# leosampaio/sketchformer

Hardware: AMD Instinct MI355X
Metric: stroke-tokens/sec training step, d_model=128 L=200 B=128, 1/2/4/8 GPU (higher is better)
Workload: dtype f32; 1 GPU; cfg2: sketch-transformer-tf2 4L/8H/d128/dff512 L=200 V=1004 C=345 dropout=0.1, fwd+bwd+Adam(WarmupDecay); global_batch=128, per_gpu_batch=128, seq_len=200, parallelism=dp1, hip_graph=0, dense_gemm_arithmetic=fp32 operands split exactly into 3 bf16 pieces, 6 product...

## Files before the change

include/skf.h:

```cpp
#ifndef SKF_H_
#define SKF_H_
#include <stddef.h>
#include <stdint.h>
#ifdef __cplusplus
extern "C" {
#endif

typedef void* skf_stream_t;

#define SKF_OK 0
#define SKF_EINVAL (-1)
#define SKF_EUNSUPPORTED (-2)
#define SKF_EHIP (-3)

const char* skf_last_error(void);
int skf_version(void);
int skf_device_info(char* name_host, size_t name_len, int* n_devices_host);

int skf_profiler_enable(int on);
int skf_profiler_report(char* buf_host, size_t len);

#define SKF_PREC_F32 0
#define SKF_PREC_BF16X3 3
#define SKF_PREC_BF16X6 6
#define SKF_ATTN_TWO_PASS 0x100
size_t skf_gemm_workspace_bytes(int M, int N, int K, int splits, int with_bias_grad);
int skf_gemm_default_splits(int M, int N, int K);
int skf_gemm_f32(int a_kcontig, int b_kcontig, int M, int N, int K, const float* A, int lda, const float* B, int ldb,
                 float* C, int ldc, const float* bias, int act, const float* relu_src, int ld_relu, int accumulate,
                 int splits, float* bias_grad, int bias_grad_accumulate, void* workspace, size_t workspace_bytes,
                 int precision, skf_stream_t stream);

typedef struct SkfReduceDesc {
  const float* slab; float* C; float* bias_grad;
  int32_t splits, M, N, ldc, block_begin, pad;
} SkfReduceDesc;
int skf_gemm_wgrad_partial(int M, int N, int K, const float* A, int lda, const float* B, int ldb, int splits,
                           int with_bias_grad, float* slab, size_t slab_bytes, int* splits_used_host, int precision,
                           skf_stream_t stream);
int skf_target_live_len(const long long* tar, int tar_ld, int B, int Ld, int* live_len, skf_stream_t stream);
size_t skf_row_blocks_bytes(int rows, int granule);
int skf_row_blocks_build(const int* live_len, int B, int rows_per_sample, int granule, int* blocks, skf_stream_t stream);
int skf_gemm_f32_rows(int a_kcontig, int b_kcontig, int M, int N, int K, const float* A, int lda, const float* B, int ldb,
                      float* C, int ldc, const float* bias, int act, const float* relu_src, int ld_relu, int accumulate,
                      int splits, float* bias_grad, int bias_grad_accumulate, void* workspace, size_t workspace_bytes,
                      int precision, const int* row_blocks, int row_block_rows, skf_stream_t stream);
size_t skf_gemm_relu_bits_bytes(int M, int N, int K, int precision);
int skf_gemm_f32_bits(int a_kcontig, int b_kcontig, int M, int N, int K, const float* A, int lda, const float* B, int ldb,
                      float* C, int ldc, const float* bias, int act, const float* relu_src, int ld_relu, int accumulate,
                      int splits, float* bias_grad, int bias_grad_accumulate, void* workspace, size_t workspace_bytes,
                      int precision, const int* row_blocks, int row_block_rows, void* relu_bits_out, const void* relu_bits_in,
                      skf_stream_t stream);
int skf_gemm_ln_residual_supported(int M, int N, int K, int precision);
int skf_gemm_ln_residual_f32(int M, int N, int K, const float* A, int lda, const float* W, int ldw, const float* bias,
                             const float* x, const float* gamma, const float* beta, float* z, float* out, float* stats,
                             float rate, unsigned site, const void* step_state, int precision, skf_stream_t stream);
int skf_ffn_fused_supported(int M, int d, int dff, int precision);
size_t skf_ffn_image_bytes(int d, int dff, int precision);
size_t skf_ffn_relu_bits_bytes(int M, int d, int dff, int precision);
int skf_ffn_weight_images(int n, const float* const* W1, const int* ld1, const float* const* W2, const int* ld2,
                          const int* transpose, void* const* images, int d, int dff, int precision, skf_stream_t stream);
int skf_ffn_fused_fwd_f32(int M, int d, int dff, const float* x, const void* image, const float* b1, const float* b2,
                          float* h, void* relu_bits_out, const float* gamma, const float* beta, float* z, float* out,
                          float* stats, float rate, unsigned site, const void* step_state, int precision, skf_stream_t stream);
int skf_ffn_fused_bwd_f32(int M, int d, int dff, const float* dy, const void* image_t, const void* relu_bits_in,
                          float* dh, float* dx, int accumulate, const int* row_blocks, int row_block_rows,
                          int precision, skf_stream_t stream);
int skf_ffn_fused_fwd_proj_f32(int M, int d, int dff, const float* x, const void* image, const float* b1, const float* b2,
                               float* h, void* relu_bits_out, const float* gamma, const float* beta, float* z, float* out,
                               float* stats, float rate, unsigned site, const void* step_state, const void* proj_image,
                               const float* proj_bias, int proj_n, float* proj_out, int precision, skf_stream_t stream);
typedef struct SkfFfnBlockFwd {
  uint32_t struct_size; int32_t M, d, dff, precision;
  const float* x; const void* image; const float* b1; const float* b2; float* h; void* relu_bits_out;
  const float* gamma; const float* beta; float* z; float* out; float* stats;
  float rate; uint32_t site; const void* step_state;
  const void* pre_image; const float* pre_bias; const float* pre_residual; const float* pre_gamma; const float* pre_beta;
  float* pre_z; float* pre_out; float* pre_stats; uint32_t pre_site; int32_t proj_n;
  const void* proj_image; const float* proj_bias; float* proj_out;
} SkfFfnBlockFwd;
int skf_ffn_block_fwd_f32(const SkfFfnBlockFwd* block, skf_stream_t stream);
int skf_ffn_fused_ln_partials(int M);
int skf_ffn_fused_bwd_ln_f32(int M, int d, int dff, const float* dout, const float* z, const float* stats, const float* gamma,
                             float rate, unsigned site, const void* step_state, const void* image_t, const void* relu_bits_in,
                             float* dy, float* dh, float* dx, float* ln_partials, size_t ln_partials_bytes,
                             const int* row_blocks, int row_block_rows, int precision, skf_stream_t stream);
size_t skf_dense_image_bytes(int K, int N, int precision);
int skf_dense_weight_images(int n, const float* const* src, const int* ld, const int* transpose, const int* K, const int* N,
                            void* const* images, int precision, skf_stream_t stream);
int skf_layernorm_bwd_dgrad_supported(int M, int d, int precision);
int skf_layernorm_bwd_dgrad_partials(int M);
int skf_layernorm_bwd_dgrad_f32(int M, int d, const float* dout, const float* z, const float* stats, const float* gamma,
                                float rate, unsigned site, const void* step_state, const void* image_t, float* dz, float* dy,
                                float* da, float* ln_partials, size_t ln_partials_bytes, const int* row_blocks,
                                int row_block_rows, int precision, skf_stream_t stream);
int skf_layernorm_bwd_dgrad_lead_f32(int M, int d, const float* dout, const float* lead_a, const void* lead_image_t, const float* z,
                                     const float* stats, const float* gamma, float rate, unsigned site, const void* step_state,
                                     const void* image_t, float* dz, float* dy, float* da, float* ln_partials, size_t ln_partials_bytes,
                                     const int* row_blocks, int row_block_rows, int precision, skf_stream_t stream);
int skf_gemm_wgrad_partial_rows(int M, int N, int K, const float* A, int lda, const float* B, int ldb, int splits,
                                int with_bias_grad, float* slab, size_t slab_bytes, int* splits_used_host, int precision,
                                const int* row_blocks, int row_block_rows, skf_stream_t stream);
typedef struct SkfWgradProblem {
  const float* A; const float* B; float* slab; size_t slab_bytes; const int* row_blocks;
  int32_t M, N, K, lda, ldb, splits, with_bias_grad, row_block_rows, splits_used, pad;
} SkfWgradProblem;
int skf_gemm_wgrad_partial_group(SkfWgradProblem* probs, int n, int precision, skf_stream_t stream);
int skf_splitk_reduce(const float* slab, int splits, int M, int N, float* C, int ldc, int accumulate, float* bias_grad,
                      int bias_grad_accumulate, skf_stream_t stream);
int skf_splitk_reduce_blocks(int M, int N);
int skf_splitk_reduce_batch(const SkfReduceDesc* descs_dev, int ndesc, int total_blocks, skf_stream_t stream);

int skf_attention_fwd(const float* Q, int ldq, const float* K, int ldk, const float* V, int ldv,
                      const unsigned char* key_mask, int key_mask_ld, int causal, int B, int H, int Lq, int Lk, int dh,
                      float* O, int ldo, float* stats, int precision, skf_stream_t stream);
int skf_attention_bwd(const float* Q, int ldq, const float* K, int ldk, const float* V, int ldv, const float* O, int ldo,
                      const float* dO, int lddo, const float* stats, const unsigned char* key_mask, int key_mask_ld,
                      int causal, int B, int H, int Lq, int Lk, int dh, float* dQ, int lddq, float* dK, int lddk,
                      float* dV, int lddv, int precision, skf_stream_t stream);
int skf_attention_bwd_rows(const float* Q, int ldq, const float* K, int ldk, const float* V, int ldv, const float* O, int ldo,
                           const float* dO, int lddo, const float* stats, const unsigned char* key_mask, int key_mask_ld,
                           int causal, int B, int H, int Lq, int Lk, int dh, float* dQ, int lddq, float* dK, int lddk,
                           float* dV, int lddv, int precision, const int* q_live_len, skf_stream_t stream);
int skf_sample_order(const unsigned char* mask_a, int lda, int La, const unsigned char* mask_b, int ldb, int Lb, int B, int* order,
                     skf_stream_t stream);
int skf_attention_fwd_ordered(const float* Q, int ldq, const float* K, int ldk, const float* V, int ldv,
                              const unsigned char* key_mask, int key_mask_ld, int causal, int B, int H, int Lq, int Lk, int dh,
                              float* O, int ldo, float* stats, int precision, const int* sample_order, skf_stream_t stream);
int skf_attention_bwd_ordered(const float* Q, int ldq, const float* K, int ldk, const float* V, int ldv, const float* O, int ldo,
                              const float* dO, int lddo, const float* stats, const unsigned char* key_mask, int key_mask_ld,
                              int causal, int B, int H, int Lq, int Lk, int dh, float* dQ, int lddq, float* dK, int lddk,
                              float* dV, int lddv, int precision, const int* q_live_len, const int* sample_order, skf_stream_t stream);
int skf_attention_weights(const float* Q, int ldq, const float* K, int ldk, const unsigned char* key_mask, int key_mask_ld,
                          int causal, int B, int H, int Lq, int Lk, int dh, float* W, skf_stream_t stream);
int skf_attention_fwd_float_mask(const float* Q, int ldq, const float* K, int ldk, const float* V, int ldv, const float* mask,
                                 long mask_stride_b, long mask_stride_h, long mask_stride_q, int B, int H, int Lq, int Lk, int dh,
                                 float* O, int ldo, float* W, skf_stream_t stream);
int skf_row_mean(const float* a, const float* b, long rows, int cols, int mode, float* out, skf_stream_t stream);

int skf_embed_fwd(const long long* tokens, int tok_ld, int B, int L, const float* table, int vocab, int d,
                  const float* pos, float* out, float rate, unsigned site, const void* step_state, skf_stream_t stream);
int skf_embed_bwd(const long long* tokens, int tok_ld, int B, int L, const float* dx, int vocab, int d, float* dtable,
                  float rate, unsigned site, const void* step_state, skf_stream_t stream);
size_t skf_embed_sort_workspace_bytes(int B, int L, int vocab);
int skf_embed_sort(const long long* tokens, int tok_ld, int B, int L, int vocab, float* zero_table, int d, void* ws,
                   size_t ws_bytes, skf_stream_t stream);
int skf_embed_bwd_sorted(const void* ws, int B, int L, const float* dx, int vocab, int d, float* dtable, float rate,
                         unsigned site, const void* step_state, skf_stream_t stream);
int skf_padding_mask(const long long* tokens, int tok_ld, int B, int L, unsigned char* out, skf_stream_t stream);

int skf_layernorm_residual_fwd(const float* x, float* y_inout_z, const float* gamma, const float* beta, float* out,
                               float* stats, int rows, int d, float rate, unsigned site, const void* step_state,
                               skf_stream_t stream);
size_t skf_layernorm_bwd_workspace_bytes(int rows, int d);
int skf_layernorm_residual_bwd(const float* dout, const float* z, const float* stats, const float* gamma, float* dz,
                               float* dy, float* dgamma, float* dbeta, int rows, int d, float rate, unsigned site,
                               const void* step_state, void* workspace, size_t workspace_bytes, skf_stream_t stream);
int skf_layernorm_residual_bwd_rows(const float* dout, const float* z, const float* stats, const float* gamma, float* dz,
                                    float* dy, float* dgamma, float* dbeta, int rows, int d, float rate, unsigned site,
                                    const void* step_state, void* workspace, size_t workspace_bytes, const int* live_len,
                                    int rows_per_sample, skf_stream_t stream);
int skf_colsum(const float* in, int nrows, int ld, int ncols, float* out, int accumulate, skf_stream_t stream);

int skf_softmax_ce(float* logits, int ld, int rows, int ncls, const long long* target, int tgt_ld, int tgt_cols,
                   int tgt_off, int mask_pad, float scale, float* row_loss, float* row_hit, float* probs_out,
                   int write_grad, skf_stream_t stream);
int skf_metrics_update(const float* recon_loss, const float* recon_hit, int recon_rows, float recon_weight,
                       const float* class_loss, const float* class_hit, int class_rows, float class_weight,
                       const float* recon_scalar ,
                       float* metrics, skf_stream_t stream);

int skf_padding_mask_continuous(const float* x, int x_ld_rows, int B, int L, unsigned char* out, skf_stream_t stream);
int skf_embed_continuous_fwd(const float* x, int x_ld_rows, int B, int L, const float* W, const float* bias, int d,
                             const float* pos, float* out, float rate, unsigned site, const void* step_state,
                             skf_stream_t stream);
size_t skf_embed_continuous_bwd_workspace_bytes(int rows, int d);
int skf_embed_continuous_bwd(const float* x, int x_ld_rows, int B, int L, const float* dx, int d, float* dW, float* dbias,
                             float rate, unsigned site, const void* step_state, void* workspace, size_t workspace_bytes,
                             skf_stream_t stream);
int skf_continuous_loss(float* pred_inout_grad, const float* target, int tgt_ld_rows, int tgt_cols, int tgt_off, int rows,
                        float weight, float* row_loc, float* row_ce, float* row_mask, float* scalars, int write_grad,
                        skf_stream_t stream);

int skf_pool_fwd(const float* u, const float* Vw, const float* x, int B, int L, int U, int d, float* a_out, float* emb,
                 skf_stream_t stream);
int skf_pool_bwd(float* u_inout_dpre, const float* Vw, const float* x, const float* a, const float* demb, int B, int L,
                 int U, int d, float* dx, float* dV, void* workspace, size_t workspace_bytes, skf_stream_t stream);
int skf_expander_fwd(const float* emb, const float* w, const float* bias, int B, int L, int d, float* pre,
                     skf_stream_t stream);
int skf_expander_bwd(const float* dpre, const float* emb, const float* w, int B, int L, int d, float* demb,
                     int demb_accumulate, float* dw, float* dbias, void* workspace, size_t workspace_bytes,
                     skf_stream_t stream);

size_t skf_step_state_bytes(void);
int skf_step_prologue(void* step_state, int schedule, float p0, float p1, float p2, float p3, float beta1, float beta2,
                      unsigned seed, skf_stream_t stream);
int skf_step_epilogue(void* step_state, skf_stream_t stream);
int skf_adam_step(float* w, const float* g, float* m, float* v, size_t n, const void* step_state, float grad_scale,
                  float beta1, float beta2, float eps, skf_stream_t stream);
int skf_sgd_momentum_step(float* w, const float* g, float* velocity, size_t n, const void* step_state, float grad_scale,
                          float momentum, skf_stream_t stream);
int skf_dropout(const float* x, float* y, size_t n, float rate, unsigned site, const void* step_state, skf_stream_t stream);
int skf_dropout_keep_mask(unsigned drop_key, unsigned site, float rate, size_t n, unsigned char* out_host);

int skf_attention_decode(const float* Q, int ldq, const float* K, const float* V, int ld_kv, long long kv_batch_stride,
                         const unsigned char* key_mask, int key_mask_ld, const int* key_limit, int key_limit_all, int B,
                         int H, int Lk, int dh, float* O, int ldo, const int* step_dev, const float* K_new,
                         const float* V_new, int ld_new, int limit_from_step, skf_stream_t stream);
int skf_decode_init(long long* tokens, int tok_ld, float* cont, int cont_ld_rows, unsigned char* selfmask, int mask_ld,
                    int* eos_seen, int* done_step, int B, long long sos, int* step_dev, skf_stream_t stream);
int skf_decode_embed(const long long* tokens, const float* cont, int ld, int B, const float* table, int vocab,
                     const float* W, const float* bias, int d, const float* pos, const int* step_dev, float* out,
                     skf_stream_t stream);
int skf_decode_select_tokens(const float* logits, int ld, int B, int V, int n_valid, int step, long long eos,
                             long long* tokens, int tok_ld, unsigned char* selfmask, int mask_ld, int* eos_seen,
                             int* done_step, int* step_dev, const long long* dyn, skf_stream_t stream);
int skf_decode_select_continuous(const float* pred, int ld, int B, int n_valid, int step, float* out, int out_ld_rows,
                                 unsigned char* selfmask, int mask_ld, int* done_step, int* step_dev,
                                 const long long* dyn, skf_stream_t stream);

typedef struct SkfSampling {
  uint32_t struct_size;
  float temperature;
  int32_t top_k;
  float top_p;
  uint32_t seed;
} SkfSampling;
float skf_sample_uniform(unsigned seed, unsigned stream_id, unsigned step);
int skf_decode_sample_tokens(const float* logits, int ld, int B, int V, int n_valid, int step, long long eos,
                             long long* tokens, int tok_ld, unsigned char* selfmask, int mask_ld, int* eos_seen,
                             int* done_step, int* step_dev, const long long* dyn, const SkfSampling* sampling,
                             const int* stream_ids, skf_stream_t stream);

#define SKF_BEAM_MAX 8
typedef struct SkfBeam {
  uint32_t struct_size;
  int32_t beam_width;
  float length_alpha;
} SkfBeam;
// ... 229 lines not shown
```

sketchformer_amd/_lib.py:

```python
import ctypes as C
import os

HERE = os.path.dirname(os.path.abspath(__file__))
LIB_PATH = os.path.join(HERE, "libskf.so")

SKF_OK = 0
PREC_F32, PREC_BF16X3, PREC_BF16X6 = 0, 3, 6


def default_precision():
    e = os.environ.get("SKF_GEMM_PRECISION", "bf16x6").lower()
    try:
        return {"f32": PREC_F32, "bf16x6": PREC_BF16X6, "bf16x3": PREC_BF16X3, "0": 0, "3": 3, "6": 6}[e]
    except KeyError:
        raise ValueError("SKF_GEMM_PRECISION must be f32, bf16x6 or bf16x3 (got %r)" % e)


class SkfError(RuntimeError):
    pass


ATTN_TWO_PASS = 0x100
MODEL_DECODE_LAYERWISE = 1
MODEL_FFN_LAUNCHES = 2
MODEL_TWO_STREAM_GRAPH = 4


class SkfConfig(C.Structure):
    _fields_ = [
        ("struct_size", C.c_uint32),
        ("batch", C.c_int32), ("seq_len", C.c_int32), ("d_model", C.c_int32), ("num_heads", C.c_int32),
        ("dff", C.c_int32), ("num_layers", C.c_int32),
        ("vocab_size", C.c_int32), ("n_classes", C.c_int32), ("lowerdim", C.c_int32), ("attn_version", C.c_int32),
        ("continuous", C.c_int32), ("blind_decoder_mask", C.c_int32), ("max_pos", C.c_int32),
        ("dropout_rate", C.c_float), ("recon_weight", C.c_float), ("class_weight", C.c_float),
        ("schedule", C.c_int32),
        ("sched_p0", C.c_float), ("sched_p1", C.c_float), ("sched_p2", C.c_float), ("sched_p3", C.c_float),
        ("beta1", C.c_float), ("beta2", C.c_float), ("eps", C.c_float),
        ("seed", C.c_uint32),
        ("use_graph", C.c_int32),
        ("optimizer", C.c_int32), ("momentum", C.c_float),
        ("class_buffer_layers", C.c_int32), ("class_dropout", C.c_float),
        ("do_classification", C.c_int32), ("do_reconstruction", C.c_int32),
        ("gemm_precision", C.c_int32), ("act_dtype", C.c_int32),
    ]

    def __init__(self, *args, **kw):
        super().__init__(*args, **kw)
        if not self.struct_size:
            self.struct_size = C.sizeof(SkfConfig)


class SkfFfnBlockFwd(C.Structure):
    _fields_ = [("struct_size", C.c_uint32), ("M", C.c_int32), ("d", C.c_int32), ("dff", C.c_int32), ("precision", C.c_int32),
                ("x", C.c_void_p), ("image", C.c_void_p), ("b1", C.c_void_p), ("b2", C.c_void_p), ("h", C.c_void_p), ("relu_bits_out", C.c_void_p),
                ("gamma", C.c_void_p), ("beta", C.c_void_p), ("z", C.c_void_p), ("out", C.c_void_p), ("stats", C.c_void_p),
                ("rate", C.c_float), ("site", C.c_uint32), ("step_state", C.c_void_p),
                ("pre_image", C.c_void_p), ("pre_bias", C.c_void_p), ("pre_residual", C.c_void_p), ("pre_gamma", C.c_void_p), ("pre_beta", C.c_void_p),
                ("pre_z", C.c_void_p), ("pre_out", C.c_void_p), ("pre_stats", C.c_void_p), ("pre_site", C.c_uint32), ("proj_n", C.c_int32),
                ("proj_image", C.c_void_p), ("proj_bias", C.c_void_p), ("proj_out", C.c_void_p)]


class SkfKmeansState(C.Structure):
    _fields_ = [("iterations", C.c_int32), ("converged", C.c_int32), ("n_empty", C.c_int32), ("pad", C.c_int32),
                ("inertia", C.c_double), ("shift", C.c_double)]


class SkfSampling(C.Structure):
    _fields_ = [("struct_size", C.c_uint32), ("temperature", C.c_float), ("top_k", C.c_int32), ("top_p", C.c_float),
                ("seed", C.c_uint32)]

    def __init__(self, *args, **kw):
        super().__init__(*args, **kw)
        if not self.struct_size:
            self.struct_size = C.sizeof(SkfSampling)


class SkfBeam(C.Structure):
    _fields_ = [("struct_size", C.c_uint32), ("beam_width", C.c_int32), ("length_alpha", C.c_float)]

    def __init__(self, *args, **kw):
        super().__init__(*args, **kw)
        if not self.struct_size:
            self.struct_size = C.sizeof(SkfBeam)


BEAM_MAX = 8


class SkfParamEntry(C.Structure):
    _fields_ = [("name", C.c_char * 96), ("offset", C.c_int64), ("rows", C.c_int32), ("cols", C.c_int32),
                ("row_stride", C.c_int32)]


_P = C.c_void_p
_I = C.c_int
_F = C.c_float
_Z = C.c_size_t
_U = C.c_uint
_L = C.c_longlong
_D = C.c_double

SIGNATURES = {
    "skf_last_error": (C.c_char_p, []),
    "skf_version": (_I, []),
    "skf_device_info": (_I, [C.c_char_p, _Z, C.POINTER(_I)]),
    "skf_profiler_enable": (_I, [_I]),
    "skf_profiler_report": (_I, [C.c_char_p, _Z]),
    "skf_gemm_workspace_bytes": (_Z, [_I, _I, _I, _I, _I]),
    "skf_gemm_default_splits": (_I, [_I, _I, _I]),
    "skf_gemm_wgrad_partial": (_I, [_I, _I, _I, _P, _I, _P, _I, _I, _I, _P, _Z, _P, _I, _P]),
    "skf_gemm_wgrad_partial_group": (_I, [_P, _I, _I, _P]),
    "skf_gemm_wgrad_partial_rows": (_I, [_I, _I, _I, _P, _I, _P, _I, _I, _I, _P, _Z, _P, _I, _P, _I, _P]),
    "skf_gemm_f32_rows": (_I, [_I, _I, _I, _I, _I, _P, _I, _P, _I, _P, _I, _P, _I, _P, _I, _I, _I, _P, _I, _P, _Z, _I, _P, _I, _P]),
    "skf_gemm_relu_bits_bytes": (_Z, [_I, _I, _I, _I]),
    "skf_gemm_f32_bits": (_I, [_I, _I, _I, _I, _I, _P, _I, _P, _I, _P, _I, _P, _I, _P, _I, _I, _I, _P, _I, _P, _Z, _I, _P, _I, _P, _P, _P]),
    "skf_gemm_ln_residual_supported": (_I, [_I, _I, _I, _I]),
    "skf_gemm_ln_residual_f32": (_I, [_I, _I, _I, _P, _I, _P, _I, _P, _P, _P, _P, _P, _P, _P, _F, _U, _P, _I, _P]),
    "skf_ffn_fused_supported": (_I, [_I, _I, _I, _I]),
    "skf_ffn_image_bytes": (_Z, [_I, _I, _I]),
    "skf_ffn_relu_bits_bytes": (_Z, [_I, _I, _I, _I]),
    "skf_ffn_weight_images": (_I, [_I, _P, _P, _P, _P, _P, _P, _I, _I, _I, _P]),
    "skf_ffn_fused_fwd_f32": (_I, [_I, _I, _I, _P, _P, _P, _P, _P, _P, _P, _P, _P, _P, _P, _F, _U, _P, _I, _P]),
    "skf_ffn_fused_bwd_f32": (_I, [_I, _I, _I, _P, _P, _P, _P, _P, _I, _P, _I, _I, _P]),
    "skf_ffn_fused_ln_partials": (_I, [_I]),
    "skf_ffn_fused_bwd_ln_f32": (_I, [_I, _I, _I, _P, _P, _P, _P, _F, _U, _P, _P, _P, _P, _P, _P, _P, _Z, _P, _I, _I, _P]),
    "skf_dense_image_bytes": (_Z, [_I, _I, _I]),
    "skf_dense_weight_images": (_I, [_I, _P, _P, _P, _P, _P, _P, _I, _P]),
    "skf_layernorm_bwd_dgrad_supported": (_I, [_I, _I, _I]),
    "skf_layernorm_bwd_dgrad_partials": (_I, [_I]),
    "skf_layernorm_bwd_dgrad_f32": (_I, [_I, _I, _P, _P, _P, _P, _F, _U, _P, _P, _P, _P, _P, _P, _Z, _P, _I, _I, _P]),
    "skf_layernorm_bwd_dgrad_lead_f32": (_I, [_I, _I, _P, _P, _P, _P, _P, _P, _F, _U, _P, _P, _P, _P, _P, _P, _Z, _P, _I, _I, _P]),
    "skf_ffn_fused_fwd_proj_f32": (_I, [_I, _I, _I, _P, _P, _P, _P, _P, _P, _P, _P, _P, _P, _P, _F, _U, _P, _P, _P, _I, _P, _I, _P]),
    "skf_ffn_block_fwd_f32": (_I, [C.POINTER(SkfFfnBlockFwd), _P]),
    "skf_target_live_len": (_I, [_P, _I, _I, _I, _P, _P]),
    "skf_row_blocks_bytes": (_Z, [_I, _I]),
    "skf_row_blocks_build": (_I, [_P, _I, _I, _I, _P, _P]),
    "skf_splitk_reduce": (_I, [_P, _I, _I, _I, _P, _I, _I, _P, _I, _P]),
    "skf_splitk_reduce_blocks": (_I, [_I, _I]),
    "skf_splitk_reduce_batch": (_I, [_P, _I, _I, _P]),
    "skf_gemm_f32": (_I, [_I, _I, _I, _I, _I, _P, _I, _P, _I, _P, _I, _P, _I, _P, _I, _I, _I, _P, _I, _P, _Z, _I, _P]),
    "skf_attention_fwd": (_I, [_P, _I, _P, _I, _P, _I, _P, _I, _I, _I, _I, _I, _I, _I, _P, _I, _P, _I, _P]),
    "skf_attention_bwd": (_I, [_P, _I, _P, _I, _P, _I, _P, _I, _P, _I, _P, _P, _I, _I, _I, _I, _I, _I, _I,
                               _P, _I, _P, _I, _P, _I, _I, _P]),
    "skf_attention_bwd_rows": (_I, [_P, _I, _P, _I, _P, _I, _P, _I, _P, _I, _P, _P, _I, _I, _I, _I, _I, _I, _I, _P, _I, _P, _I, _P, _I, _I, _P, _P]),
    "skf_attention_fwd_ordered": (_I, [_P, _I, _P, _I, _P, _I, _P, _I, _I, _I, _I, _I, _I, _I, _P, _I, _P, _I, _P, _P]),
    "skf_attention_bwd_ordered": (_I, [_P, _I, _P, _I, _P, _I, _P, _I, _P, _I, _P, _P, _I, _I, _I, _I, _I, _I, _I, _P, _I, _P, _I, _P, _I, _I, _P, _P, _P]),
    "skf_sample_order": (_I, [_P, _I, _I, _P, _I, _I, _I, _P, _P]),
    "skf_attention_weights": (_I, [_P, _I, _P, _I, _P, _I, _I, _I, _I, _I, _I, _I, _P, _P]),
    "skf_attention_fwd_float_mask": (_I, [_P, _I, _P, _I, _P, _I, _P, C.c_long, C.c_long, C.c_long, _I, _I, _I, _I, _I, _P, _I, _P, _P]),
    "skf_row_mean": (_I, [_P, _P, C.c_long, _I, _I, _P, _P]),
    "skf_embed_fwd": (_I, [_P, _I, _I, _I, _P, _I, _I, _P, _P, _F, _U, _P, _P]),
    "skf_embed_bwd": (_I, [_P, _I, _I, _I, _P, _I, _I, _P, _F, _U, _P, _P]),
    "skf_embed_sort_workspace_bytes": (_Z, [_I, _I, _I]),
    "skf_embed_sort": (_I, [_P, _I, _I, _I, _I, _P, _I, _P, _Z, _P]),
    "skf_embed_bwd_sorted": (_I, [_P, _I, _I, _P, _I, _I, _P, _F, _U, _P, _P]),
    "skf_padding_mask": (_I, [_P, _I, _I, _I, _P, _P]),
    "skf_layernorm_residual_fwd": (_I, [_P, _P, _P, _P, _P, _P, _I, _I, _F, _U, _P, _P]),
    "skf_layernorm_bwd_workspace_bytes": (_Z, [_I, _I]),
    "skf_layernorm_residual_bwd": (_I, [_P, _P, _P, _P, _P, _P, _P, _P, _I, _I, _F, _U, _P, _P, _Z, _P]),
    "skf_layernorm_residual_bwd_rows": (_I, [_P, _P, _P, _P, _P, _P, _P, _P, _I, _I, _F, _U, _P, _P, _Z, _P, _I, _P]),
    "skf_colsum": (_I, [_P, _I, _I, _I, _P, _I, _P]),
    "skf_softmax_ce": (_I, [_P, _I, _I, _I, _P, _I, _I, _I, _I, _F, _P, _P, _P, _I, _P]),
    "skf_metrics_update": (_I, [_P, _P, _I, _F, _P, _P, _I, _F, _P, _P, _P]),
    "skf_padding_mask_continuous": (_I, [_P, _I, _I, _I, _P, _P]),
    "skf_embed_continuous_fwd": (_I, [_P, _I, _I, _I, _P, _P, _I, _P, _P, _F, _U, _P, _P]),
    "skf_embed_continuous_bwd_workspace_bytes": (_Z, [_I, _I]),
    "skf_embed_continuous_bwd": (_I, [_P, _I, _I, _I, _P, _I, _P, _P, _F, _U, _P, _P, _Z, _P]),
    "skf_continuous_loss": (_I, [_P, _P, _I, _I, _I, _I, _F, _P, _P, _P, _P, _I, _P]),
    "skf_pool_fwd": (_I, [_P, _P, _P, _I, _I, _I, _I, _P, _P, _P]),
    "skf_pool_bwd": (_I, [_P, _P, _P, _P, _P, _I, _I, _I, _I, _P, _P, _P, _Z, _P]),
    "skf_expander_fwd": (_I, [_P, _P, _P, _I, _I, _I, _P, _P]),
    "skf_expander_bwd": (_I, [_P, _P, _P, _I, _I, _I, _P, _I, _P, _P, _P, _Z, _P]),
    "skf_config_size": (_Z, []),
    "skf_model_set_flags": (_I, [_P, C.c_uint32]),
    "skf_step_state_bytes": (_Z, []),
    "skf_step_prologue": (_I, [_P, _I, _F, _F, _F, _F, _F, _F, _U, _P]),
    "skf_step_epilogue": (_I, [_P, _P]),
    "skf_adam_step": (_I, [_P, _P, _P, _P, _Z, _P, _F, _F, _F, _F, _P]),
    "skf_sgd_momentum_step": (_I, [_P, _P, _P, _Z, _P, _F, _F, _P]),
    "skf_dropout": (_I, [_P, _P, _Z, _F, _U, _P, _P]),
    "skf_dropout_keep_mask": (_I, [_U, _U, _F, _Z, _P]),
    "skf_attention_decode": (_I, [_P, _I, _P, _P, _I, C.c_longlong, _P, _I, _P, _I, _I, _I, _I, _I, _P, _I, _P, _P, _P, _I,
                                  _I, _P]),
    "skf_decode_init": (_I, [_P, _I, _P, _I, _P, _I, _P, _P, _I, C.c_longlong, _P, _P]),
    "skf_decode_embed": (_I, [_P, _P, _I, _I, _P, _I, _P, _P, _I, _P, _P, _P, _P]),
    "skf_decode_select_tokens": (_I, [_P, _I, _I, _I, _I, _I, C.c_longlong, _P, _I, _P, _I, _P, _P, _P, _P, _P]),
    "skf_sample_uniform": (_F, [_U, _U, _U]),
    "skf_decode_sample_tokens": (_I, [_P, _I, _I, _I, _I, _I, C.c_longlong, _P, _I, _P, _I, _P, _P, _P, _P, C.POINTER(SkfSampling), _P, _P]),
    "skf_decode_select_continuous": (_I, [_P, _I, _I, _I, _I, _P, _I, _P, _I, _P, _P, _P, _P]),
    "skf_gemm_bf16": (_I, [_I, _I, _I, _P, _I, _P, _I, _P, _I, _P, _I, _P, _I, _I, _P, _I, _P]),
    "skf_gemm_bf16_tile_rows": (_I, [_I, _I, _I, _I]),
    "skf_gemm_bf16_rows": (_I, [_I, _I, _I, _P, _I, _P, _I, _P, _I, _P, _I, _P, _I, _I, _P, _I, _P, _I, _P]),
    "skf_gemm_bf16_relu_bits_bytes": (_Z, [_I, _I]),
    "skf_gemm_bf16_bits": (_I, [_I, _I, _I, _P, _I, _P, _I, _P, _I, _P, _I, _P, _I, _I, _P, _I, _P, _I, _P, _P, _I, _P]),
    "skf_gemm_bf16_wgrad_rows": (_I, [_I, _I, _I, _P, _I, _P, _I, _P, _I, _P, _P, _Z, _P, _P]),
    "skf_gemm_bf16_wgrad_partial_rows": (_I, [_I, _I, _I, _P, _I, _P, _I, _I, _I, _P, _Z, _P, _P, _P]),
    "skf_gemm_bf16_wgrad_splits": (_I, [_I, _I, _I]),
    "skf_gemm_bf16_wgrad_workspace_bytes": (_Z, [_I, _I, _I, _I]),
    "skf_gemm_bf16_wgrad_partial": (_I, [_I, _I, _I, _P, _I, _P, _I, _I, _I, _P, _Z, _P, _P]),
    "skf_gemm_bf16_wgrad": (_I, [_I, _I, _I, _P, _I, _P, _I, _P, _I, _P, _P, _Z, _P]),
    "skf_attention_bf16_fwd": (_I, [_P, _I, _P, _I, _P, _I, _P, _I, _I, _I, _I, _I, _I, _I, _P, _I, _P, _P, _P]),
    "skf_attention_bf16_bwd_workspace_bytes": (_Z, [_I, _I, _I]),
    "skf_attention_bf16_bwd": (_I, [_P, _I, _P, _I, _P, _I, _P, _I, _P, _P, _I, _P, _P, _I, _I, _I, _I, _I, _I, _I,
                                    _P, _I, _P, _I, _P, _I, _P, _Z, _P]),
    "skf_attention_bf16_bwd_rows": (_I, [_P, _I, _P, _I, _P, _I, _P, _I, _P, _P, _I, _P, _P, _I, _I, _I, _I, _I, _I, _I, _P, _I, _P, _I, _P, _I, _P, _Z, _P, _P]),
    "skf_attention_bf16_fwd_ordered": (_I, [_P, _I, _P, _I, _P, _I, _P, _I, _I, _I, _I, _I, _I, _I, _P, _I, _P, _P, _P, _P]),
    "skf_attention_bf16_bwd_ordered": (_I, [_P, _I, _P, _I, _P, _I, _P, _I, _P, _P, _I, _P, _P, _I, _I, _I, _I, _I, _I, _I, _P, _I, _P, _I, _P, _I, _P, _Z, _P, _P, _P]),
    "skf_embed_fwd_bf16": (_I, [_P, _I, _I, _I, _P, _I, _I, _P, _P, _F, _U, _P, _P]),
    "skf_embed_bwd_sorted_bf16": (_I, [_P, _I, _I, _P, _I, _I, _P, _F, _U, _P, _P]),
    "skf_layernorm_residual_fwd_bf16": (_I, [_P, _P, _P, _P, _P, _P, _I, _I, _F, _U, _P, _P]),
    "skf_layernorm_bwd_bf16_workspace_bytes": (_Z, [_I, _I]),
    "skf_layernorm_residual_bwd_bf16": (_I, [_P, _P, _P, _P, _P, _P, _P, _P, _I, _I, _F, _U, _P, _P, _Z, _P]),
    "skf_layernorm_residual_bwd_bf16_rows": (_I, [_P, _P, _P, _P, _P, _P, _P, _P, _I, _I, _F, _U, _P, _P, _Z, _P, _I, _P]),
    "skf_softmax_ce_bf16": (_I, [_P, _I, _I, _I, _P, _I, _I, _I, _I, _F, _P, _P, _I, _P]),
    "skf_pool_fwd_bf16": (_I, [_P, _P, _P, _I, _I, _I, _I, _P, _P, _P]),
    "skf_pool_bwd_bf16": (_I, [_P, _P, _P, _P, _P, _I, _I, _I, _I, _P, _P, _P, _Z, _P]),
    "skf_expander_fwd_bf16": (_I, [_P, _P, _P, _I, _I, _I, _P, _P]),
    "skf_expander_bwd_bf16": (_I, [_P, _P, _P, _I, _I, _I, _P, _I, _P, _P, _P, _Z, _P]),
    "skf_cast_weight_bf16": (_I, [_P, _I, _I, _I, _P, _I, _P, _I, _P]),
    "skf_cast_weight_bf16_blocks": (_I, [_I, _I, _I, _I, _P]),
    "skf_cast_weight_bf16_batch": (_I, [_P, _I, _I, _P]),
    "skf_cast_f32_to_bf16": (_I, [_P, _P, _Z, _P]),
    "skf_cast_bf16_to_f32": (_I, [_P, _P, _Z, _P]),
    "skf_config_validate": (_I, [C.POINTER(SkfConfig)]),
    "skf_model_param_floats": (_Z, [C.POINTER(SkfConfig)]),
    "skf_model_param_entries": (_I, [C.POINTER(SkfConfig), C.POINTER(SkfParamEntry), _I]),
    "skf_model_workspace_bytes": (_Z, [C.POINTER(SkfConfig)]),
    "skf_model_create": (_I, [C.POINTER(SkfConfig), C.POINTER(_P)]),
    "skf_model_destroy": (None, [_P]),
    "skf_model_bind": (_I, [_P, _P, _P, _P, _P, _P, _P, _Z, _P, _P]),
    "skf_model_forward": (_I, [_P, _P, _P, _I, _I, _P]),
    "skf_model_wait_inputs_staged": (_I, [_P, _P]),
    "skf_model_forward_backward": (_I, [_P, _P, _P, _I, _P, _P]),
    "skf_model_grad_buckets": (_I, [_P, _I, C.POINTER(_Z), C.POINTER(_Z)]),
    "skf_model_wait_grad_bucket": (_I, [_P, _I, _P]),
    "skf_model_apply_gradients_range": (_I, [_P, _Z, _Z, _F, _I, _P]),
    "skf_model_encode": (_I, [_P, _P, _P]),
    "skf_model_greedy_decode": (_I, [_P, _P, C.POINTER(_I), _I, C.c_longlong, C.c_longlong, _I, _P, C.POINTER(_I), _P]),
    "skf_model_greedy_decode_attn": (_I, [_P, _P, C.POINTER(_I), _I, C.c_longlong, C.c_longlong, _I, _P, C.POINTER(_I), _P, _P]),
    "skf_model_sample_decode": (_I, [_P, _P, C.POINTER(_I), _I, C.c_longlong, C.c_longlong, _I, _P, C.POINTER(_I), C.POINTER(SkfSampling),
                                     C.POINTER(_I), _P]),
    "skf_beam_finish": (_I, [_P, _P, _P, _I, _P, _I, _I, _I, _I, _I, _F, _P, _P, _P, _P]),
    "skf_beam_advance": (_I, [_P, _P, _I, _I, _I, C.c_longlong, _P, _P, _P, _P, _I, _P, _I, _P, _I, _P, _P]),
    "skf_model_beam_decode": (_I, [_P, _P, C.POINTER(_I), _I, C.c_longlong, C.c_longlong, _I, _P, _P, _P, C.POINTER(_I), C.POINTER(SkfBeam), _P]),
    "skf_model_apply_gradients": (_I, [_P, _F, _P]),
    "skf_model_buffer": (_I, [_P, C.c_char_p, C.POINTER(_P), C.POINTER(_I), C.POINTER(_I)]),
    "skf_model_buffer_info": (_I, [_P, C.c_char_p, C.POINTER(_P), C.POINTER(_I), C.POINTER(_I), C.POINTER(_I), C.POINTER(_I)]),
    "skf_knn_workspace_bytes": (_Z, [_I, _I, _I]),
    "skf_knn_topk_f32": (_I, [_P, _I, _I, _P, _I, _I, _I, _I, _P, _P, _P, _P, _Z, _P]),
    "skf_row_normalize_f32": (_I, [_P, _I, _I, _I, _P, _I, _P]),
    "skf_kmeans_workspace_bytes": (_Z, [_L, _I]),
    "skf_kmeans_assign_f32": (_I, [_P, _I, _L, _I, _P, _I, _I, _P, _P, _P]),
    "skf_kmeans_step_f32": (_I, [_P, _I, _L, _I, _P, _I, _I, _I, _D, _P, _P, _P, _P, _Z, _P]),
    "skf_interpolate_f32": (_I, [_P, _I, _P, _I, _I, _I, _P, _I, _I, _P, _I, _P]),
    "skf_tsne_workspace_bytes": (_Z, [_I]),
    "skf_tsne_affinities_f32": (_I, [_P, _I, _I, _I, _D, _P, _I, _P, _P, _Z, _P]),
    "skf_tsne_step_f32": (_I, [_P, _I, _I, _P, _P, _P, _P, _F, _F, _F, _P, _Z, _P]),
    "skf_tsne_kl_f32": (_I, [_P, _I, _I, _P, _P, _P, _Z, _P]),
    "skf_sketch_points": (_I, [_I, _P, _L, _P, _P, _I, _I, _I, _P, _P, _P, _P, _P]),
    "skf_rasterize_f32": (_I, [_P, _P, _P, _P, _I, _I, _I, _I, _F, _F, _P, _P]),
    "skf_raster_overlap_f32": (_I, [_P, _L, _P, _L, _I, _L, _P, _P]),
    "skf_nearest_center_f64": (_I, [_P, _I, _L, _P, _I, _P, _P]),
    "skf_sketch_encode_workspace_bytes": (_Z, [_L, _I]),
    "skf_sketch_encode": (_I, [_P, _L, _P, _I, _I, _P, _I, _I, _U, _P, _P, _P, _Z, _P]),
    "skf_sketch_augment_workspace_bytes": (_Z, [_L, _I]),
    "skf_sketch_augment": (_I, [_P, _L, _P, _I, _P, _D, _D, _U, _P, _P, _P, _Z, _P]),
    "skf_edit_distance_i64": (_I, [_P, _L, _P, _I, _I, _P, _L, _P, _I, _I, _I, _P, _P]),
    "skf_dtw_f32": (_I, [_P, _L, _P, _I, _I, _P, _L, _P, _I, _I, _I, _P, _P]),
}

_lib = None


def load():
    global _lib
    if _lib is not None:
        return _lib
    if not os.path.exists(LIB_PATH):
# ... 24 lines not shown
```

sketchformer_amd/csrc/skf_ffn_fused.h:

```cpp
#pragma once
#include <hip/hip_runtime.h>
#include <stddef.h>

struct FfnFusedParams {
  const float* A; int lda; int M;
  const char* img1; const char* img2;
  const float* bias1; const float* bias2;
  float* H;
  unsigned long long* bits_out;
  const unsigned long long* bits_in;
  float* C;
  int accumulate;
  const float* res;
  const float* gamma; const float* beta; float* out; float* stats;
  float rate; unsigned site; const void* state;
  const int* row_blocks;
  const char* pre_img; const float* pre_bias; const float* pre_res; const float* pre_gamma; const float* pre_beta; unsigned pre_site;
  float* pre_z; float* pre_out; float* pre_stats;
  const char* img3; const float* bias3; float* out2; int n2;
  const float* ln_dout; const float* ln_z; const float* ln_stats;
  float* ln_dy;
  float* ln_part;
};

int skf_ffn_fused_launch(const FfnFusedParams& p, int pieces, int direction, hipStream_t st);
```

sketchformer_amd/csrc/skf_ffn_fused.hip:

```cpp
#include "skf_common.h"
#include "skf_ffn_fused.h"
#include <string>
#include <vector>

namespace {

typedef __bf16 bf16x8 __attribute__((ext_vector_type(8)));
typedef unsigned u32x4 __attribute__((ext_vector_type(4)));
typedef unsigned u32x2 __attribute__((ext_vector_type(2)));

constexpr int FD = 128;
constexpr int FF = 512;
constexpr int HB = 128;
constexpr int NBLK = FF / HB;
constexpr int TR = 16;
constexpr int MAXRT = 4;
constexpr int ROWS = TR * MAXRT;
constexpr int RPITCH = 256;
constexpr int PLANE = ROWS * RPITCH;
constexpr int NKS = 4;
constexpr int YPITCH = FD + 4;
constexpr unsigned OOB = 0x7ffffff0u;

__device__ __forceinline__ f32x4 mfma_bf16(u32x4 a, u32x4 b, f32x4 c) {
  return __builtin_amdgcn_mfma_f32_16x16x32_bf16(__builtin_bit_cast(bf16x8, a), __builtin_bit_cast(bf16x8, b), c, 0, 0, 0);
}

__device__ __forceinline__ __amdgpu_buffer_rsrc_t ffn_rows_rsrc(const float* base, int ld, int M, int row0) {
  const int rows_left = M - row0 > 0 ? M - row0 : 0;
  const unsigned rem = rows_left > 0 ? (unsigned)rows_left * (unsigned)ld * 4u : 0u;
  const unsigned off = rows_left > 0 ? (unsigned)row0 * (unsigned)ld * 4u : 0u;
  return __builtin_amdgcn_make_buffer_rsrc(const_cast<char*>(reinterpret_cast<const char*>(base) + off), 0, rem, 0x00020000);
}

size_t image_bytes(int pieces) { return (size_t)2 * pieces * (FD * FF * 2); }

struct DenseImageDesc { const float* src; char* img; int ld, transpose, K, N, block_begin, pad; };
constexpr int kImageBatch = 80;
struct DenseImageBatch { DenseImageDesc d[kImageBatch]; int n; };

template <int P>
__global__ __launch_bounds__(256) void dense_image_kernel(DenseImageBatch batch) {
  int j = 0;
  while (j + 1 < batch.n && (int)blockIdx.x >= batch.d[j + 1].block_begin) ++j;
  const DenseImageDesc d = batch.d[j];
  const SkfSplitSel sel = skf_split_sel();
  const int t = ((int)blockIdx.x - d.block_begin) * 256 + threadIdx.x;
  const int nks = d.K / 32, f = t >> 6, lane = t & 63, i = lane & 15, g = lane >> 4;
  if (f >= (d.N / 16) * nks) return;
  const int cb = f / nks, s = f % nks;
  float v[8];
#pragma unroll
  for (int e = 0; e < 8; ++e) {
    const int k = 32 * s + 8 * g + e, n = 16 * cb + i;
    v[e] = d.transpose ? d.src[(size_t)n * d.ld + k] : d.src[(size_t)k * d.ld + n];
  }
  u32x4 pc[P];
#pragma unroll
  for (int dd = 0; dd < 4; ++dd) {
    unsigned o[P];
    skf_split2<P>(v[2 * dd], v[2 * dd + 1], o, sel);
#pragma unroll
    for (int q = 0; q < P; ++q) pc[q][dd] = o[q];
  }
  char* base = d.img + (size_t)f * P * 1024 + lane * 16;
#pragma unroll
  for (int q = 0; q < P; ++q) *reinterpret_cast<u32x4*>(base + q * 1024) = pc[q];
}

int launch_images(const DenseImageDesc* descs, int n, int P, hipStream_t st) {
  for (int b0 = 0; b0 < n; b0 += kImageBatch) {
    DenseImageBatch batch{};
    batch.n = n - b0 < kImageBatch ? n - b0 : kImageBatch;
    int blocks = 0;
    for (int j = 0; j < batch.n; ++j) {
      batch.d[j] = descs[b0 + j];
      batch.d[j].block_begin = blocks;
      blocks += skf_cdiv((batch.d[j].N / 16) * (batch.d[j].K / 32) * 64, 256);
    }
    if (P == 2) hipLaunchKernelGGL(dense_image_kernel<2>, dim3(blocks), dim3(256), 0, st, batch);
    else hipLaunchKernelGGL(dense_image_kernel<3>, dim3(blocks), dim3(256), 0, st, batch);
    SKF_LAUNCH_CHECK();
  }
  return SKF_OK;
}

template <int P>
__device__ __forceinline__ void load_frags(u32x4 (&w)[NKS][P], __amdgpu_buffer_rsrc_t img, unsigned lane16, int soff) {
#pragma unroll
  for (int s = 0; s < NKS; ++s)
#pragma unroll
    for (int q = 0; q < P; ++q) w[s][q] = __builtin_amdgcn_raw_buffer_load_b128(img, lane16, soff + (s * P + q) * 1024, 0);
}

template <int P> struct FfnFrags { u32x4 f[2][2][P]; };
template <int P>
__device__ __forceinline__ void load_half(const char* rows, const unsigned (&a_off)[NKS], u32x4 (&f)[2][P], int half) {
#pragma unroll
  for (int sl = 0; sl < 2; ++sl)
#pragma unroll
    for (int q = 0; q < P; ++q) f[sl][q] = *reinterpret_cast<const u32x4*>(rows + q * PLANE + a_off[2 * half + sl]);
}
template <int P>
__device__ __forceinline__ void half_products(const u32x4 (&w)[NKS][P], const u32x4 (&f)[2][P], int half, f32x4& acc0, f32x4& acc1, int& c) {
#pragma unroll
  for (int sl = 0; sl < 2; ++sl) {
    const int s = 2 * half + sl;
#pragma unroll
    for (int d = 1; d < P; ++d)
#pragma unroll
      for (int qa = 0; qa <= d; ++qa) {
        if (c & 1) acc1 = mfma_bf16(w[s][d - qa], f[sl][qa], acc1);
        else acc0 = mfma_bf16(w[s][d - qa], f[sl][qa], acc0);
        ++c;
      }
  }
#pragma unroll
  for (int sl = 0; sl < 2; ++sl) {
    if (c & 1) acc1 = mfma_bf16(w[2 * half + sl][0], f[sl][0], acc1);
    else acc0 = mfma_bf16(w[2 * half + sl][0], f[sl][0], acc0);
    ++c;
  }
}

__device__ __forceinline__ float ffn_half_wave_sum(float v) {
  v += __builtin_bit_cast(float, __builtin_amdgcn_update_dpp(0, __builtin_bit_cast(int, v), 0xB1, 0xf, 0xf, true));
  v += __builtin_bit_cast(float, __builtin_amdgcn_update_dpp(0, __builtin_bit_cast(int, v), 0x4E, 0xf, 0xf, true));
  v += __builtin_bit_cast(float, __builtin_amdgcn_update_dpp(0, __builtin_bit_cast(int, v), 0x141, 0xf, 0xf, true));
  v += __builtin_bit_cast(float, __builtin_amdgcn_update_dpp(0, __builtin_bit_cast(int, v), 0x140, 0xf, 0xf, true));
  return v + __shfl_xor(v, 16, 64);
}

template <int P, int MODE, bool LNB, bool POST, bool PRE, bool NOFFN>
__device__ __forceinline__ void ffn_fused_body(const FfnFusedParams& p) {
  static_assert(!LNB || MODE == 1, "LayerNorm-backward prologue: backward only");
  static_assert(!POST || MODE == 0, "chained projection: forward only");
  static_assert(!PRE || MODE == 0, "leading projection + LayerNorm: forward only");
  static_assert(!NOFFN || (PRE && POST), "tail + projection: needs both stages");
  extern __shared__ __attribute__((aligned(16))) char smem_f[];
  char* Xp = smem_f;
  char* Hp = smem_f + P * PLANE;
  float* Yt = reinterpret_cast<float*>(P * PLANE >= ROWS * YPITCH * 4 ? Hp : Hp + 2 * P * PLANE);
  float* B1s = reinterpret_cast<float*>(Hp + 2 * P * PLANE + (P * PLANE >= ROWS * YPITCH * 4 ? 0 : ROWS * YPITCH * 4));

  const SkfSplitSel sel = skf_split_sel();
  const int tid = threadIdx.x, lane = tid & 63;
  const int wave = __builtin_amdgcn_readfirstlane(tid >> 6);
  const int i = lane & 15, g = lane >> 4;
  const int ntiles = (p.M + TR - 1) / TR;
  typedef const __attribute__((address_space(4))) int* const_i32p;
  const const_i32p blk = (const_i32p)p.row_blocks;
  const int nlive = blk ? blk[0] : ntiles;
  auto phys = [&](int pos) -> int { return pos < nlive ? (blk ? blk[2 + pos] : pos) : ntiles; };

  const int G = gridDim.x, wg = blockIdx.x;
  const int base = nlive / G, rem = nlive % G;
  const int pos_begin = wg * base + (wg < rem ? wg : rem), count = base + (wg < rem ? 1 : 0);
  const int nsub = (count + MAXRT - 1) / MAXRT;

  unsigned a_off[NKS];
#pragma unroll
  for (int s = 0; s < NKS; ++s) a_off[s] = (unsigned)(i * RPITCH + (((4 * s + g) ^ i) << 4));
  const unsigned hw_off = (unsigned)(i * RPITCH + (((2 * wave + (g >> 1)) ^ i) << 4) + 8 * (g & 1));
  const unsigned hc_voff = (unsigned)(i * FF + 16 * wave + 4 * g) * 4u;
  const int st_row = tid >> 5, st_c = tid & 31;
  const unsigned st_off = (unsigned)(st_row * RPITCH + (((st_c >> 1) ^ st_row) << 4) + (st_c & 1) * 8);
  const unsigned st_voff = (unsigned)(st_row * p.lda + 4 * st_c) * 4u;
  if (MODE == 0 && !NOFFN && tid < FF / 4) *reinterpret_cast<f32x4*>(B1s + 4 * tid) = *reinterpret_cast<const f32x4*>(p.bias1 + 4 * tid);
  float* B3s = B1s + FF;
  if (POST && tid >= 128 && tid - 128 < p.n2 / 4) *reinterpret_cast<f32x4*>(B3s + 4 * (tid - 128)) = *reinterpret_cast<const f32x4*>(p.bias3 + 4 * (tid - 128));
  float* PREs = B3s + 384;
  if (PRE && tid >= 256 && tid < 256 + 96) {
    const int j = tid - 256, which = j >> 5, c4 = (j & 31) * 4;
    const float* src = which == 0 ? p.pre_bias : which == 1 ? p.pre_gamma : p.pre_beta;
    *reinterpret_cast<f32x4*>(PREs + which * FD + c4) = *reinterpret_cast<const f32x4*>(src + c4);
  }
  const float* bias1_p = B1s + 16 * wave + 4 * g;
  const f32x4 bias2_r = MODE == 0 && !NOFFN ? *reinterpret_cast<const f32x4*>(p.bias2 + 16 * wave + 4 * g) : (f32x4){0.f, 0.f, 0.f, 0.f};

  const int e_half = lane >> 5, e_sub = lane & 31;
  float inv_keep = 1.f;
  uint32_t thresh = 0u, sk = 0u;
  f32x4 gm = (f32x4){0.f, 0.f, 0.f, 0.f}, bt = gm;
  if constexpr (MODE == 0 || LNB) {
    if (p.rate > 0.f) {
      typedef const __attribute__((address_space(4))) uint32_t* const_u32p;
      const uint32_t key = *(const_u32p)&reinterpret_cast<const SkfStepState*>(p.state)->drop_key;
      sk = skf_site_key(key, p.site);
      thresh = skf_drop_thresh(p.rate);
      inv_keep = 1.0f / (1.0f - p.rate);
    }
    if constexpr (!NOFFN) {
      gm = *reinterpret_cast<const f32x4*>(p.gamma + 4 * e_sub);
      if constexpr (MODE == 0) bt = *reinterpret_cast<const f32x4*>(p.beta + 4 * e_sub);
    }
  }
  f32x4 ln_dg = (f32x4){0.f, 0.f, 0.f, 0.f}, ln_db = ln_dg;

  const __amdgpu_buffer_rsrc_t r_H = __builtin_amdgcn_make_buffer_rsrc(p.H, 0, p.M * (FF * 4), 0x00020000);
  const __amdgpu_buffer_rsrc_t r_A = __builtin_amdgcn_make_buffer_rsrc(const_cast<float*>(LNB ? p.ln_dout : p.A), 0, p.M * p.lda * 4, 0x00020000);
  const __amdgpu_buffer_rsrc_t r_Z = __builtin_amdgcn_make_buffer_rsrc(const_cast<float*>(LNB ? p.ln_z : p.A), 0, LNB ? p.M * (FD * 4) : 0, 0x00020000);
  const __amdgpu_buffer_rsrc_t r_S = __builtin_amdgcn_make_buffer_rsrc(const_cast<float*>(LNB ? p.ln_stats : p.A), 0, LNB ? p.M * 8 : 0, 0x00020000);
  const __amdgpu_buffer_rsrc_t r_DY = __builtin_amdgcn_make_buffer_rsrc(LNB ? p.ln_dy : p.H, 0, LNB ? p.M * (FD * 4) : 0, 0x00020000);
  const __amdgpu_buffer_rsrc_t r_bits = __builtin_amdgcn_make_buffer_rsrc(MODE == 0 && p.bits_out ? (void*)p.bits_out : (void*)p.H, 0,
                                                                          MODE == 0 && p.bits_out ? ntiles * (NBLK * 8 * 32) : 0, 0x00020000);
  const unsigned bits_voff = lane < 4 ? (unsigned)lane * 8u : OOB;
  const __amdgpu_buffer_rsrc_t r_O2 = __builtin_amdgcn_make_buffer_rsrc(POST ? (void*)p.out2 : (void*)p.H, 0, POST ? p.M * p.n2 * 4 : 0, 0x00020000);
  const __amdgpu_buffer_rsrc_t r_R = __builtin_amdgcn_make_buffer_rsrc(const_cast<float*>(PRE ? p.pre_out : p.A), 0, p.M * (PRE ? FD : p.lda) * 4, 0x00020000);
  const __amdgpu_buffer_rsrc_t r_PR = __builtin_amdgcn_make_buffer_rsrc(const_cast<float*>(PRE ? p.pre_res : p.A), 0, PRE ? p.M * (FD * 4) : 0, 0x00020000);
  const __amdgpu_buffer_rsrc_t r_imgp = __builtin_amdgcn_make_buffer_rsrc(const_cast<char*>(PRE ? p.pre_img : p.img1), 0, PRE ? P * FD * FD * 2 : 0, 0x00020000);
  uint32_t sk_pre = 0u;
  if constexpr (PRE) {
    if (p.rate > 0.f) {
      typedef const __attribute__((address_space(4))) uint32_t* const_u32p;
      sk_pre = skf_site_key(*(const_u32p)&reinterpret_cast<const SkfStepState*>(p.state)->drop_key, p.pre_site);
    }
  }
  const unsigned lane16 = (unsigned)lane * 16u;
  const __amdgpu_buffer_rsrc_t r_img1 = __builtin_amdgcn_make_buffer_rsrc(const_cast<char*>(p.img1), 0, P * (FD * FF * 2), 0x00020000);
  const __amdgpu_buffer_rsrc_t r_img2 = __builtin_amdgcn_make_buffer_rsrc(const_cast<char*>(p.img2), 0, P * (FD * FF * 2), 0x00020000);
  const __amdgpu_buffer_rsrc_t r_img3 = __builtin_amdgcn_make_buffer_rsrc(const_cast<char*>(POST ? p.img3 : p.img1), 0, POST ? P * FD * 2 * p.n2 : 0, 0x00020000);
  const int img1_w = wave * (NKS * P * 1024);
  const int img2_w = wave * (16 * P * 1024);
  u32x4 w1[NKS][P], w2[NKS][P];
  if (!NOFFN && nsub > 0) load_frags<P>(w1, r_img1, lane16, img1_w);

  f32x4 xn[MAXRT];
  f32x4 zn[LNB ? MAXRT : 1];
  u32x2 sn[LNB ? MAXRT : 1];
  int tn[MAXRT];
  auto sub_tiles = [&](int pos0, int sub_i, int (&t)[MAXRT]) -> int {
    const int left = count - (pos0 - pos_begin);
    const int n = sub_i < nsub ? (left + (nsub - sub_i) - 1) / (nsub - sub_i) : 0;
#pragma unroll
    for (int rt = 0; rt < MAXRT; ++rt) t[rt] = rt < n ? phys(pos0 + rt) : ntiles;
    return n;
  };
  auto request_rows = [&](const int (&t)[MAXRT], f32x4 (&x)[MAXRT]) {
#pragma unroll
    for (int rt = 0; rt < MAXRT; ++rt) {
      const unsigned voff = t[rt] < ntiles ? st_voff + (unsigned)t[rt] * (unsigned)(TR * p.lda * 4) : OOB;
      x[rt] = __builtin_bit_cast(f32x4, __builtin_amdgcn_raw_buffer_load_b128(r_A, voff, 0, 0));
      if constexpr (LNB) {
        zn[rt] = __builtin_bit_cast(f32x4, __builtin_amdgcn_raw_buffer_load_b128(r_Z, voff, 0, 0));
        sn[rt] = __builtin_amdgcn_raw_buffer_load_b64(r_S, t[rt] < ntiles ? (unsigned)(t[rt] * TR + st_row) * 8u : OOB, 0, 0);
      }
    }
  };
  int pos = pos_begin;
  int nrt_next = sub_tiles(pos, 0, tn);
  request_rows(tn, xn);
  for (int sub = 0; sub < nsub; ++sub) {
    const int nrt = nrt_next;
    int tl[MAXRT];
#pragma unroll
    for (int rt = 0; rt < MAXRT; ++rt) tl[rt] = tn[rt];
    pos += nrt;

    {
    constexpr int NRT = MAXRT;
    constexpr int TILE = TR * RPITCH;
    f32x4 dzr[LNB ? NRT : 1];
#pragma unroll
    for (int rt = 0; rt < NRT; ++rt) {
      if constexpr (LNB) {
        const f32x4 dv = xn[rt], zv = zn[rt];
        typedef float f32x2_t __attribute__((ext_vector_type(2)));
        const f32x2_t ms = __builtin_bit_cast(f32x2_t, sn[rt]);
        const float mean = ms[0], rstd = ms[1];
        const f32x4 xh = (zv - mean) * rstd, gg = dv * gm;
        ln_dg += dv * xh; ln_db += dv;
        const float s1 = ffn_half_wave_sum((gg[0] + gg[1]) + (gg[2] + gg[3])) * (1.0f / FD);
        const float s2 = ffn_half_wave_sum((gg[0] * xh[0] + gg[1] * xh[1]) + (gg[2] * xh[2] + gg[3] * xh[3])) * (1.0f / FD);
        const f32x4 gz = rstd * (gg - s1 - xh * s2);
        dzr[rt] = gz;
        f32x4 gy = gz;
        const unsigned voff = tl[rt] < ntiles ? st_voff + (unsigned)tl[rt] * (unsigned)(TR * FD * 4) : OOB;
        if (p.rate > 0.f) {
#pragma unroll
          for (int e = 0; e < 4; ++e) gy[e] = gz[e] * (skf_keep(sk, (voff >> 2) + e, thresh) ? inv_keep : 0.f);
        }
        __builtin_amdgcn_raw_buffer_store_b128(__builtin_bit_cast(u32x4, gy), r_DY, voff, 0, 0);
        xn[rt] = gy;
      }
      unsigned lo[P], hi[P];
      skf_split2<P>(xn[rt][0], xn[rt][1], lo, sel);
      skf_split2<P>(xn[rt][2], xn[rt][3], hi, sel);
#pragma unroll
      for (int q = 0; q < P; ++q) *reinterpret_cast<u32x2*>(Xp + q * PLANE + rt * TILE + st_off) = (u32x2){lo[q], hi[q]};
    }
    __syncthreads();
    FfnFrags<P> fr;
    auto ln_row = [&](int rt, const f32x4& yv, const f32x4& xv, uint32_t skey, const f32x4& gmv, const f32x4& btv, float* zp, float* op,
                      float* sp, bool planes) {
      const int grow = tl[rt] * TR + 2 * wave + e_half;
      const bool ok = grow < p.M;
      const size_t off = (size_t)(ok ? grow : 0) * FD + 4 * e_sub;
      f32x4 z;
      float sum = 0.f;
#pragma unroll
      for (int e = 0; e < 4; ++e) {
        float yy = yv[e];
        if (p.rate > 0.f) yy *= skf_keep(skey, (uint32_t)off + e, thresh) ? inv_keep : 0.f;
        z[e] = xv[e] + yy;
        sum += z[e];
      }
      const float mean = ffn_half_wave_sum(sum) * (1.0f / FD);
      float sq = 0.f;
#pragma unroll
      for (int e = 0; e < 4; ++e) { const float c = z[e] - mean; sq += c * c; }
      const float rstd = rsqrtf(ffn_half_wave_sum(sq) * (1.0f / FD) + 1e-6f);
      const f32x4 o = (z - mean) * rstd * gmv + btv;
      if (ok) {
        *reinterpret_cast<f32x4*>(zp + off) = z;
        *reinterpret_cast<f32x4*>(op + off) = o;
        if (e_sub == 0) { sp[2 * (size_t)grow] = mean; sp[2 * (size_t)grow + 1] = rstd; }
      }
      if (planes) {
        unsigned lo[P], hi[P];
        skf_split2<P>(o[0], o[1], lo, sel);
        skf_split2<P>(o[2], o[3], hi, sel);
#pragma unroll
        for (int q = 0; q < P; ++q) *reinterpret_cast<u32x2*>(Xp + q * PLANE + rt * TILE + st_off) = (u32x2){lo[q], hi[q]};
      }
    };
    if constexpr (PRE) {
      load_frags<P>(w2, r_imgp, lane16, wave * (NKS * P * 1024));
      f32x4 xres[NRT];
#pragma unroll
      for (int rt = 0; rt < NRT; ++rt)
        xres[rt] = __builtin_bit_cast(f32x4, __builtin_amdgcn_raw_buffer_load_b128(r_PR, tl[rt] < ntiles ? st_voff + (unsigned)tl[rt] * (unsigned)(TR * FD * 4) : OOB, 0, 0));
      const f32x4 bp = *reinterpret_cast<const f32x4*>(PREs + 16 * wave + 4 * g);
      load_half<P>(Xp, a_off, fr.f[0], 0);
#pragma unroll
      for (int t = 0; t < NRT; ++t) {
        if (t < nrt) {
          load_half<P>(Xp + t * TILE, a_off, fr.f[1], 1);
          f32x4 acc0 = bp, acc1 = (f32x4){0.f, 0.f, 0.f, 0.f};
          int c = 0;
          half_products<P>(w2, fr.f[0], 0, acc0, acc1, c);
          if (t + 1 < NRT) load_half<P>(Xp + (t + 1) * TILE, a_off, fr.f[0], 0);
          half_products<P>(w2, fr.f[1], 1, acc0, acc1, c);
          *reinterpret_cast<f32x4*>(Yt + (t * TR + i) * YPITCH + 16 * wave + 4 * g) = acc0 + acc1;
          __builtin_amdgcn_sched_barrier(0);
        }
      }
      __syncthreads();
      const f32x4 gmp = *reinterpret_cast<const f32x4*>(PREs + FD + 4 * e_sub), btp = *reinterpret_cast<const f32x4*>(PREs + 2 * FD + 4 * e_sub);
#pragma unroll
      for (int rt = 0; rt < NRT; ++rt) {
        const f32x4 yv = *reinterpret_cast<const f32x4*>(Yt + (rt * TR + 2 * wave + e_half) * YPITCH + 4 * e_sub);
        ln_row(rt, yv, xres[rt], sk_pre, gmp, btp, p.pre_z, p.pre_out, p.pre_stats, true);
      }
      __syncthreads();
    }

    f32x4 y[NRT];
#pragma unroll
    for (int rt = 0; rt < NRT; ++rt) y[rt] = bias2_r;

#pragma unroll 1
    for (int b = 0; b < (NOFFN ? 0 : NBLK); ++b) {
      char* Hb = Hp + (b & 1) * (P * PLANE);
      const f32x4 b1 = MODE == 0 ? *reinterpret_cast<const f32x4*>(bias1_p + HB * b) : (f32x4){0.f, 0.f, 0.f, 0.f};
      if (b == NBLK - 1) {
        nrt_next = sub_tiles(pos, sub + 1, tn);
        request_rows(tn, xn);
      }
      auto hidden_out = [&](int rt, const f32x4& acc0, const f32x4& acc1) {
        f32x4 h = acc0 + acc1;
        const int tile = tl[rt];
        if constexpr (MODE == 0) {
          unsigned wlo = 0u, whi = 0u;
#pragma unroll
          for (int r = 0; r < 4; ++r) h[r] = __builtin_amdgcn_fmed3f(h[r], 0.f, __builtin_inff());
          const unsigned long long m0 = __ballot(h[0] > 0.f), m1 = __ballot(h[1] > 0.f), m2 = __ballot(h[2] > 0.f), m3 = __ballot(h[3] > 0.f);
#define FFN_WRITELANE(M, L) asm("s_nop 1\n\tv_writelane_b32 %0, %2, " #L "\n\tv_writelane_b32 %1, %3, " #L : "+v"(wlo), "+v"(whi) : "s"((unsigned)(M)), "s"((unsigned)((M) >> 32)))
          FFN_WRITELANE(m0, 0); FFN_WRITELANE(m1, 1); FFN_WRITELANE(m2, 2); FFN_WRITELANE(m3, 3);
#undef FFN_WRITELANE
          __builtin_amdgcn_raw_buffer_store_b64((u32x2){wlo, whi}, r_bits, bits_voff, ((tile * NBLK + b) * 8 + wave) * 32, 0);
        } else {
          typedef const __attribute__((address_space(4))) unsigned long long* const_u64p;
          const const_u64p wp = (const_u64p)(p.bits_in + (((size_t)tile * NBLK + b) * 8 + wave) * 4);
          f32x4 hm;
#pragma unroll
          for (int r = 0; r < 4; ++r) {
            const unsigned long long m = wp[r];
            float v;
            asm("v_cndmask_b32 %0, 0, %1, %2" : "=v"(v) : "v"(h[r]), "s"(m));
            hm[r] = v;
          }
          h = hm;
        }
        __builtin_amdgcn_raw_buffer_store_b128(__builtin_bit_cast(u32x4, h), r_H, hc_voff + (unsigned)tile * (TR * FF * 4), b * (HB * 4), 0);
        unsigned p01[P], p23[P];
        skf_split2<P>(h[0], h[1], p01, sel);
        skf_split2<P>(h[2], h[3], p23, sel);
        char* hrow = Hb + rt * TILE;
#pragma unroll
        for (int q = 0; q < P; ++q) *reinterpret_cast<u32x2*>(hrow + q * PLANE + hw_off) = (u32x2){p01[q], p23[q]};
      };
      load_half<P>(Xp, a_off, fr.f[0], 0);
      f32x4 pacc0 = b1, pacc1 = b1;
#pragma unroll
      for (int t = 0; t < NRT; ++t) {
        if (t < nrt) {
          load_half<P>(Xp + t * TILE, a_off, fr.f[1], 1);
          f32x4 acc0 = b1, acc1 = (f32x4){0.f, 0.f, 0.f, 0.f};
          int c = 0;
          half_products<P>(w1, fr.f[0], 0, acc0, acc1, c);
          if (t == 0) {
            __builtin_amdgcn_sched_barrier(0);
            load_frags<P>(w2, r_img2, lane16, img2_w + b * (NKS * P * 1024));
            __builtin_amdgcn_sched_barrier(0);
          }
          if (t > 0) hidden_out(t - 1, pacc0, pacc1);
          if (t + 1 < NRT) load_half<P>(Xp + (t + 1) * TILE, a_off, fr.f[0], 0);
          half_products<P>(w1, fr.f[1], 1, acc0, acc1, c);
          pacc0 = acc0; pacc1 = acc1;
          __builtin_amdgcn_sched_barrier(0);
        }
      }
#pragma unroll
      for (int t = 0; t < NRT; ++t)
        if (t == nrt - 1) hidden_out(t, pacc0, pacc1);
      load_frags<P>(w1, r_img1, lane16, img1_w + ((b + 1) & (NBLK - 1)) * (8 * NKS * P * 1024));
      __syncthreads();
      load_half<P>(Hb, a_off, fr.f[0], 0);
#pragma unroll
      for (int t = 0; t < NRT; ++t) {
        if (t < nrt) {
          load_half<P>(Hb + t * TILE, a_off, fr.f[1], 1);
          int c = 0;
          f32x4 ya = (f32x4){0.f, 0.f, 0.f, 0.f}, yb = ya;
          half_products<P>(w2, fr.f[0], 0, ya, yb, c);
          if (t + 1 < NRT) load_half<P>(Hb + (t + 1) * TILE, a_off, fr.f[0], 0);
          half_products<P>(w2, fr.f[1], 1, ya, yb, c);
          y[t] += ya + yb;
          __builtin_amdgcn_sched_barrier(0);
        }
      }
    }

    if constexpr (NOFFN) {
      nrt_next = sub_tiles(pos, sub + 1, tn);
      request_rows(tn, xn);
    }
    if constexpr (POST) load_frags<P>(w2, r_img3, lane16, wave * (NKS * P * 1024));
    if constexpr (!NOFFN) {
#pragma unroll
    for (int rt = 0; rt < NRT; ++rt) *reinterpret_cast<f32x4*>(Yt + (rt * TR + i) * YPITCH + 16 * wave + 4 * g) = y[rt];
    f32x4 xres[NRT];
    if constexpr (MODE == 0) {
#pragma unroll
      for (int rt = 0; rt < NRT; ++rt)
        xres[rt] = __builtin_bit_cast(f32x4, __builtin_amdgcn_raw_buffer_load_b128(r_R, tl[rt] < ntiles ? st_voff + (unsigned)tl[rt] * (unsigned)(TR * (PRE ? FD : p.lda) * 4) : OOB, 0, 0));
    }
    __syncthreads();
#pragma unroll
    for (int rt = 0; rt < NRT; ++rt) {
      const int rloc = rt * TR + 2 * wave + e_half;
      const int grow = tl[rt] * TR + 2 * wave + e_half;
      const bool ok = grow < p.M;
      const size_t off = (size_t)(ok ? grow : 0) * FD + 4 * e_sub;
      const f32x4 yv = *reinterpret_cast<const f32x4*>(Yt + rloc * YPITCH + 4 * e_sub);
      if constexpr (MODE == 0) {
        ln_row(rt, yv, xres[rt], sk, gm, bt, p.C, p.out, p.stats, POST);
      } else {
        if (ok) {
          f32x4 v = yv;
          if constexpr (LNB) v += dzr[rt];
          else if (p.accumulate) v += *reinterpret_cast<const f32x4*>(p.C + off);
          *reinterpret_cast<f32x4*>(p.C + off) = v;
        }
      }
    }
    }
    if constexpr (POST) {
      const int nb2 = p.n2 >> 7;
      const int img3_w = wave * (NKS * P * 1024);
      const unsigned o_voff = (unsigned)(i * p.n2 + 16 * wave + 4 * g) * 4u;
      auto post_block = [&](const u32x4 (&w)[NKS][P], int nb) {
        const f32x4 b3 = *reinterpret_cast<const f32x4*>(B3s + nb * 128 + 16 * wave + 4 * g);
        load_half<P>(Xp, a_off, fr.f[0], 0);
#pragma unroll
        for (int t = 0; t < NRT; ++t) {
          if (t < nrt) {
            load_half<P>(Xp + t * TILE, a_off, fr.f[1], 1);
            f32x4 acc0 = b3, acc1 = (f32x4){0.f, 0.f, 0.f, 0.f};
            int c = 0;
            half_products<P>(w, fr.f[0], 0, acc0, acc1, c);
            if (t + 1 < NRT) load_half<P>(Xp + (t + 1) * TILE, a_off, fr.f[0], 0);
            half_products<P>(w, fr.f[1], 1, acc0, acc1, c);
            const f32x4 r = acc0 + acc1;
            __builtin_amdgcn_raw_buffer_store_b128(__builtin_bit_cast(u32x4, r), r_O2, o_voff + (unsigned)tl[t] * (unsigned)(TR * 4) * (unsigned)p.n2, nb * 512, 0);
            __builtin_amdgcn_sched_barrier(0);
          }
        }
      };
      __syncthreads();
      if (nb2 > 1) load_frags<P>(w1, r_img3, lane16, img3_w + 1 * (8 * NKS * P * 1024));
      post_block(w2, 0);
      if (nb2 > 1) {
        if (nb2 > 2) load_frags<P>(w2, r_img3, lane16, img3_w + 2 * (8 * NKS * P * 1024));
        post_block(w1, 1);
        if (nb2 > 2) post_block(w2, 2);
        if constexpr (!NOFFN) load_frags<P>(w1, r_img1, lane16, img1_w);
      }
      __syncthreads();
    }
    }
  }

  if (MODE == 1 && blk) {
    const f32x4 zero = (f32x4){0.f, 0.f, 0.f, 0.f};
    for (int dpos = nlive + wg; dpos < ntiles; dpos += G) {
      const int tile = blk[2 + dpos];
#pragma unroll
      for (int v = 0; v < 4; ++v) {
        const int e = tid + v * 512, row = tile * TR + e / (FF / 4), c4 = (e % (FF / 4)) * 4;
        if (row < p.M) *reinterpret_cast<f32x4*>(p.H + (size_t)row * FF + c4) = zero;
      }
      if (LNB || !p.accumulate) {
        const int row = tile * TR + (tid >> 5);
        if (row < p.M) {
          *reinterpret_cast<f32x4*>(p.C + (size_t)row * FD + 4 * (tid & 31)) = zero;
          if constexpr (LNB) *reinterpret_cast<f32x4*>(p.ln_dy + (size_t)row * FD + 4 * (tid & 31)) = zero;
        }
      }
    }
  }
  if constexpr (LNB) {
#pragma unroll
    for (int e = 0; e < 4; ++e) { ln_dg[e] += __shfl_xor(ln_dg[e], 32, 64); ln_db[e] += __shfl_xor(ln_db[e], 32, 64); }
    float* red = reinterpret_cast<float*>(smem_f);
    __syncthreads();
    if (lane < 32) {
      *reinterpret_cast<f32x4*>(red + (wave * 2 + 0) * FD + 4 * lane) = ln_dg;
      *reinterpret_cast<f32x4*>(red + (wave * 2 + 1) * FD + 4 * lane) = ln_db;
    }
    __syncthreads();
    if (tid < 2 * FD) {
      float t = red[tid];
#pragma unroll
      for (int k = 1; k < 8; ++k) t += red[k * 2 * FD + tid];
      p.ln_part[(size_t)wg * 2 * FD + tid] = t;
    }
  }
}

template <int P, int MODE, bool LNB = false, bool POST = false, bool PRE = false>
__global__ __launch_bounds__(512, 2) void ffn_fused_kernel(FfnFusedParams p) { ffn_fused_body<P, MODE, LNB, POST, PRE, false>(p); }
template <int P>
__global__ __launch_bounds__(512, 2) void attn_tail_proj_kernel(FfnFusedParams p) { ffn_fused_body<P, 0, false, true, true, true>(p); }

struct LnDgradParams {
  const float* dout; const float* z; const float* stats; const float* gamma;
  float* dz; float* dy; float* C;
  const char* img;
  float* part;
  int M; float rate; unsigned site; const void* state;
  const int* row_blocks;
  const float* lead_a; const char* lead_img;
};

template <int P, bool LEAD>
__global__ __launch_bounds__(512, 2) void ln_bwd_dgrad_kernel(LnDgradParams p) {
  extern __shared__ __attribute__((aligned(16))) char smem_f[];
  char* Xp = smem_f;
  float* Yt = reinterpret_cast<float*>(smem_f + P * PLANE);
  constexpr int TILE = TR * RPITCH;
  const SkfSplitSel sel = skf_split_sel();
  const int tid = threadIdx.x, lane = tid & 63;
  const int wave = __builtin_amdgcn_readfirstlane(tid >> 6);
  const int i = lane & 15, g = lane >> 4;
  const int ntiles = (p.M + TR - 1) / TR;
  typedef const __attribute__((address_space(4))) int* const_i32p;
  const const_i32p blk = (const_i32p)p.row_blocks;
  const int nlive = blk ? blk[0] : ntiles;
  auto phys = [&](int pos) -> int { return pos < nlive ? (blk ? blk[2 + pos] : pos) : ntiles; };
  const int G = gridDim.x, wg = blockIdx.x;
  const int base = nlive / G, rem = nlive % G;
  const int pos_begin = wg * base + (wg < rem ? wg : rem), count = base + (wg < rem ? 1 : 0);
  const int nsub = (count + MAXRT - 1) / MAXRT;

  unsigned a_off[NKS];
#pragma unroll
  for (int s = 0; s < NKS; ++s) a_off[s] = (unsigned)(i * RPITCH + (((4 * s + g) ^ i) << 4));
  const unsigned c_voff = (unsigned)(i * FD + 16 * wave + 4 * g) * 4u;
  const int st_row = tid >> 5, st_c = tid & 31;
  const unsigned st_off = (unsigned)(st_row * RPITCH + (((st_c >> 1) ^ st_row) << 4) + (st_c & 1) * 8);
  const unsigned st_voff = (unsigned)(st_row * FD + 4 * st_c) * 4u;
  float inv_keep = 1.f;
  uint32_t thresh = 0u, sk = 0u;
  if (p.rate > 0.f) {
    typedef const __attribute__((address_space(4))) uint32_t* const_u32p;
    const uint32_t key = *(const_u32p)&reinterpret_cast<const SkfStepState*>(p.state)->drop_key;
    sk = skf_site_key(key, p.site);
    thresh = skf_drop_thresh(p.rate);
    inv_keep = 1.0f / (1.0f - p.rate);
  }
  const f32x4 gm = *reinterpret_cast<const f32x4*>(p.gamma + 4 * st_c);
  f32x4 ln_dg = (f32x4){0.f, 0.f, 0.f, 0.f}, ln_db = ln_dg;
  const unsigned row_bytes = (unsigned)p.M * (FD * 4);
  const __amdgpu_buffer_rsrc_t r_D = __builtin_amdgcn_make_buffer_rsrc(const_cast<float*>(p.dout), 0, row_bytes, 0x00020000);
  const __amdgpu_buffer_rsrc_t r_Z = __builtin_amdgcn_make_buffer_rsrc(const_cast<float*>(p.z), 0, row_bytes, 0x00020000);
  const __amdgpu_buffer_rsrc_t r_S = __builtin_amdgcn_make_buffer_rsrc(const_cast<float*>(p.stats), 0, (unsigned)p.M * 8u, 0x00020000);
  const __amdgpu_buffer_rsrc_t r_DZ = __builtin_amdgcn_make_buffer_rsrc(p.dz, 0, row_bytes, 0x00020000);
  const __amdgpu_buffer_rsrc_t r_DY = __builtin_amdgcn_make_buffer_rsrc(p.dy, 0, row_bytes, 0x00020000);
  const __amdgpu_buffer_rsrc_t r_C = __builtin_amdgcn_make_buffer_rsrc(p.C, 0, row_bytes, 0x00020000);
  const __amdgpu_buffer_rsrc_t r_L = __builtin_amdgcn_make_buffer_rsrc(const_cast<float*>(LEAD ? p.lead_a : p.dout), 0, LEAD ? row_bytes : 0, 0x00020000);

  u32x4 w[NKS][P];
  if (nsub > 0) load_frags<P>(w, __builtin_amdgcn_make_buffer_rsrc(const_cast<char*>(p.img), 0, P * FD * FD * 2, 0x00020000), (unsigned)lane * 16u, wave * (NKS * P * 1024));
  u32x4 wl[LEAD ? NKS : 1][P];
  if constexpr (LEAD) {
    if (nsub > 0) load_frags<P>(wl, __builtin_amdgcn_make_buffer_rsrc(const_cast<char*>(p.lead_img), 0, P * FD * FD * 2, 0x00020000), (unsigned)lane * 16u, wave * (NKS * P * 1024));
  }

  f32x4 xn[MAXRT], zn[MAXRT];
  f32x4 an[LEAD ? MAXRT : 1];
  u32x2 sn[MAXRT];
  int tn[MAXRT];
  auto sub_tiles = [&](int pos0, int sub_i, int (&t)[MAXRT]) -> int {
    const int left = count - (pos0 - pos_begin);
    const int n = sub_i < nsub ? (left + (nsub - sub_i) - 1) / (nsub - sub_i) : 0;
#pragma unroll
    for (int rt = 0; rt < MAXRT; ++rt) t[rt] = rt < n ? phys(pos0 + rt) : ntiles;
    return n;
  };
  auto request_rows = [&]() {
#pragma unroll
    for (int rt = 0; rt < MAXRT; ++rt) {
      const unsigned voff = tn[rt] < ntiles ? st_voff + (unsigned)tn[rt] * (unsigned)(TR * FD * 4) : OOB;
      if constexpr (LEAD) an[rt] = __builtin_bit_cast(f32x4, __builtin_amdgcn_raw_buffer_load_b128(r_L, voff, 0, 0));
      xn[rt] = __builtin_bit_cast(f32x4, __builtin_amdgcn_raw_buffer_load_b128(r_D, voff, 0, 0));
      zn[rt] = __builtin_bit_cast(f32x4, __builtin_amdgcn_raw_buffer_load_b128(r_Z, voff, 0, 0));
      sn[rt] = __builtin_amdgcn_raw_buffer_load_b64(r_S, tn[rt] < ntiles ? (unsigned)(tn[rt] * TR + st_row) * 8u : OOB, 0, 0);
    }
  };
  int pos = pos_begin;
  int nrt_next = sub_tiles(pos, 0, tn);
  request_rows();
  for (int sub = 0; sub < nsub; ++sub) {
    const int nrt = nrt_next;
    int tl[MAXRT];
#pragma unroll
    for (int rt = 0; rt < MAXRT; ++rt) tl[rt] = tn[rt];
    pos += nrt;
    if constexpr (LEAD) {
#pragma unroll
      for (int rt = 0; rt < MAXRT; ++rt) {
        unsigned lo[P], hi[P];
        skf_split2<P>(an[rt][0], an[rt][1], lo, sel);
        skf_split2<P>(an[rt][2], an[rt][3], hi, sel);
#pragma unroll
        for (int q = 0; q < P; ++q) *reinterpret_cast<u32x2*>(Xp + q * PLANE + rt * TILE + st_off) = (u32x2){lo[q], hi[q]};
      }
      __syncthreads();
#pragma unroll
      for (int t = 0; t < MAXRT; ++t) {
        if (t < nrt) {
          FfnFrags<P> fr;
          load_half<P>(Xp + t * TILE, a_off, fr.f[0], 0);
          load_half<P>(Xp + t * TILE, a_off, fr.f[1], 1);
          f32x4 acc0 = (f32x4){0.f, 0.f, 0.f, 0.f}, acc1 = acc0;
          int c = 0;
          half_products<P>(wl, fr.f[0], 0, acc0, acc1, c);
          half_products<P>(wl, fr.f[1], 1, acc0, acc1, c);
          *reinterpret_cast<f32x4*>(Yt + (t * TR + i) * YPITCH + 16 * wave + 4 * g) = acc0 + acc1;
        }
      }
      __syncthreads();
    }
#pragma unroll
    for (int rt = 0; rt < MAXRT; ++rt) {
      typedef float f32x2_t __attribute__((ext_vector_type(2)));
      const f32x2_t ms = __builtin_bit_cast(f32x2_t, sn[rt]);
      f32x4 dv = xn[rt];
      if constexpr (LEAD) { if (rt < nrt) dv += *reinterpret_cast<const f32x4*>(Yt + (rt * TR + st_row) * YPITCH + 4 * st_c); }
      const f32x4 zv = zn[rt];
      const f32x4 xh = (zv - ms[0]) * ms[1], gg = dv * gm;
      ln_dg += dv * xh; ln_db += dv;
      const float s1 = ffn_half_wave_sum((gg[0] + gg[1]) + (gg[2] + gg[3])) * (1.0f / FD);
      const float s2 = ffn_half_wave_sum((gg[0] * xh[0] + gg[1] * xh[1]) + (gg[2] * xh[2] + gg[3] * xh[3])) * (1.0f / FD);
      const f32x4 gz = ms[1] * (gg - s1 - xh * s2);
      f32x4 gy = gz;
      const unsigned voff = tl[rt] < ntiles ? st_voff + (unsigned)tl[rt] * (unsigned)(TR * FD * 4) : OOB;
      if (p.rate > 0.f) {
#pragma unroll
        for (int e = 0; e < 4; ++e) gy[e] = gz[e] * (skf_keep(sk, (voff >> 2) + e, thresh) ? inv_keep : 0.f);
      }
      __builtin_amdgcn_raw_buffer_store_b128(__builtin_bit_cast(u32x4, gz), r_DZ, voff, 0, 0);
      __builtin_amdgcn_raw_buffer_store_b128(__builtin_bit_cast(u32x4, gy), r_DY, voff, 0, 0);
      unsigned lo[P], hi[P];
      skf_split2<P>(gy[0], gy[1], lo, sel);
      skf_split2<P>(gy[2], gy[3], hi, sel);
#pragma unroll
      for (int q = 0; q < P; ++q) *reinterpret_cast<u32x2*>(Xp + q * PLANE + rt * TILE + st_off) = (u32x2){lo[q], hi[q]};
    }
    nrt_next = sub_tiles(pos, sub + 1, tn);
    request_rows();
    __syncthreads();
#pragma unroll
    for (int t = 0; t < MAXRT; ++t) {
      if (t < nrt) {
        FfnFrags<P> fr;
        load_half<P>(Xp + t * TILE, a_off, fr.f[0], 0);
        load_half<P>(Xp + t * TILE, a_off, fr.f[1], 1);
        f32x4 acc0 = (f32x4){0.f, 0.f, 0.f, 0.f}, acc1 = acc0;
        int c = 0;
        half_products<P>(w, fr.f[0], 0, acc0, acc1, c);
        half_products<P>(w, fr.f[1], 1, acc0, acc1, c);
        const f32x4 r = acc0 + acc1;
        __builtin_amdgcn_raw_buffer_store_b128(__builtin_bit_cast(u32x4, r), r_C, c_voff + (unsigned)tl[t] * (TR * FD * 4), 0, 0);
      }
    }
    __syncthreads();
  }
  if (blk) {
    const f32x4 zero = (f32x4){0.f, 0.f, 0.f, 0.f};
    for (int dpos = nlive + wg; dpos < ntiles; dpos += G) {
      const int row = blk[2 + dpos] * TR + st_row;
      if (row < p.M) {
        const size_t off = (size_t)row * FD + 4 * st_c;
        *reinterpret_cast<f32x4*>(p.dz + off) = zero;
        *reinterpret_cast<f32x4*>(p.dy + off) = zero;
        *reinterpret_cast<f32x4*>(p.C + off) = zero;
      }
    }
  }
#pragma unroll
  for (int e = 0; e < 4; ++e) { ln_dg[e] += __shfl_xor(ln_dg[e], 32, 64); ln_db[e] += __shfl_xor(ln_db[e], 32, 64); }
  float* red = reinterpret_cast<float*>(smem_f);
  __syncthreads();
  if (lane < 32) {
    *reinterpret_cast<f32x4*>(red + (wave * 2 + 0) * FD + 4 * lane) = ln_dg;
    *reinterpret_cast<f32x4*>(red + (wave * 2 + 1) * FD + 4 * lane) = ln_db;
  }
  __syncthreads();
  if (tid < 2 * FD) {
    float t = red[tid];
#pragma unroll
    for (int k = 1; k < 8; ++k) t += red[k * 2 * FD + tid];
    p.part[(size_t)wg * 2 * FD + tid] = t;
  }
}

int n_cus() {
  static int cache[64] = {0};
  int dev = 0;
  if (hipGetDevice(&dev) != hipSuccess || dev < 0 || dev >= 64) dev = 0;
  if (!cache[dev]) {
    int n = 0;
    if (hipDeviceGetAttribute(&n, hipDeviceAttributeMultiprocessorCount, dev) != hipSuccess || n <= 0) n = 256;
    cache[dev] = n;
  }
  return cache[dev];
}

int ffn_grid(int M) {
  const int ntiles = skf_cdiv(M, TR);
  int g = n_cus();
  if (g > 64) g -= 1;
  return g > ntiles ? ntiles : g;
}

template <int P, int MODE, bool LNB = false, bool POST = false, bool PRE = false>
int launch_ffn(const FfnFusedParams& p, hipStream_t st) {
  const int grid = ffn_grid(p.M);
  const size_t smem = (size_t)3 * P * PLANE + (P * PLANE >= ROWS * YPITCH * 4 ? 0 : ROWS * YPITCH * 4) + (FF + 384 + 3 * FD) * sizeof(float);
  SKF_HIP(hipFuncSetAttribute(reinterpret_cast<const void*>(&ffn_fused_kernel<P, MODE, LNB, POST, PRE>), hipFuncAttributeMaxDynamicSharedMemorySize, (int)smem));
  static const std::string tag = "ffn_fused<d128,dff512,bf16x" + std::to_string(P * (P + 1) / 2) + ">";
  const double live = skf_prof_list_fraction(p.row_blocks);
  const double flops = 2.0 * 2.0 * p.M * FD * FF + (POST ? 2.0 * p.M * FD * p.n2 : 0.0) + (PRE ? 2.0 * p.M * FD * FD : 0.0);
  const double bytes = 4.0 * ((double)p.M * FD * (MODE == 0 ? 4 : 3) + (double)p.M * FF + (POST ? (double)p.M * p.n2 : 0.0) + (PRE ? 4.0 * p.M * FD : 0.0)) + 2.0 * image_bytes(P) / 2;
  SkfProfScope ps(st, tag.c_str(), flops, bytes);
  ps.done(flops * live, bytes * live);
  SKF_LAUNCH_TAIL((ffn_fused_kernel<P, MODE, LNB, POST, PRE>), dim3(grid), dim3(512), smem, st, p);
  SKF_LAUNCH_CHECK();
  return SKF_OK;
}

template <int P>
int launch_tail_proj(const FfnFusedParams& p, hipStream_t st) {
  const int grid = ffn_grid(p.M);
  const size_t smem = (size_t)3 * P * PLANE + (P * PLANE >= ROWS * YPITCH * 4 ? 0 : ROWS * YPITCH * 4) + (FF + 384 + 3 * FD) * sizeof(float);
  SKF_HIP(hipFuncSetAttribute(reinterpret_cast<const void*>(&attn_tail_proj_kernel<P>), hipFuncAttributeMaxDynamicSharedMemorySize, (int)smem));
  static const std::string tag = std::string("attn_tail_proj<d128,bf16x") + std::to_string(P * (P + 1) / 2) + ">";
  const double flops = 2.0 * p.M * FD * FD + 2.0 * p.M * FD * p.n2;
  const double bytes = 4.0 * ((double)p.M * FD * 4 + (double)p.M * p.n2) + 2.0 * P * FD * (FD + p.n2);
  SkfProfScope ps(st, tag.c_str(), flops, bytes);
  ps.done(flops, bytes);
  hipLaunchKernelGGL((attn_tail_proj_kernel<P>), dim3(grid), dim3(512), smem, st, p);
  SKF_LAUNCH_CHECK();
  return SKF_OK;
}

}

int skf_ffn_fused_launch(const FfnFusedParams& p, int pieces, int direction, hipStream_t st) {
  if (direction == 0 && p.pre_img && p.img3 && !p.img1) return pieces == 2 ? launch_tail_proj<2>(p, st) : launch_tail_proj<3>(p, st);
  if (direction == 1 && p.ln_dout) return pieces == 2 ? launch_ffn<2, 1, true>(p, st) : launch_ffn<3, 1, true>(p, st);
  if (direction == 0 && p.pre_img && p.img3) return pieces == 2 ? launch_ffn<2, 0, false, true, true>(p, st) : launch_ffn<3, 0, false, true, true>(p, st);
  if (direction == 0 && p.pre_img) return pieces == 2 ? launch_ffn<2, 0, false, false, true>(p, st) : launch_ffn<3, 0, false, false, true>(p, st);
  if (direction == 0 && p.img3) return pieces == 2 ? launch_ffn<2, 0, false, true>(p, st) : launch_ffn<3, 0, false, true>(p, st);
  if (pieces == 2) return direction == 0 ? launch_ffn<2, 0>(p, st) : launch_ffn<2, 1>(p, st);
  return direction == 0 ? launch_ffn<3, 0>(p, st) : launch_ffn<3, 1>(p, st);
}

extern "C" int skf_ffn_fused_supported(int M, int d, int dff, int precision) {
  return (precision == SKF_PREC_BF16X6 || precision == SKF_PREC_BF16X3) && d == FD && dff == FF && M >= 1 && (double)M * FF * 4 < 2147483648.0;
}
extern "C" size_t skf_ffn_image_bytes(int d, int dff, int precision) {
  if (!skf_ffn_fused_supported(1, d, dff, precision)) return 0;
  return image_bytes(precision == SKF_PREC_BF16X3 ? 2 : 3);
}
extern "C" size_t skf_ffn_relu_bits_bytes(int M, int d, int dff, int precision) {
  if (!skf_ffn_fused_supported(M, d, dff, precision)) return 0;
  return (size_t)skf_cdiv(M, TR) * NBLK * 8 * 4 * sizeof(unsigned long long);
}

extern "C" size_t skf_dense_image_bytes(int K, int N, int precision) {
  if ((precision != SKF_PREC_BF16X6 && precision != SKF_PREC_BF16X3) || K <= 0 || N <= 0 || (K & 31) || (N & 15)) return 0;
  return (size_t)(precision == SKF_PREC_BF16X3 ? 2 : 3) * K * N * 2;
}

extern "C" int skf_dense_weight_images(int n, const float* const* src, const int* ld, const int* transpose, const int* K, const int* N,
                                       void* const* images, int precision, skf_stream_t stream) {
  SKF_CHECK_ARG(precision == SKF_PREC_BF16X6 || precision == SKF_PREC_BF16X3, "pre-split images exist in the split-arithmetic modes only");
  SKF_CHECK_ARG(n >= 0 && (n == 0 || (src && ld && transpose && K && N && images)), "null argument");
  std::vector<DenseImageDesc> descs((size_t)n);
  for (int j = 0; j < n; ++j) {
    SKF_CHECK_ARG(src[j] && images[j] && ((uintptr_t)images[j] & 15) == 0, "null / unaligned operand");
    SKF_CHECK_ARG(K[j] > 0 && N[j] > 0 && (K[j] & 31) == 0 && (N[j] & 15) == 0 && ld[j] >= (transpose[j] ? K[j] : N[j]), "K % 32, N % 16, pitch");
    descs[j] = DenseImageDesc{src[j], (char*)images[j], ld[j], transpose[j] ? 1 : 0, K[j], N[j], 0, 0};
  }
  return launch_images(descs.data(), n, precision == SKF_PREC_BF16X3 ? 2 : 3, (hipStream_t)stream);
}

extern "C" int skf_ffn_weight_images(int n, const float* const* W1, const int* ld1, const float* const* W2, const int* ld2,
                                     const int* transpose, void* const* images, int d, int dff, int precision, skf_stream_t stream) {
  SKF_CHECK_ARG(skf_ffn_fused_supported(1, d, dff, precision), "skf_ffn_weight_images: d = 128, dff = 512 in a split-arithmetic mode only");
  SKF_CHECK_ARG(n >= 0 && (n == 0 || (W1 && ld1 && W2 && ld2 && transpose && images)), "null argument");
  const int P = precision == SKF_PREC_BF16X3 ? 2 : 3;
  std::vector<DenseImageDesc> descs;
  for (int j = 0; j < n; ++j) {
    SKF_CHECK_ARG(W1[j] && W2[j] && images[j] && ld1[j] >= dff && ld2[j] >= d, "bad weight operand");
    SKF_CHECK_ARG(((uintptr_t)images[j] & 15) == 0, "images must be 16-byte aligned");
    char* img = (char*)images[j];
    if (!transpose[j]) {
      descs.push_back(DenseImageDesc{W1[j], img, ld1[j], 0, d, dff, 0, 0});
      descs.push_back(DenseImageDesc{W2[j], img + image_bytes(P) / 2, ld2[j], 0, dff, d, 0, 0});
    } else {
      descs.push_back(DenseImageDesc{W2[j], img, ld2[j], 1, d, dff, 0, 0});
      descs.push_back(DenseImageDesc{W1[j], img + image_bytes(P) / 2, ld1[j], 1, dff, d, 0, 0});
    }
  }
  return launch_images(descs.data(), (int)descs.size(), P, (hipStream_t)stream);
}

static int ffn_common_checks(int M, int d, int dff, int precision, const void* a, const void* img, const void* hid, const void* c) {
  SKF_CHECK_ARG(skf_ffn_fused_supported(M, d, dff, precision), "fused feed-forward block: d = 128, dff = 512 in a split-arithmetic mode only (skf_ffn_fused_supported)");
  SKF_CHECK_ARG(a && img && hid && c, "null operand");
  SKF_CHECK_ARG((((uintptr_t)a | (uintptr_t)img | (uintptr_t)hid | (uintptr_t)c) & 15) == 0, "operands must be 16-byte aligned");
  return SKF_OK;
}

extern "C" int skf_ffn_fused_fwd_f32(int M, int d, int dff, const float* x, const void* image, const float* b1, const float* b2,
                                     float* h, void* relu_bits_out, const float* gamma, const float* beta, float* z, float* out,
                                     float* stats, float rate, unsigned site, const void* step_state, int precision, skf_stream_t stream) {
  const int rc = ffn_common_checks(M, d, dff, precision, x, image, h, z);
  if (rc != SKF_OK) return rc;
  SKF_CHECK_ARG(gamma && beta && out && stats && b1 && b2, "null bias / LayerNorm operand");
  SKF_CHECK_ARG(rate >= 0.f && rate < 1.f && (rate == 0.f || step_state), "dropout needs 0 <= rate < 1 and the step state");
  SKF_CHECK_ARG((((uintptr_t)out | (uintptr_t)gamma | (uintptr_t)beta) & 15) == 0 && (((uintptr_t)stats | (uintptr_t)relu_bits_out) & 7) == 0, "operands must be 16-byte aligned");
  const int P = precision == SKF_PREC_BF16X3 ? 2 : 3;
  FfnFusedParams p{};
  p.A = x; p.lda = d; p.M = M;
  p.img1 = (const char*)image; p.img2 = (const char*)image + image_bytes(P) / 2;
  p.bias1 = b1; p.bias2 = b2; p.H = h; p.bits_out = (unsigned long long*)relu_bits_out;
  p.C = z; p.res = x; p.gamma = gamma; p.beta = beta; p.out = out; p.stats = stats;
  p.rate = rate; p.site = site; p.state = step_state;
  return skf_ffn_fused_launch(p, P, 0, (hipStream_t)stream);
}

extern "C" int skf_ffn_fused_bwd_f32(int M, int d, int dff, const float* dy, const void* image_t, const void* relu_bits_in,
                                     float* dh, float* dx, int accumulate, const int* row_blocks, int row_block_rows,
                                     int precision, skf_stream_t stream) {
  const int rc = ffn_common_checks(M, d, dff, precision, dy, image_t, dh, dx);
  if (rc != SKF_OK) return rc;
  SKF_CHECK_ARG(relu_bits_in && ((uintptr_t)relu_bits_in & 7) == 0, "the backward needs the sign bits the forward wrote");
  SKF_CHECK_ARG(!row_blocks || row_block_rows == TR, "row-block lists of this kernel have 16-row blocks");
  const int P = precision == SKF_PREC_BF16X3 ? 2 : 3;
  FfnFusedParams p{};
  p.A = dy; p.lda = d; p.M = M;
  p.img1 = (const char*)image_t; p.img2 = (const char*)image_t + image_bytes(P) / 2;
  p.H = dh; p.bits_in = (const unsigned long long*)relu_bits_in;
  p.C = dx; p.accumulate = accumulate; p.row_blocks = row_blocks;
  return skf_ffn_fused_launch(p, P, 1, (hipStream_t)stream);
}

extern "C" int skf_ffn_fused_ln_partials(int M) { return ffn_grid(M); }

extern "C" int skf_ffn_fused_bwd_ln_f32(int M, int d, int dff, const float* dout, const float* z, const float* stats, const float* gamma,
                                        float rate, unsigned site, const void* step_state, const void* image_t, const void* relu_bits_in,
                                        float* dy, float* dh, float* dx, float* ln_partials, size_t ln_partials_bytes,
                                        const int* row_blocks, int row_block_rows, int precision, skf_stream_t stream) {
  const int rc = ffn_common_checks(M, d, dff, precision, dout, image_t, dh, dx);
  if (rc != SKF_OK) return rc;
  SKF_CHECK_ARG(z && stats && gamma && dy && ln_partials, "null LayerNorm operand");
  SKF_CHECK_ARG((((uintptr_t)z | (uintptr_t)gamma | (uintptr_t)dy | (uintptr_t)ln_partials) & 15) == 0 && ((uintptr_t)stats & 7) == 0, "operands must be 16-byte aligned");
  SKF_CHECK_ARG(relu_bits_in && ((uintptr_t)relu_bits_in & 7) == 0, "the backward needs the sign bits the forward wrote");
  SKF_CHECK_ARG(rate >= 0.f && rate < 1.f && (rate == 0.f || step_state), "dropout needs 0 <= rate < 1 and the step state");
  SKF_CHECK_ARG(!row_blocks || row_block_rows == TR, "row-block lists of this kernel have 16-row blocks");
  SKF_CHECK_ARG(ln_partials_bytes >= (size_t)ffn_grid(M) * 2 * FD * sizeof(float), "partial buffer too small (skf_ffn_fused_ln_partials(M) x 2 x d floats)");
  const int P = precision == SKF_PREC_BF16X3 ? 2 : 3;
  FfnFusedParams p{};
  p.A = dout; p.lda = d; p.M = M;
  p.img1 = (const char*)image_t; p.img2 = (const char*)image_t + image_bytes(P) / 2;
  p.H = dh; p.bits_in = (const unsigned long long*)relu_bits_in;
  p.C = dx; p.accumulate = 0; p.row_blocks = row_blocks;
  p.gamma = gamma; p.rate = rate; p.site = site; p.state = step_state;
  p.ln_dout = dout; p.ln_z = z; p.ln_stats = stats; p.ln_dy = dy; p.ln_part = ln_partials;
  return skf_ffn_fused_launch(p, P, 1, (hipStream_t)stream);
}

extern "C" int skf_layernorm_bwd_dgrad_supported(int M, int d, int precision) {
  return (precision == SKF_PREC_BF16X6 || precision == SKF_PREC_BF16X3) && d == FD && M >= 1 && (double)M * FD * 4 < 2147483648.0;
}
extern "C" int skf_layernorm_bwd_dgrad_partials(int M) { return ffn_grid(M); }

extern "C" int skf_layernorm_bwd_dgrad_f32(int M, int d, const float* dout, const float* z, const float* stats, const float* gamma,
                                           float rate, unsigned site, const void* step_state, const void* image_t, float* dz, float* dy,
                                           float* da, float* ln_partials, size_t ln_partials_bytes, const int* row_blocks,
                                           int row_block_rows, int precision, skf_stream_t stream) {
  return skf_layernorm_bwd_dgrad_lead_f32(M, d, dout, nullptr, nullptr, z, stats, gamma, rate, site, step_state, image_t, dz, dy, da, ln_partials,
                                          ln_partials_bytes, row_blocks, row_block_rows, precision, stream);
}

extern "C" int skf_layernorm_bwd_dgrad_lead_f32(int M, int d, const float* dout, const float* lead_a, const void* lead_image_t, const float* z,
                                                const float* stats, const float* gamma, float rate, unsigned site, const void* step_state,
                                                const void* image_t, float* dz, float* dy, float* da, float* ln_partials, size_t ln_partials_bytes,
                                                const int* row_blocks, int row_block_rows, int precision, skf_stream_t stream) {
  SKF_CHECK_ARG(skf_layernorm_bwd_dgrad_supported(M, d, precision), "LayerNorm backward + input gradient: d = 128 in a split-arithmetic mode only");
  SKF_CHECK_ARG(!lead_a == !lead_image_t && (((uintptr_t)lead_a | (uintptr_t)lead_image_t) & 15) == 0, "leading product: rows and the transposed image together, 16-byte aligned");
  SKF_CHECK_ARG(dout && z && stats && gamma && image_t && dz && dy && da && ln_partials, "null operand");
  SKF_CHECK_ARG((((uintptr_t)dout | (uintptr_t)z | (uintptr_t)gamma | (uintptr_t)image_t | (uintptr_t)dz | (uintptr_t)dy | (uintptr_t)da |
                  (uintptr_t)ln_partials) & 15) == 0 && ((uintptr_t)stats & 7) == 0, "operands must be 16-byte aligned");
  SKF_CHECK_ARG(rate >= 0.f && rate < 1.f && (rate == 0.f || step_state), "dropout needs 0 <= rate < 1 and the step state");
  SKF_CHECK_ARG(!row_blocks || row_block_rows == TR, "row-block lists of this kernel have 16-row blocks");
  SKF_CHECK_ARG(ln_partials_bytes >= (size_t)ffn_grid(M) * 2 * FD * sizeof(float), "partial buffer too small (skf_layernorm_bwd_dgrad_partials(M) x 2 x d floats)");
  const int P = precision == SKF_PREC_BF16X3 ? 2 : 3;
  LnDgradParams p{};
  p.dout = dout; p.z = z; p.stats = stats; p.gamma = gamma; p.dz = dz; p.dy = dy; p.C = da; p.img = (const char*)image_t;
  p.part = ln_partials; p.M = M; p.rate = rate; p.site = site; p.state = step_state; p.row_blocks = row_blocks;
  p.lead_a = lead_a; p.lead_img = (const char*)lead_image_t;
  const int grid = ffn_grid(M);
  const bool lead = lead_a != nullptr;
  const size_t smem = (size_t)P * PLANE + (lead ? (size_t)ROWS * YPITCH * sizeof(float) : 0);
  hipStream_t st = (hipStream_t)stream;
  static const std::string tag2 = "ln_bwd_dgrad<d128,bf16x3>", tag3 = "ln_bwd_dgrad<d128,bf16x6>";
  const double live = skf_prof_list_fraction(row_blocks);
  const double nprod = lead ? 2.0 : 1.0, nrows = lead ? 6.0 : 5.0;
  SkfProfScope ps(st, (P == 2 ? tag2 : tag3).c_str(), nprod * 2.0 * M * FD * FD, 4.0 * nrows * M * FD);
  ps.done(nprod * 2.0 * M * FD * FD * live, 4.0 * nrows * M * FD * live);
#define SKF_LN_DGRAD_GO(PV, LV)                                                                                                                  \
  {                                                                                                                                              \
    SKF_HIP(hipFuncSetAttribute(reinterpret_cast<const void*>(&ln_bwd_dgrad_kernel<PV, LV>), hipFuncAttributeMaxDynamicSharedMemorySize, (int)smem)); \
    SKF_LAUNCH_TAIL((ln_bwd_dgrad_kernel<PV, LV>), dim3(grid), dim3(512), smem, st, p);                                                          \
  }
  if (P == 2) { if (lead) SKF_LN_DGRAD_GO(2, true) else SKF_LN_DGRAD_GO(2, false) }
  else { if (lead) SKF_LN_DGRAD_GO(3, true) else SKF_LN_DGRAD_GO(3, false) }
#undef SKF_LN_DGRAD_GO
  SKF_LAUNCH_CHECK();
  return SKF_OK;
}

extern "C" int skf_ffn_fused_fwd_proj_f32(int M, int d, int dff, const float* x, const void* image, const float* b1, const float* b2,
                                          float* h, void* relu_bits_out, const float* gamma, const float* beta, float* z, float* out,
                                          float* stats, float rate, unsigned site, const void* step_state, const void* proj_image,
                                          const float* proj_bias, int proj_n, float* proj_out, int precision, skf_stream_t stream) {
  const int rc = ffn_common_checks(M, d, dff, precision, x, image, h, z);
  if (rc != SKF_OK) return rc;
  SKF_CHECK_ARG(gamma && beta && out && stats && b1 && b2, "null bias / LayerNorm operand");
  SKF_CHECK_ARG(rate >= 0.f && rate < 1.f && (rate == 0.f || step_state), "dropout needs 0 <= rate < 1 and the step state");
  SKF_CHECK_ARG((((uintptr_t)out | (uintptr_t)gamma | (uintptr_t)beta) & 15) == 0 && (((uintptr_t)stats | (uintptr_t)relu_bits_out) & 7) == 0, "operands must be 16-byte aligned");
  SKF_CHECK_ARG(proj_image && proj_bias && proj_out && (proj_n == 128 || proj_n == 256 || proj_n == 384), "chained projection: N in {128, 256, 384} with its image, bias and output");
  SKF_CHECK_ARG((((uintptr_t)proj_image | (uintptr_t)proj_bias | (uintptr_t)proj_out) & 15) == 0 && (double)M * proj_n * 4 < 2147483648.0, "chained projection operands");
  const int P = precision == SKF_PREC_BF16X3 ? 2 : 3;
  FfnFusedParams p{};
  p.A = x; p.lda = d; p.M = M;
  p.img1 = (const char*)image; p.img2 = (const char*)image + image_bytes(P) / 2;
  p.bias1 = b1; p.bias2 = b2; p.H = h; p.bits_out = (unsigned long long*)relu_bits_out;
  p.C = z; p.res = x; p.gamma = gamma; p.beta = beta; p.out = out; p.stats = stats;
  p.rate = rate; p.site = site; p.state = step_state;
  p.img3 = (const char*)proj_image; p.bias3 = proj_bias; p.out2 = proj_out; p.n2 = proj_n;
  return skf_ffn_fused_launch(p, P, 0, (hipStream_t)stream);
}

extern "C" int skf_ffn_block_fwd_f32(const SkfFfnBlockFwd* b, skf_stream_t stream) {
  SKF_CHECK_ARG(b && b->struct_size == sizeof(SkfFfnBlockFwd), "SkfFfnBlockFwd.struct_size does not match this library's include/skf.h");
  const bool tail_only = !b->image;
  if (tail_only) {
    SKF_CHECK_ARG(skf_ffn_fused_supported(b->M, b->d, b->dff > 0 ? b->dff : FF, b->precision), "row-owner launches: d = 128 in a split-arithmetic mode only");
    SKF_CHECK_ARG(b->x && b->pre_image && b->proj_image && ((uintptr_t)b->x & 15) == 0, "without a feed-forward image the launch needs the leading stage and the chained projection");
  } else {
    const int rc = ffn_common_checks(b->M, b->d, b->dff, b->precision, b->x, b->image, b->h, b->z);
    if (rc != SKF_OK) return rc;
    SKF_CHECK_ARG(b->gamma && b->beta && b->out && b->stats && b->b1 && b->b2, "null bias / LayerNorm operand");
    SKF_CHECK_ARG((((uintptr_t)b->out | (uintptr_t)b->gamma | (uintptr_t)b->beta | (uintptr_t)b->b1 | (uintptr_t)b->b2) & 15) == 0 &&
                  (((uintptr_t)b->stats | (uintptr_t)b->relu_bits_out) & 7) == 0, "operands must be 16-byte aligned");
  }
  SKF_CHECK_ARG(b->rate >= 0.f && b->rate < 1.f && (b->rate == 0.f || b->step_state), "dropout needs 0 <= rate < 1 and the step state");
  const int P = b->precision == SKF_PREC_BF16X3 ? 2 : 3;
  FfnFusedParams p{};
  p.A = b->x; p.lda = b->d; p.M = b->M;
  p.img1 = (const char*)b->image; p.img2 = tail_only ? nullptr : (const char*)b->image + image_bytes(P) / 2;
  p.bias1 = b->b1; p.bias2 = b->b2; p.H = b->h; p.bits_out = (unsigned long long*)b->relu_bits_out;
  p.C = b->z; p.res = b->x; p.gamma = b->gamma; p.beta = b->beta; p.out = b->out; p.stats = b->stats;
  p.rate = b->rate; p.site = b->site; p.state = b->step_state;
  if (b->pre_image) {
    SKF_CHECK_ARG(b->pre_bias && b->pre_residual && b->pre_gamma && b->pre_beta && b->pre_z && b->pre_out && b->pre_stats, "leading projection: null operand");
    SKF_CHECK_ARG((((uintptr_t)b->pre_image | (uintptr_t)b->pre_bias | (uintptr_t)b->pre_residual | (uintptr_t)b->pre_gamma | (uintptr_t)b->pre_beta |
                    (uintptr_t)b->pre_z | (uintptr_t)b->pre_out) & 15) == 0 && ((uintptr_t)b->pre_stats & 7) == 0, "leading projection: alignment");
    p.pre_img = (const char*)b->pre_image; p.pre_bias = b->pre_bias; p.pre_res = b->pre_residual; p.pre_gamma = b->pre_gamma;
    p.pre_beta = b->pre_beta; p.pre_site = b->pre_site; p.pre_z = b->pre_z; p.pre_out = b->pre_out; p.pre_stats = b->pre_stats;
  }
  if (b->proj_image) {
    SKF_CHECK_ARG(b->proj_bias && b->proj_out && (b->proj_n == 128 || b->proj_n == 256 || b->proj_n == 384), "chained projection: N in {128, 256, 384} with its image, bias and output");
    SKF_CHECK_ARG((((uintptr_t)b->proj_image | (uintptr_t)b->proj_bias | (uintptr_t)b->proj_out) & 15) == 0 && (double)b->M * b->proj_n * 4 < 2147483648.0, "chained projection operands");
    p.img3 = (const char*)b->proj_image; p.bias3 = b->proj_bias; p.out2 = b->proj_out; p.n2 = b->proj_n;
  }
  return skf_ffn_fused_launch(p, P, 0, (hipStream_t)stream);
}
```

sketchformer_amd/csrc/skf_model_bwd.hip:

```cpp
#include "skf_model_internal.h"

namespace skf_model_detail {
namespace {

template <typename F>
int with_ready_event(SkfModel* M, bool want, hipEvent_t* ready, F call) {
  hipEvent_t e = (want && may_park(M)) ? M->sched.take_event() : nullptr;
  bool rode = false;
  const int rc = with_tail_event(M, e, &rode, call);
  *ready = rode ? e : nullptr;
  return rc;
}

int ffn_bwd(SkfModel* M, const DenseP& f1, const DenseP& f2, const float* x_in, const float* h, const float* dy,
            float* dh, float* dx_acc, int rows, hipStream_t s, const void* hbits, const void* image_t) {
  if (M->ctx.ffn_fused) {
    SKF_TRY(dense_wgrad(M, f2, h, f2.in, dy, f2.out, rows, s));
    SKF_TRY(M->sched.before_write(M, dh, s));
    SKF_TRY(M->sched.before_write(M, dx_acc, s));
    const int* blocks = M->ctx.live_blocks(rows, 16);
    hipEvent_t ready = nullptr;
    SKF_TRY(with_ready_event(M, M->sched.holding(), &ready, [&] {
      return skf_ffn_fused_bwd_f32(rows, M->cfg.d_model, M->cfg.dff, dy, image_t, hbits, dh, dx_acc, 1, blocks, blocks ? 16 : 0,
                                   M->cfg.gemm_precision, s);
    }));
    SKF_TRY(M->sched.issue_held(M, s, ready));
    return dense_wgrad(M, f1, x_in, f1.in, dh, f1.out, rows, s);
  }
  SKF_TRY(dense_wgrad(M, f2, h, f2.in, dy, f2.out, rows, s));
  SKF_TRY(dense_dgrad(M, f2, dy, f2.out, rows, dh, f2.in, 0, h, f2.in, s, hbits));
  SKF_TRY(dense_wgrad(M, f1, x_in, f1.in, dh, f1.out, rows, s));
  SKF_TRY(dense_dgrad(M, f1, dh, f1.out, rows, dx_acc, f1.in, 1, nullptr, 0, s));
  return SKF_OK;
}

int ln_partials_desc(SkfModel* M, const LnP& ln, const float* part, int splits) {
  const int d = M->cfg.d_model;
  SkfReduceDesc r;
  r.slab = part; r.C = M->G(ln.g); r.bias_grad = nullptr; r.splits = splits; r.M = 1; r.N = 2 * d;
  r.ldc = 2 * d; r.block_begin = M->red.blocks(); r.pad = 0;
  SKF_TRY(M->red.add(r, skf_splitk_reduce_blocks(1, 2 * d)));
  M->red.ln_cursor += 1;
  return SKF_OK;
}

int colsum_desc(SkfModel* M, const float* part, int splits, int n, float* C) {
  SKF_CHECK_ARG(M->red.end() < M->plan.n_wgrads, "reduction descriptor table exhausted");
  SkfReduceDesc r;
  r.slab = part; r.C = C; r.bias_grad = nullptr; r.splits = splits; r.M = 1; r.N = n;
  r.ldc = n; r.block_begin = M->red.blocks(); r.pad = 0;
  return M->red.add(r, skf_splitk_reduce_blocks(1, n));
}

int ln_bwd(SkfModel* M, const LnP& ln, const float* dout, const float* z, const float* st, float* dz, float* dy,
           int rows, float rate, unsigned site, hipStream_t s) {
  const Plan& P = M->plan;
  const int d = M->cfg.d_model;
  SKF_TRY(M->sched.before_write(M, dz, s));
  if (dy != dz) SKF_TRY(M->sched.before_write(M, dy, s));
  const int* ll = M->ctx.live_lengths(rows);
  const int rps = M->cfg.seq_len - 1;
  if (!M->sched.side || ln.b != ln.g + (size_t)d)
    return skf_layernorm_residual_bwd_rows(dout, z, st, M->P(ln.g), dz, dy, M->G(ln.g), M->G(ln.b), rows, d, rate,
                                           site, M->state, M->at<char>(P.small_ws), P.small_ws_bytes, ll, rps, s);
  float* part = M->red.take_ln_partial(M);
  if (!part) return SKF_EINVAL;
  const size_t bytes = skf_layernorm_bwd_workspace_bytes(rows, d);
  SKF_TRY(skf_layernorm_residual_bwd_rows(dout, z, st, M->P(ln.g), dz, dy, nullptr, nullptr, rows, d, rate, site, M->state, part,
                                          bytes, ll, rps, s));
  return ln_partials_desc(M, ln, part, (int)(bytes / (8 * (size_t)d)));
}

bool row_owner_takes_ln(const SkfModel* M, const LnP& ln, size_t pbytes, int rows = 0, const DenseP* o = nullptr, const DenseP* lead_w = nullptr) {
  const int d = M->cfg.d_model;
  auto square = [d](const DenseP* w) { return !w || (w->in == d && w->out == d); };
  return M->ctx.ffn_fused && M->sched.side && ln.b == ln.g + (size_t)d && pbytes <= M->plan.ln_part_stride && square(o) && square(lead_w) &&
         (!o || skf_layernorm_bwd_dgrad_supported(rows, d, M->cfg.gemm_precision));
}

int ffn_ln_bwd(SkfModel* M, const LnP& ln, const DenseP& f1, const DenseP& f2, const float* dout, const float* z, const float* st,
               const float* x_in, const float* h, float* dy, float* dh, float* dx, int rows, float rate, unsigned site, hipStream_t s,
               const void* hbits, const void* image_t) {
  const int d = M->cfg.d_model;
  M->ctx.last_ready = nullptr;
  const size_t pbytes = (size_t)skf_ffn_fused_ln_partials(rows) * 2 * d * sizeof(float);
  if (!row_owner_takes_ln(M, ln, pbytes)) {
    SKF_TRY(ln_bwd(M, ln, dout, z, st, dx, dy, rows, rate, site, s));
    return ffn_bwd(M, f1, f2, x_in, h, dy, dh, dx, rows, s, hbits, image_t);
  }
  float* part = M->red.take_ln_partial(M);
  if (!part) return SKF_EINVAL;
  SKF_TRY(M->sched.before_write(M, dy, s));
  SKF_TRY(M->sched.before_write(M, dh, s));
  SKF_TRY(M->sched.before_write(M, dx, s));
  const int* blocks = M->ctx.live_blocks(rows, 16);
  hipEvent_t ready = nullptr;
  SKF_TRY(with_ready_event(M, M->sched.holding(), &ready, [&] {
    return skf_ffn_fused_bwd_ln_f32(rows, d, M->cfg.dff, dout, z, st, M->P(ln.g), rate, site, M->state, image_t, hbits, dy, dh, dx, part,
                                    pbytes, blocks, blocks ? 16 : 0, M->cfg.gemm_precision, s);
  }));
  SKF_TRY(ln_partials_desc(M, ln, part, skf_ffn_fused_ln_partials(rows)));
  M->ctx.last_ready = ready;
  SKF_TRY(M->sched.issue_held(M, s, ready));
  SKF_TRY(dense_wgrad(M, f2, h, f2.in, dy, f2.out, rows, s));
  return dense_wgrad(M, f1, x_in, f1.in, dh, f1.out, rows, s);
}

size_t ln_oproj_partial_bytes(const SkfModel* M, int rows) { return (size_t)skf_layernorm_bwd_dgrad_partials(rows) * 2 * M->cfg.d_model * sizeof(float); }
int ln_oproj_bwd(SkfModel* M, const LnP& ln, const DenseP& o, const float* dout, const float* z, const float* st, const float* a_in,
                 float* dz, float* dy, float* da, int rows, float rate, unsigned site, hipStream_t s, const void* image_t,
                 const float* lead_a = nullptr, const void* lead_image_t = nullptr) {
  const int d = M->cfg.d_model;
  const size_t pbytes = ln_oproj_partial_bytes(M, rows);
  if (!row_owner_takes_ln(M, ln, pbytes, rows, &o)) {
    SKF_CHECK_ARG(!lead_a && !lead_image_t, "a lead operand needs the fused launch");
    SKF_TRY(ln_bwd(M, ln, dout, z, st, dz, dy, rows, rate, site, s));
    SKF_TRY(dense_wgrad(M, o, a_in, d, dy, d, rows, s));
    return dense_dgrad(M, o, dy, d, rows, da, d, 0, nullptr, 0, s);
  }
  float* part = M->red.take_ln_partial(M);
  if (!part) return SKF_EINVAL;
  SKF_TRY(M->sched.before_write(M, dz, s));
  SKF_TRY(M->sched.before_write(M, dy, s));
  SKF_TRY(M->sched.before_write(M, da, s));
  const int* blocks = M->ctx.live_blocks(rows, 16);
  SKF_TRY(skf_layernorm_bwd_dgrad_lead_f32(rows, d, dout, lead_a, lead_image_t, z, st, M->P(ln.g), rate, site, M->state, image_t, dz, dy, da, part,
                                           pbytes, blocks, blocks ? 16 : 0, M->cfg.gemm_precision, s));
  SKF_TRY(ln_partials_desc(M, ln, part, skf_layernorm_bwd_dgrad_partials(rows)));
  return dense_wgrad(M, o, a_in, d, dy, d, rows, s);
}

int build_row_lists(SkfModel* M, hipStream_t s) {
  const SkfConfig& c = M->cfg;
  const Plan& P = M->plan;
  M->ctx.lists_built = false;
  if (c.continuous || !do_recon(c) || c.gemm_precision == SKF_PREC_F32) return SKF_OK;
  const int B = c.batch, Le = c.seq_len, Ld = c.seq_len - 1;
  SKF_TRY(skf_target_live_len(M->at<long long>(P.tar), Le, B, Ld, M->at<int>(P.live_len), s));
  SKF_TRY(skf_row_blocks_build(M->at<int>(P.live_len), B, Ld, 16, M->at<int>(P.live16), s));
  SKF_TRY(skf_row_blocks_build(M->at<int>(P.live_len), B, Ld, 32, M->at<int>(P.live32), s));
  M->ctx.lists_built = true;
  return SKF_OK;
}

}

int run_backward(SkfModel* M, hipStream_t s) {
  M->ctx.begin_backward();
  M->sched.begin_backward();
  M->red.begin_step();
  const SkfConfig& c = M->cfg;
  const Layout& L = M->lay;
  const Plan& P = M->plan;
  const int B = c.batch, Le = c.seq_len, Ld = c.seq_len - 1, d = c.d_model, H = c.num_heads, dh = d / H;
  const int Me = B * Le, Md = B * Ld, N = c.num_layers;
  const float rate = c.dropout_rate;
  const long long* inp = M->at<long long>(P.inp);
  const long long* tar = M->at<long long>(P.tar);
  const unsigned char* emask = M->at<unsigned char>(P.enc_mask);
  const unsigned char* dmask = M->at<unsigned char>(P.dec_mask);
  float* G = M->at<float>(P.gA);
  float* G2 = M->at<float>(P.gB);
  float* dO = M->at<float>(P.do_);
  float* dpre = M->at<float>(P.dpre);
  float* demb = M->at<float>(P.demb);
  int layer_no = 0;

  const bool bott = has_bott(c), cls = has_cls(c), recon = do_recon(c);
  float* enc_out = M->at<float>(P.enc[N - 1].x2);
  const float* pre = bott ? M->at<float>(P.pre) : enc_out;
  if (recon) {
  if (!M->ctx.lists_built) SKF_TRY(build_row_lists(M, s));
  if (M->ctx.lists_built) M->ctx.set_live(Md, M->at<int>(P.live_len), 16, M->at<int>(P.live16), 32, M->at<int>(P.live32));
  M->ctx.lists_built = false;
  const float* dlog = M->at<float>(P.logits);
  SKF_TRY(dense_wgrad(M, L.out, M->at<float>(P.dec[N - 1].out3), d, dlog, L.out.out, Md, s));
  {
    hipEvent_t ready = nullptr;
    SKF_TRY(with_ready_event(M, true, &ready, [&] { return dense_dgrad(M, L.out, dlog, L.out.out, Md, G, d, 0, nullptr, 0, s); }));
    SKF_TRY(M->sched.issue(M, s, ready));
  }
  const unsigned char* cross_mask = c.blind_decoder_mask ? nullptr : emask;
  for (int i = N - 1; i >= 0; --i, ++layer_no) {
    const DecLayerP& w = L.dec[i];
    const DecAct& a = P.dec[i];
    const Plan::GradSet& gs = P.gs[layer_no % P.n_gs];
    float* dy3 = M->at<float>(gs.dy[0]); float* dy2 = M->at<float>(gs.dy[1]); float* dy1 = M->at<float>(gs.dy[2]);
    float* dqkv = M->at<float>(gs.dqkv); float* dkv2 = M->at<float>(gs.dkv2); float* dq2 = M->at<float>(gs.dq2);
    SKF_TRY(ffn_ln_bwd(M, w.ln3, w.f1, w.f2, G, M->at<float>(a.z3), M->at<float>(a.st3), M->at<float>(a.out2), M->at<float>(a.h), dy3,
                       M->at<float>(gs.dh), G2, Md, rate, site_dec(N, i, 2), s, hbits_of(M, a.hbits, Md), M->at<char>(a.img[1])));
    SKF_TRY(ln_oproj_bwd(M, w.ln2, w.mha2.o, G2, M->at<float>(a.z2), M->at<float>(a.st2), M->at<float>(a.o2), G, dy2, dO, Md, rate,
                         site_dec(N, i, 1), s, M->at<char>(a.img_o2)));
    const float* kv2 = M->at<float>(a.kv2);
    SKF_TRY(M->sched.before_write(M, dq2, s));
    SKF_TRY(M->sched.before_write(M, dkv2, s));
    const int* qlive = M->ctx.live_lengths(Md);
    SKF_TRY(skf_attention_bwd_ordered(M->at<float>(a.q2), d, kv2, 2 * d, kv2 + d, 2 * d, M->at<float>(a.o2), d, dO, d,
                                      M->at<float>(a.astats2), cross_mask, Le, 0, B, H, Ld, Le, dh, dq2, d, dkv2, 2 * d,
                                      dkv2 + d, 2 * d, M->cfg.gemm_precision, qlive, M->ctx.order, s));
    SKF_TRY(dense_wgrad(M, w.mha2.q, M->at<float>(a.out1), d, dq2, d, Md, s));
    const bool lead = row_owner_takes_ln(M, w.ln1, ln_oproj_partial_bytes(M, Md), Md, &w.mha1.o, &w.mha2.q);
    if (!lead) SKF_TRY(dense_dgrad(M, w.mha2.q, dq2, d, Md, G, d, 1, nullptr, 0, s));
    SKF_TRY(dense_wgrad(M, w.mha2.kv, pre, L.E, dkv2, 2 * d, Me, s));
    if (i == 0) {
      SKF_TRY(M->sched.before_read(M, dpre, s));
      SKF_TRY(dense_dgrad(M, w.mha2.kv, dkv2, 2 * d, Me, dpre, L.E, i != N - 1, nullptr, 0, s));
    } else SKF_TRY(dense_dgrad_deferred(M, w.mha2.kv, dkv2, 2 * d, Me, dpre, L.E, i != N - 1, s));
    SKF_TRY(ln_oproj_bwd(M, w.ln1, w.mha1.o, G, M->at<float>(a.z1), M->at<float>(a.st1), M->at<float>(a.o1), G2, dy1, dO, Md, rate,
                         site_dec(N, i, 0), s, M->at<char>(a.img_o1), lead ? dq2 : nullptr, lead ? M->at<char>(a.img_q2t) : nullptr));
    const float* qkv = M->at<float>(a.qkv);
    SKF_TRY(M->sched.before_write(M, dqkv, s));
    SKF_TRY(skf_attention_bwd_ordered(qkv, 3 * d, qkv + d, 3 * d, qkv + 2 * d, 3 * d, M->at<float>(a.o1), d, dO, d,
                                      M->at<float>(a.astats1), dmask, Ld, 1, B, H, Ld, Ld, dh, dqkv, 3 * d, dqkv + d, 3 * d,
                                      dqkv + 2 * d, 3 * d, M->cfg.gemm_precision, qlive, M->ctx.order, s));
    SKF_TRY(dense_wgrad(M, w.mha1.qkv, M->at<float>(a.x_in), d, dqkv, 3 * d, Md, s));
    const bool hold = M->ctx.ffn_fused && i > 0;
    hipEvent_t ready = nullptr;
    SKF_TRY(with_ready_event(M, !hold, &ready, [&] { return dense_dgrad(M, w.mha1.qkv, dqkv, 3 * d, Md, G2, d, 1, nullptr, 0, s); }));
    float* t = G; G = G2; G2 = t;
    if (hold) SKF_TRY(M->sched.hold(M, s));
    else SKF_TRY(M->sched.issue(M, s, ready));
  }
  M->ctx.clear_live();
  hipEvent_t dec_emb_done = nullptr;
  if (c.continuous) {
    SKF_TRY(skf_embed_continuous_bwd(M->at<float>(P.tar), Le, B, Ld, G, d, M->G(L.dec_embd.w), M->G(L.dec_embd.b), rate,
                                     site_dec_embed(N), M->state, M->at<char>(P.small_ws), P.small_ws_bytes, s));
  } else {
    if (P.emb_sort_bytes) {
      SKF_TRY(with_ready_event(M, M->n_buckets == 2, &dec_emb_done, [&] {
        return skf_embed_bwd_sorted(M->at<char>(P.emb_sort[1]), B, Ld, G, c.vocab_size, d, M->G(L.dec_emb), rate, site_dec_embed(N), M->state, s);
      }));
    } else {
      SKF_HIP(hipMemsetAsync(M->G(L.dec_emb), 0, (size_t)c.vocab_size * d * sizeof(float), s));
      SKF_TRY(skf_embed_bwd(tar, Le, B, Ld, G, c.vocab_size, d, M->G(L.dec_emb), rate, site_dec_embed(N), M->state, s));
    }
  }
  if (M->n_buckets == 2) SKF_TRY(flush_wgrads(M, s, 0, false, true, dec_emb_done));
  SKF_TRY(M->sched.before_read(M, dpre, s));
  }
  const int E = L.E, Ua = L.Ua, U = c.lowerdim, NB = c.class_buffer_layers;
  hipEvent_t bott_ready = nullptr;
  if (bott) {
    const bool defer_sums = M->sched.side && Ua <= 4096;
    float* xp1 = M->at<float>(P.bott_part);
    float* xp2 = xp1 + (size_t)B * Le;
    float* pvp = xp2 + (size_t)B * Le;
    if (recon && defer_sums) {
      SKF_TRY(skf_expander_bwd_partials(dpre, M->at<float>(P.emb), M->P(L.exp_w), B, Le, E, demb, 0, xp1, xp2, s));
      SKF_TRY(colsum_desc(M, xp1, B, Le, M->G(L.exp_w)));
      SKF_TRY(colsum_desc(M, xp2, B, Le, M->G(L.exp_b)));
    } else if (recon)
      SKF_TRY(skf_expander_bwd(dpre, M->at<float>(P.emb), M->P(L.exp_w), B, Le, E, demb, 0, M->G(L.exp_w), M->G(L.exp_b),
                               M->at<char>(P.small_ws), P.small_ws_bytes, s));
    const int acc_emb = recon ? 1 : 0;
    const float* dcls = M->at<float>(P.cls_logits);
    if (cls && NB == 0) {
      SKF_TRY(dense_wgrad(M, L.cls, M->at<float>(P.emb), E, dcls, c.n_classes, B, s));
      SKF_TRY(dense_dgrad(M, L.cls, dcls, c.n_classes, B, demb, E, acc_emb, nullptr, 0, s));
    } else if (cls) {
      float* dz = M->at<float>(P.dcb[0]);
      float* dz2 = M->at<float>(P.dcb[1]);
      SKF_TRY(M->sched.before_write(M, dz, s));
      SKF_TRY(dense_wgrad(M, L.cls, M->at<float>(P.cb_f[NB - 1]), U, dcls, c.n_classes, B, s));
      SKF_TRY(dense_dgrad(M, L.cls, dcls, c.n_classes, B, dz, U, 0, M->at<float>(P.cb_h[NB - 1]), U, s));
      for (int i = NB - 1; i >= 0; --i) {
        SKF_TRY(skf_dropout(dz, dz, (size_t)B * U, c.class_dropout, site_class(N, i), M->state, s));
        const float* in = i == 0 ? M->at<float>(P.emb) : M->at<float>(P.cb_f[i - 1]);
        const int in_w = i == 0 ? E : U;
        SKF_TRY(dense_wgrad(M, L.cbuf[i], in, in_w, dz, U, B, s));
        if (i == 0) {
          SKF_TRY(dense_dgrad(M, L.cbuf[0], dz, U, B, demb, E, acc_emb, nullptr, 0, s));
        } else {
          SKF_TRY(M->sched.before_write(M, dz2, s));
          SKF_TRY(dense_dgrad(M, L.cbuf[i], dz, U, B, dz2, U, 0, M->at<float>(P.cb_h[i - 1]), U, s));
          float* t = dz; dz = dz2; dz2 = t;
        }
      }
    }
    const float* dpool = demb;
    if (c.attn_version == 2) {
      SKF_TRY(M->sched.before_write(M, M->at<float>(P.dpooled), s));
      SKF_TRY(dense_wgrad(M, L.bott_e, M->at<float>(P.pooled), d, demb, U, B, s));
      SKF_TRY(dense_dgrad(M, L.bott_e, demb, U, B, M->at<float>(P.dpooled), d, 0, nullptr, 0, s));
      dpool = M->at<float>(P.dpooled);
    }
    SKF_TRY(M->sched.before_write(M, G, s));
    if (defer_sums) {
      SKF_TRY(skf_pool_bwd_partials(M->at<float>(P.u), M->P(L.bott_v), enc_out, M->at<float>(P.pool_a), dpool, B, Le, Ua, d, G, pvp, s));
      SKF_TRY(colsum_desc(M, pvp, B, Ua, M->G(L.bott_v)));
    } else
    SKF_TRY(skf_pool_bwd(M->at<float>(P.u), M->P(L.bott_v), enc_out, M->at<float>(P.pool_a), dpool, B, Le, Ua, d,
                         G, M->G(L.bott_v), M->at<char>(P.small_ws), P.small_ws_bytes, s));
    SKF_TRY(dense_wgrad(M, L.bott_w, enc_out, d, M->at<float>(P.u), Ua, Me, s));
    SKF_TRY(with_ready_event(M, true, &bott_ready, [&] { return dense_dgrad(M, L.bott_w, M->at<float>(P.u), Ua, Me, G, d, 1, nullptr, 0, s); }));
  } else {
    float* spare = (G == M->at<float>(P.gA)) ? M->at<float>(P.gB) : M->at<float>(P.gA);
    G = dpre; G2 = spare;
  }
  SKF_TRY(M->sched.issue(M, s, bott_ready));
  for (int i = N - 1; i >= 0; --i, ++layer_no) {
    const EncLayerP& w = L.enc[i];
    const EncAct& a = P.enc[i];
    const Plan::GradSet& gs = P.gs[layer_no % P.n_gs];
    float* dy2 = M->at<float>(gs.dy[0]); float* dy1 = M->at<float>(gs.dy[1]);
    float* dqkv = M->at<float>(gs.dqkv);
    SKF_TRY(ffn_ln_bwd(M, w.ln2, w.f1, w.f2, G, M->at<float>(a.z2), M->at<float>(a.st2), M->at<float>(a.x1), M->at<float>(a.h), dy2,
                       M->at<float>(gs.dh), G2, Me, rate, site_enc(i, 1), s, hbits_of(M, a.hbits, Me), M->at<char>(a.img[1])));
    if (i == 0) SKF_TRY(M->sched.issue(M, s, M->ctx.last_ready));
    M->ctx.last_ready = nullptr;
    {
      hipEvent_t ready = nullptr;
      SKF_TRY(with_ready_event(M, i == 0, &ready, [&] {
        return ln_oproj_bwd(M, w.ln1, w.mha.o, G2, M->at<float>(a.z1), M->at<float>(a.st1), M->at<float>(a.o), G, dy1, dO, Me, rate,
                            site_enc(i, 0), s, M->at<char>(a.img_o));
      }));
      if (i == 0) SKF_TRY(M->sched.issue(M, s, ready));
    }
    const float* qkv = M->at<float>(a.qkv);
    SKF_TRY(M->sched.before_write(M, dqkv, s));
    SKF_TRY(skf_attention_bwd_ordered(qkv, 3 * d, qkv + d, 3 * d, qkv + 2 * d, 3 * d, M->at<float>(a.o), d, dO, d,
                                      M->at<float>(a.astats), emask, Le, 0, B, H, Le, Le, dh, dqkv, 3 * d, dqkv + d, 3 * d,
                                      dqkv + 2 * d, 3 * d, M->cfg.gemm_precision, nullptr, M->ctx.order, s));
    SKF_TRY(dense_wgrad(M, w.mha.qkv, M->at<float>(a.x_in), d, dqkv, 3 * d, Me, s));
    if (i == 0) SKF_TRY(M->sched.issue(M, s, nullptr, !M->sched.holding()));
    SKF_TRY(dense_dgrad(M, w.mha.qkv, dqkv, 3 * d, Me, G, d, 1, nullptr, 0, s));
    if (M->ctx.ffn_fused && i > 0) SKF_TRY(M->sched.hold(M, s));
    else SKF_TRY(M->sched.issue(M, s));
    if (!M->ctx.ffn_fused && M->sched.side && N >= 2 && i == N / 2) SKF_TRY(flush_wgrads(M, s, -1, false, !M->sched.holding()));
  }
  if (c.continuous) {
    SKF_TRY(skf_embed_continuous_bwd(M->at<float>(P.inp), Le, B, Le, G, d, M->G(L.enc_embd.w), M->G(L.enc_embd.b), rate,
                                     site_enc_embed(), M->state, M->at<char>(P.small_ws), P.small_ws_bytes, s));
  } else {
    if (P.emb_sort_bytes) {
      SKF_TRY(skf_embed_bwd_sorted(M->at<char>(P.emb_sort[0]), B, Le, G, c.vocab_size, d, M->G(L.enc_emb), rate, site_enc_embed(),
                                   M->state, s));
    } else {
      SKF_HIP(hipMemsetAsync(M->G(L.enc_emb), 0, (size_t)c.vocab_size * d * sizeof(float), s));
      SKF_TRY(skf_embed_bwd(inp, Le, B, Le, G, c.vocab_size, d, M->G(L.enc_emb), rate, site_enc_embed(), M->state, s));
    }
  }
  return flush_wgrads(M, s, M->n_buckets - 1, true);
}

int issue_embed_sorts(SkfModel* M, hipStream_t s) {
  const SkfConfig& c = M->cfg;
  const Layout& L = M->lay;
  const Plan& P = M->plan;
  if (!P.emb_sort_bytes) return SKF_OK;
  const int B = c.batch, Le = c.seq_len, Ld = c.seq_len - 1, d = c.d_model;
  hipStream_t ss = s;
  if (M->sched.side && do_recon(c)) {
    hipEvent_t staged = (M->inputs_staged && M->inputs_staged_valid && !g_capturing) ? M->inputs_staged : nullptr;
    if (!staged) {
      staged = M->sched.take_event();
      SKF_CHECK_ARG(staged, "event allocation failed");
      SKF_HIP(hipEventRecord(staged, s));
    }
    SKF_HIP(hipStreamWaitEvent(M->sched.side, staged, 0));
    ss = M->sched.side;
    hipEvent_t masks = M->sched.take_event(), ready = M->sched.take_event();
    SKF_CHECK_ARG(masks && ready, "event allocation failed");
    SKF_TRY(forward_preamble(M, true, false, ss, masks));
    SKF_HIP(hipEventRecord(ready, ss));
    M->ctx.masks_ready = masks; M->ctx.pre_ready = ready;
  }
  SKF_TRY(skf_embed_sort(M->at<long long>(P.inp), Le, B, Le, c.vocab_size, M->G(L.enc_emb), d, M->at<char>(P.emb_sort[0]),
                         P.emb_sort_bytes, ss));
  if (do_recon(c))
    SKF_TRY(skf_embed_sort(M->at<long long>(P.tar), Le, B, Ld, c.vocab_size, M->G(L.dec_emb), d, M->at<char>(P.emb_sort[1]),
                           P.emb_sort_bytes, ss));
  return build_row_lists(M, ss);
}
}
```

sketchformer_amd/csrc/skf_model_internal.h:

```cpp
#pragma once
#include <stdarg.h>
#include <stdlib.h>
#include <string.h>
#include <string>
#include <vector>
#include <map>
#include <algorithm>
#include "skf_common.h"
#include "skf_attention_params.h"
#include "skf_decode_fused.h"

namespace skf_model_detail {

struct DenseP { size_t w, b; int in, out, ld; };
struct LnP { size_t g, b; };
struct SelfMhaP { DenseP qkv, o; };
struct CrossMhaP { DenseP q, kv, o; };
struct EncLayerP { SelfMhaP mha; DenseP f1, f2; LnP ln1, ln2; };
struct DecLayerP { SelfMhaP mha1; CrossMhaP mha2; DenseP f1, f2; LnP ln1, ln2, ln3; };

inline bool has_bott(const SkfConfig& c) { return c.lowerdim > 0; }
inline bool has_cls(const SkfConfig& c) { return c.lowerdim > 0 && c.do_classification != 0; }
inline bool do_recon(const SkfConfig& c) { return c.do_reconstruction != 0; }

struct Layout {
  size_t total = 0;
  size_t enc_emb = 0, dec_emb = 0;
  DenseP enc_embd{}, dec_embd{};
  std::vector<EncLayerP> enc;
  std::vector<DecLayerP> dec;
  DenseP bott_w{};
  size_t bott_v = 0;
  DenseP bott_e{};
  std::vector<DenseP> cbuf;
  size_t dec_off = 0;
  int E = 0, Ua = 0;
  DenseP cls{}, out{};
  size_t exp_w = 0, exp_b = 0;
  std::vector<SkfParamEntry> entries;
};

struct Bump {
  size_t off = 0;
  size_t take(size_t bytes) { size_t o = off; off += (bytes + 255) & ~(size_t)255; return o; }
};

struct DecodeAreas {
  size_t pre = 0;
  std::vector<size_t> kv2;
  std::vector<size_t> cache;
  size_t img = 0;
  size_t mask = 0, flags = 0;
  size_t limit = 0;
  size_t dyn = 0;
  size_t anc = 0, cand = 0, beam = 0;
};

struct EncAct { size_t x_in, qkv, o, z1, st1, astats, x1, h, z2, st2, x2, hbits, img[2], img_o, img_qkv, img_of; };
struct DecAct { size_t x_in, qkv, o1, z1, st1, astats1, out1, q2, kv2, o2, astats2, z2, st2, out2, h, z3, st3, out3, hbits, img[2], img_o1, img_o2, img_qkv, img_o2f, img_o1f, img_q2, img_q2t; };

struct Plan {
  size_t bytes = 0;
  size_t inp, tar, labels, enc_mask, dec_mask;
  size_t order;
  std::vector<EncAct> enc;
  std::vector<DecAct> dec;
  size_t u, pool_a, emb, pooled, dpooled, cls_logits, cls_probs, pre, logits;
  std::vector<size_t> cb_h, cb_f;
  size_t dcb[2];
  size_t recon_loss, recon_hit, cls_loss, cls_hit, row_mask, cont_scal;
  size_t gA, gB, gC, dqkv, dh, do_, dpre, dkv2, dq2, demb;
  struct GradSet { size_t dy[3], dh, dq2, dkv2, dqkv; };
  std::vector<GradSet> gs;
  int n_gs = 2;
  size_t gemm_ws, gemm_ws_bytes, small_ws, small_ws_bytes;
  size_t emb_sort[2] = {0, 0}, emb_sort_bytes = 0;
  size_t slab_arena, slab_arena_bytes, descs, n_wgrads;
  size_t ln_part, ln_part_stride;
  size_t bott_part = 0;
  DecodeAreas dca;
  size_t dc_x[2], dc_q, dc_o, dc_z, dc_out1, dc_out2, dc_h, dc_logits, dc_stats, dc_kvnew;
  size_t live_len = 0, live16 = 0, live32 = 0;
};

struct Img16 { size_t w = 0, wt = 0; int in = 0, out = 0, ld_src = 0, ldw = 0, ldt = 0; size_t src = 0; };
struct Enc16 { size_t x_in, qkv, o, olo, z1, st1, astats, x1, h, z2, st2, x2, hbits; };
struct Dec16 { size_t x_in, qkv, o1, olo1, z1, st1, astats1, out1, q2, kv2, o2, olo2, astats2, z2, st2, out2, h, z3, st3, out3, hbits; };

struct Plan16 {
  size_t bytes = 0;
  size_t inp = 0, tar = 0, labels = 0, enc_mask = 0, dec_mask = 0;
  std::vector<Enc16> enc;
  std::vector<Dec16> dec;
  size_t u = 0, pool_a = 0, emb = 0, cls_logits = 0, cls_probs = 0, pre = 0, logits = 0;
  int ld_logits = 0;
  size_t recon_loss = 0, recon_hit = 0, cls_loss = 0, cls_hit = 0;
  size_t gA = 0, gB = 0, dy = 0, dqkv = 0, dh = 0, dO = 0, dpre = 0, dkv2 = 0, dq2 = 0, demb = 0;
  size_t slab = 0, slab_bytes = 0, small_ws = 0, small_ws_bytes = 0, attn_ws = 0, attn_ws_bytes = 0, ln_ws = 0, ln_ws_bytes = 0;
  size_t cast_descs = 0, cast_descs_bytes = 0; int cast_n = 0, cast_blocks = 0; const float* cast_for = nullptr;
  const char* tables_ws = nullptr;
  size_t ln_slabs = 0, ln_descs = 0; int ln_n = 0, ln_n_dec = 0, ln_blocks_dec = 0, ln_blocks_enc = 0, ln_cursor = 0; bool ln_batched = false;
  DecodeAreas dca;
  size_t order = 0;
  size_t live_len = 0, live1 = 0, live64 = 0;
  size_t emb_sort[2] = {0, 0}, emb_sort_bytes = 0;
  std::map<size_t, Img16> img;
};

struct ReduceBatch {
  std::vector<SkfReduceDesc> descs;
  bool descs_uploaded = false;
  size_t slab_cursor = 0, desc_cursor = 0, ln_cursor = 0;
  int reduce_blocks = 0;
  size_t phase_desc_begin = 0;
  bool side_used = false;

  void begin_step();
  void reset();
  int add(const SkfReduceDesc& d, int blocks);
  float* take_ln_partial(SkfModel* M);
  float* take_slab(SkfModel* M, size_t bytes, size_t queued);
  size_t begin() const { return phase_desc_begin; }
  size_t end() const { return desc_cursor; }
  int blocks() const { return reduce_blocks; }
  void end_phase(bool final);
};

struct SideSched {
  hipStream_t side = nullptr;
  hipEvent_t fork_event = nullptr, join_event = nullptr;
  std::vector<hipEvent_t> events;
  size_t next_event = 0;
  struct SideEvent { hipEvent_t e; long seq; };
  long side_seq = 0, side_waited = 0;
  std::map<const void*, SideEvent> pending_readers;
  std::map<const void*, SideEvent> pending_writers;
  struct Queued { DenseP w; const float* x; int ldx; const float* dy; int lddy; int rows; int kind = 0; float* dx = nullptr; int lddx = 0; int accumulate = 0; const int* blocks32 = nullptr; };
  std::vector<Queued> wq;
  std::vector<Queued> wq_held;

  int create(bool captured);
  void destroy();
  hipEvent_t take_event();
  void rewind_events() { next_event = 0; }
  void begin_backward() { wq.clear(); wq_held.clear(); pending_readers.clear(); pending_writers.clear(); rewind_events(); }
  void queue_wgrad(const DenseP& w, const float* x, int ldx, const float* dy, int lddy, int rows, const int* blocks32) { wq.push_back(Queued{w, x, ldx, dy, lddy, rows, 0, nullptr, 0, 0, blocks32}); }
  void queue_dgrad(const DenseP& w, const float* dy, int lddy, int rows, float* dx, int lddx, int accumulate) { wq.push_back(Queued{w, nullptr, 0, dy, lddy, rows, 1, dx, lddx, accumulate}); }
  bool holding() const { return !wq_held.empty(); }
  int hold(SkfModel* M, hipStream_t s);
  int issue(SkfModel* M, hipStream_t s, hipEvent_t ready_recorded = nullptr, bool on_main = false);
  int issue_held(SkfModel* M, hipStream_t s, hipEvent_t ready_recorded = nullptr);
  int before_write(SkfModel* M, const void* buf, hipStream_t s) { return wait_side(M, false, buf, s); }
  int before_read(SkfModel* M, const void* buf, hipStream_t s) { return wait_side(M, true, buf, s); }
  int wait_side(SkfModel* M, bool writers, const void* buf, hipStream_t s);
  int join(hipStream_t s);
  bool fork_into_capture(hipStream_t s) { return hipEventRecord(fork_event, s) == hipSuccess && hipStreamWaitEvent(side, fork_event, 0) == hipSuccess; }
  bool join_capture(hipStream_t s) { return hipEventRecord(join_event, side) == hipSuccess && hipStreamWaitEvent(s, join_event, 0) == hipSuccess; }
};

struct StepCtx {
  bool lists_set = false;
  int live_rows = 0;
  const int* live_len = nullptr;
  struct LiveList { int granule; const int* blocks; } lists[2] = {};
  const int* order = nullptr;
  hipEvent_t pre_ready = nullptr, masks_ready = nullptr;
  bool lists_built = false;
  bool masks_staged = false;
  bool ffn_fused = false;
  hipEvent_t last_ready = nullptr;

  void reset() { *this = StepCtx(); }
  void begin_backward() { clear_live(); last_ready = nullptr; }
  void set_live(int rows, const int* len, int g0, const int* b0, int g1, const int* b1) { lists_set = true; live_rows = rows; live_len = len; lists[0] = {g0, b0}; lists[1] = {g1, b1}; }
  void clear_live() { lists_set = false; live_rows = 0; live_len = nullptr; lists[0] = lists[1] = LiveList{}; }
  bool live(int rows) const { return lists_set && rows == live_rows; }
  const int* live_lengths(int rows) const { return live(rows) ? live_len : nullptr; }
  const int* live_blocks(int rows, int granule) const {
    return !live(rows) ? nullptr : lists[0].granule == granule ? lists[0].blocks : lists[1].granule == granule ? lists[1].blocks : nullptr;
  }
};

}

struct SkfModel {
  SkfConfig cfg;
  uint32_t flags = 0;
  bool no_ln_fuse = false, no_relu_bits = false;
  skf_model_detail::StepCtx ctx;
  skf_model_detail::Layout lay;
  skf_model_detail::Plan plan;
  skf_model_detail::Plan16 p16;
  bool bf16 = false;
  float *params = nullptr, *grads = nullptr, *m = nullptr, *v = nullptr, *metrics = nullptr;
  const float* pos = nullptr;
  char* ws = nullptr;
  void* state = nullptr;
  hipGraphExec_t g_fb = nullptr, g_opt = nullptr, g_dec = nullptr;
  long long dec_dyn_host[2] = {0, 0};
  std::vector<int> dec_stream_host;
  float g_opt_scale = 0.f;
  skf_model_detail::SideSched sched;
  hipEvent_t inputs_staged = nullptr;
  bool inputs_staged_valid = false;
  skf_model_detail::ReduceBatch red;
  hipEvent_t bucket_ready[2] = {nullptr, nullptr};
  int n_buckets = 1;

  struct Named { size_t off; int rows, cols, ld, bf16; };
  std::map<std::string, Named> named;
  void reg(const std::string& name, size_t off, size_t rows, size_t cols, size_t ld, int is_bf16) {
    named[name] = {off, (int)rows, (int)cols, (int)ld, is_bf16};
  }

  template <typename T> T* at(size_t off) const { return reinterpret_cast<T*>(ws + off); }
  float* P(size_t off) const { return params + off; }
  float* G(size_t off) const { return grads + off; }
};

#define SKF_TRY(call)            \
  do {                           \
    int rc__ = (call);           \
    if (rc__ != SKF_OK) return rc__; \
  } while (0)

namespace skf_model_detail {

extern thread_local int g_capturing;

inline unsigned site_enc_embed() { return 0; }
inline unsigned site_enc(int layer, int j) { return 1 + 2 * layer + j; }
inline unsigned site_dec_embed(int N) { return 1 + 2 * N; }
inline unsigned site_class(int N, int i) { return 2 + 5 * N + i; }
inline unsigned site_dec(int N, int layer, int j) { return 2 + 2 * N + 3 * layer + j; }

inline bool may_park(const SkfModel* M, bool needs_side = true) { return !g_capturing && (M->sched.side || !needs_side); }
template <typename F>
int with_tail_event(SkfModel* M, hipEvent_t e, bool* rode, F call, bool needs_side = true) {
  SkfTailScope scope(may_park(M, needs_side) ? e : nullptr);
  const int rc = call();
  *rode = scope.attached();
  return rc;
}

Layout build_layout(const SkfConfig& c);
bool decode_areas_ok(const DecodeAreas& A, size_t plan_bytes);
Plan build_plan(const SkfConfig& c);
Plan16 build_plan16(const SkfConfig& c, const Layout& L);

int dense_fwd(SkfModel* M, const DenseP& w, const float* x, int rows, float* y, int act, hipStream_t s);
int dense_ln_fwd(SkfModel* M, const DenseP& w, const float* a, int rows, const float* x, float* z, const LnP& ln, float* out,
                 float* stats, float rate, unsigned site, hipStream_t s);
void* hbits_of(SkfModel* M, size_t off, int rows);
int dense_fwd_relu_bits(SkfModel* M, const DenseP& w, const float* x, int rows, float* y, void* bits, hipStream_t s);
int dense_fwd_ld(SkfModel* M, const DenseP& w, const float* x, int ldx, int rows, float* y, int ldy, int act, hipStream_t s);
int dense_wgrad(SkfModel* M, const DenseP& w, const float* x, int ldx, const float* dy, int lddy, int rows, hipStream_t s);
int flush_wgrads(SkfModel* M, hipStream_t s, int bucket, bool final, bool issue_queued = true, hipEvent_t main_here = nullptr);
int dense_dgrad(SkfModel* M, const DenseP& w, const float* dy, int lddy, int rows, float* dx, int lddx, int accumulate,
                const float* relu_src, int ld_relu, hipStream_t s, const void* relu_bits = nullptr);
int dense_dgrad_deferred(SkfModel* M, const DenseP& w, const float* dy, int lddy, int rows, float* dx, int lddx, int accumulate,
                         hipStream_t s);

int classify_fwd(SkfModel* M, bool training, hipStream_t s);
int forward_preamble(SkfModel* M, bool with_backward, bool encoder_only, hipStream_t s, hipEvent_t masks_ready = nullptr);
int run_forward(SkfModel* M, bool training, bool with_loss, hipStream_t s, bool encoder_only = false);
int run_backward(SkfModel* M, hipStream_t s);
int issue_embed_sorts(SkfModel* M, hipStream_t s);

struct BeamOut { long long* tokens; float* scores; int* lengths; };
struct DecodeRequest {
  const float* embedding = nullptr;
  const int* expected_len_host = nullptr;
  int n_valid = 0;
// ... 19 lines not shown
```

sketchformer_amd/csrc/skf_model_sched.hip:

```cpp
#include "skf_model_internal.h"

namespace skf_model_detail {

int dense_fwd(SkfModel* M, const DenseP& w, const float* x, int rows, float* y, int act, hipStream_t s) {
  return skf_gemm_f32(1, 0, rows, w.out, w.in, x, w.in, M->P(w.w), w.ld, y, w.out, M->P(w.b), act, nullptr, 0, 0, 1,
                      nullptr, 0, nullptr, 0, M->cfg.gemm_precision, s);
}
int dense_ln_fwd(SkfModel* M, const DenseP& w, const float* a, int rows, const float* x, float* z, const LnP& ln, float* out,
                 float* stats, float rate, unsigned site, hipStream_t s) {
  if (!M->no_ln_fuse && skf_gemm_ln_residual_supported(rows, w.out, w.in, M->cfg.gemm_precision)) {
    const int rc = skf_gemm_ln_residual_f32(rows, w.out, w.in, a, w.in, M->P(w.w), w.ld, M->P(w.b), x, M->P(ln.g), M->P(ln.b), z, out, stats,
                                            rate, site, M->state, M->cfg.gemm_precision, s);
    if (rc != SKF_EUNSUPPORTED) return rc;
    M->no_ln_fuse = true;
  }
  SKF_TRY(dense_fwd(M, w, a, rows, z, 0, s));
  return skf_layernorm_residual_fwd(x, z, M->P(ln.g), M->P(ln.b), out, stats, rows, w.out, rate, site, M->state, s);
}
void* hbits_of(SkfModel* M, size_t off, int rows) {
  if (M->ctx.ffn_fused) return M->at<char>(off);
  if (M->no_relu_bits || !skf_gemm_relu_bits_bytes(rows, M->cfg.dff, M->cfg.d_model, M->cfg.gemm_precision)) return nullptr;
  return M->at<char>(off);
}
int dense_fwd_relu_bits(SkfModel* M, const DenseP& w, const float* x, int rows, float* y, void* bits, hipStream_t s) {
// ... 63 lines not shown
  if (!wq_held.empty()) SKF_TRY(issue(M, s));
  wq_held.swap(wq);
  return SKF_OK;
}
int SideSched::issue(SkfModel* M, hipStream_t s, hipEvent_t ready_recorded, bool on_main) {
  SkfTailScope shield(nullptr);
  SKF_TRY(issue_held(M, s));
  if (wq.empty()) return SKF_OK;
  std::vector<Queued> group;
  group.swap(wq);
  hipStream_t ws = on_main ? s : side;
  hipEvent_t ready = nullptr, done = nullptr;
  if (!on_main) {
    ready = ready_recorded ? ready_recorded : take_event(); done = take_event();
    SKF_CHECK_ARG(ready && done, "event allocation failed");
    if (!ready_recorded) SKF_HIP(hipEventRecord(ready, s));
    SKF_HIP(hipStreamWaitEvent(side, ready, 0));
  }
  hipEvent_t dgrad_done = nullptr;
  for (const auto& q : group) {
    if (q.kind != 1) continue;
    const DenseP& w = q.w;
    SKF_TRY(skf_gemm_f32(1, 1, q.rows, w.in, w.out, q.dy, q.lddy, M->P(w.w), w.ld, q.dx, q.lddx, nullptr, 0, nullptr, 0,
                         q.accumulate, 1, nullptr, 0, nullptr, 0, M->cfg.gemm_precision, ws));
    if (!dgrad_done && !on_main) { dgrad_done = take_event(); SKF_CHECK_ARG(dgrad_done, "event allocation failed"); }
  }
  long dgrad_seq = 0;
  if (dgrad_done) { SKF_HIP(hipEventRecord(dgrad_done, side)); dgrad_seq = ++side_seq; }
  std::vector<SkfWgradProblem> probs;
  std::vector<const Queued*> prob_q;
  for (const auto& q : group) {
    const DenseP& w = q.w;
    if (q.kind == 1) continue;
    if ((double)w.in * w.out * q.rows <= 33554432.0) {
      SKF_TRY(dense_wgrad_on(M, w, q.x, q.ldx, q.dy, q.lddy, q.rows, ws));
      continue;
    }
    const int splits = skf_gemm_default_splits(w.in, w.out, q.rows);
    const size_t bytes = (skf_gemm_workspace_bytes(w.in, w.out, q.rows, splits, 1) + 255) & ~(size_t)255;
    SkfWgradProblem pr{};
    pr.A = q.x; pr.B = q.dy; pr.slab = M->red.take_slab(M, bytes, probs.size()); pr.slab_bytes = bytes;
    if (!pr.slab) return SKF_EINVAL;
    pr.row_blocks = q.blocks32; pr.row_block_rows = 32;
    pr.M = w.in; pr.N = w.out; pr.K = q.rows; pr.lda = q.ldx; pr.ldb = q.lddy; pr.splits = splits; pr.with_bias_grad = 1;
    probs.push_back(pr); prob_q.push_back(&q);
  }
  bool small = true;
  for (const auto& pr : probs) small = small && 2.0 * pr.M * pr.N * pr.K < 4e9;
  const size_t gmax = small ? 8 : 1;
  for (size_t b0 = 0; b0 < probs.size(); b0 += gmax) {
    const int nb = (int)std::min<size_t>(gmax, probs.size() - b0);
    SKF_TRY(skf_gemm_wgrad_partial_group(probs.data() + b0, nb, M->cfg.gemm_precision, ws));
  }
  for (size_t i = 0; i < probs.size(); ++i) {
    const DenseP& w = prob_q[i]->w;
    SkfReduceDesc d;
    d.slab = probs[i].slab; d.C = M->G(w.w); d.bias_grad = M->G(w.b); d.splits = probs[i].splits_used; d.M = w.in; d.N = w.out; d.ldc = w.ld;
    d.block_begin = M->red.blocks(); d.pad = 0;
    SKF_TRY(M->red.add(d, skf_splitk_reduce_blocks(w.in, w.out)));
  }
  M->red.side_used = true;
  if (on_main) return SKF_OK;
  SKF_HIP(hipEventRecord(done, side));
  const long done_seq = ++side_seq;
  for (const auto& q : group) {
    pending_readers[q.dy] = SideEvent{done, done_seq};
    if (q.x) pending_readers[q.x] = SideEvent{done, done_seq};
    if (q.kind == 1) pending_writers[q.dx] = SideEvent{dgrad_done, dgrad_seq};
  }
  return SKF_OK;
}
int SideSched::join(hipStream_t s) {
  hipEvent_t e = take_event();
  SKF_CHECK_ARG(e, "event allocation failed");
  SKF_HIP(hipEventRecord(e, side));
  SKF_HIP(hipStreamWaitEvent(s, e, 0));
  pending_readers.clear();
  pending_writers.clear();
  side_waited = side_seq;
  return SKF_OK;
}
int dense_wgrad(SkfModel* M, const DenseP& w, const float* x, int ldx, const float* dy, int lddy, int rows, hipStream_t s) {
  if (!M->sched.side) return dense_wgrad_on(M, w, x, ldx, dy, lddy, rows, s);
  M->sched.queue_wgrad(w, x, ldx, dy, lddy, rows, M->ctx.live_blocks(rows, 32));
  return SKF_OK;
}
int flush_wgrads(SkfModel* M, hipStream_t s, int bucket, bool final, bool issue_queued, hipEvent_t main_here) {
  if (issue_queued) SKF_TRY(M->sched.issue(M, s));
  const size_t begin = M->red.begin(), end = M->red.end();
  hipStream_t ready_on = s;
  bool bucket_recorded = false;
  hipStream_t side = M->sched.side;
  if (side && M->red.side_used && end > begin) {
    if (!M->red.descs_uploaded) {
      SKF_HIP(hipMemcpy(M->at<SkfReduceDesc>(M->plan.descs) + begin, M->red.descs.data() + begin,
                        (end - begin) * sizeof(SkfReduceDesc), hipMemcpyHostToDevice));
      if (final) M->red.descs_uploaded = true;
    }
    if (final) {
      SKF_TRY(M->sched.join(s));
      SKF_TRY(with_tail_event(M, bucket >= 0 ? M->bucket_ready[bucket] : nullptr, &bucket_recorded, [&] {
        return skf_splitk_reduce_batch(M->at<SkfReduceDesc>(M->plan.descs) + begin, (int)(end - begin), M->red.blocks(), s);
      }));
    } else {
      hipEvent_t em = main_here ? main_here : M->sched.take_event();
      SKF_CHECK_ARG(em, "event allocation failed");
      if (!main_here) SKF_HIP(hipEventRecord(em, s));
      SKF_HIP(hipStreamWaitEvent(side, em, 0));
      SKF_TRY(skf_splitk_reduce_batch(M->at<SkfReduceDesc>(M->plan.descs) + begin, (int)(end - begin), M->red.blocks(), side));
      ready_on = side;
    }
  }
  if (bucket >= 0 && M->bucket_ready[bucket] && !bucket_recorded) SKF_HIP(hipEventRecord(M->bucket_ready[bucket], ready_on));
  M->red.end_phase(final);
  return SKF_OK;
}
int dense_dgrad(SkfModel* M, const DenseP& w, const float* dy, int lddy, int rows, float* dx, int lddx, int accumulate,
                const float* relu_src, int ld_relu, hipStream_t s, const void* relu_bits) {
  SKF_TRY(M->sched.before_write(M, dx, s));
  const int* blocks = M->ctx.live_blocks(rows, 16);
  if (relu_bits)
    return skf_gemm_f32_bits(1, 1, rows, w.in, w.out, dy, lddy, M->P(w.w), w.ld, dx, lddx, nullptr, 0, nullptr, 0,
                             accumulate, 1, nullptr, 0, nullptr, 0, M->cfg.gemm_precision, blocks, 16, nullptr, relu_bits, s);
  return skf_gemm_f32_rows(1, 1, rows, w.in, w.out, dy, lddy, M->P(w.w), w.ld, dx, lddx, nullptr, 0, relu_src, ld_relu,
                           accumulate, 1, nullptr, 0, nullptr, 0, M->cfg.gemm_precision, blocks, 16, s);
}

int dense_dgrad_deferred(SkfModel* M, const DenseP& w, const float* dy, int lddy, int rows, float* dx, int lddx, int accumulate,
                         hipStream_t s) {
  if (!M->sched.side) return dense_dgrad(M, w, dy, lddy, rows, dx, lddx, accumulate, nullptr, 0, s);
  M->sched.queue_dgrad(w, dy, lddy, rows, dx, lddx, accumulate);
  return SKF_OK;
}

void ReduceBatch::begin_step() {
  side_used = false;
  slab_cursor = 0; desc_cursor = 0; reduce_blocks = 0; phase_desc_begin = 0; ln_cursor = 0;
}
void ReduceBatch::reset() {
  descs.clear(); descs_uploaded = false;
  slab_cursor = 0; desc_cursor = 0; ln_cursor = 0; reduce_blocks = 0; phase_desc_begin = 0;
}
int ReduceBatch::add(const SkfReduceDesc& d, int blocks) {
  if (!descs_uploaded) descs.push_back(d);
  else {
    const SkfReduceDesc& o = descs[desc_cursor];
    SKF_CHECK_ARG(o.slab == d.slab && o.C == d.C && o.splits == d.splits && o.block_begin == d.block_begin, "wgrad sequence changed between steps");
  }
  reduce_blocks += blocks;
  desc_cursor += 1;
  side_used = true;
  return SKF_OK;
}
float* ReduceBatch::take_ln_partial(SkfModel* M) {
  const Plan& P = M->plan;
  if (!(ln_cursor < 5 * (size_t)M->cfg.num_layers && desc_cursor < P.n_wgrads)) {
    skf_set_error("%s: LayerNorm partial arena exhausted", __func__);
    return nullptr;
  }
  return M->at<float>(P.ln_part + ln_cursor * P.ln_part_stride);
}
float* ReduceBatch::take_slab(SkfModel* M, size_t bytes, size_t queued) {
  if (!(slab_cursor + bytes <= M->plan.slab_arena_bytes && desc_cursor + queued < M->plan.n_wgrads)) {
    skf_set_error("%s: slab arena exhausted", __func__);
    return nullptr;
  }
  float* slab = M->at<float>(M->plan.slab_arena + slab_cursor);
  slab_cursor += bytes;
  return slab;
}
void ReduceBatch::end_phase(bool final) {
  phase_desc_begin = desc_cursor;
  reduce_blocks = 0;
  if (final) side_used = false;
}
}
```

sketchformer_amd/ops.py:

```python
import ctypes as C

import torch

from . import _lib


def _stream():
    return C.c_void_p(torch.cuda.current_stream().cuda_stream)


def _p(t):
    if t is None:
        return None
    if not t.is_cuda:
        raise _lib.SkfError("sketchformer_amd ops need CUDA(HIP) tensors; got a CPU tensor (no CPU fallback)")
    return C.c_void_p(t.data_ptr())


def _prec(precision):
    return _lib.default_precision() if precision is None else int(precision)


def _f32(t, name):
    if t.dtype != torch.float32:
# ... 187 lines not shown
    V, d = table.shape
    out = torch.empty(B, L, d, dtype=torch.float32, device=table.device)
    _lib.call("skf_embed_fwd", _p(tokens), ld, B, L, _p(table), V, d, _p(pos), _p(out), rate, site, _p(state), _stream())
    return out


def embed_bwd(tokens, dx, vocab, L=None, rate=0.0, site=0, state=None):
    B, ld = tokens.shape
    L = L or ld
    d = dx.shape[-1]
    dtable = torch.zeros(vocab, d, dtype=torch.float32, device=dx.device)
    _lib.call("skf_embed_bwd", _p(tokens), ld, B, L, _p(dx), vocab, d, _p(dtable), rate, site, _p(state), _stream())
    return dtable


def embed_bwd_sorted(tokens, dx, vocab, L=None, rate=0.0, site=0, state=None, prefill=None):
    B, ld = tokens.shape
    L = L or ld
    d = dx.shape[-1]
    dtable = torch.full((vocab, d), float("nan") if prefill is None else prefill, dtype=torch.float32, device=dx.device)
    nbytes = _lib.load().skf_embed_sort_workspace_bytes(B, L, vocab)
    ws = torch.empty((nbytes + 3) // 4, dtype=torch.int32, device=dx.device)
    _lib.call("skf_embed_sort", _p(tokens), ld, B, L, vocab, _p(dtable), d, _p(ws), nbytes, _stream())
    _lib.call("skf_embed_bwd_sorted", _p(ws), B, L, _p(dx), vocab, d, _p(dtable), rate, site, _p(state), _stream())
    return dtable


def layernorm_residual_fwd(x, y, gamma, beta, rate=0.0, site=0, state=None):
    d = x.shape[-1]
    rows = x.numel() // d
    z = y.clone()
    out = torch.empty_like(x)
    stats = torch.empty(rows, 2, dtype=torch.float32, device=x.device)
    _lib.call("skf_layernorm_residual_fwd", _p(x), _p(z), _p(gamma), _p(beta), _p(out), _p(stats), rows, d, rate, site,
              _p(state), _stream())
    return out, z, stats


def gemm_ln_residual(a, w, bias, x, gamma, beta, rate=0.0, site=0, state=None, precision=None):
    _f32(a, "a"); _f32(w, "w"); _f32(x, "x")
    M, K = a.shape
    N = w.shape[1]
    z = torch.empty(M, N, dtype=torch.float32, device=a.device)
    out = torch.empty_like(z)
    stats = torch.empty(M, 2, dtype=torch.float32, device=a.device)
    _lib.call("skf_gemm_ln_residual_f32", M, N, K, _p(a), a.stride(0), _p(w), w.stride(0), _p(bias), _p(x), _p(gamma), _p(beta),
              _p(z), _p(out), _p(stats), rate, site, _p(state), _prec(precision), _stream())
    return out, z, stats


def ffn_fused_supported(M, d, dff, precision=None):
    return bool(_lib.load().skf_ffn_fused_supported(M, d, dff, _prec(precision)))


def ffn_weight_images(pairs, transpose, precision=None):
    n = len(pairs)
    d, dff = pairs[0][0].shape
    nbytes = _lib.load().skf_ffn_image_bytes(d, dff, _prec(precision))
    if not nbytes:
        raise _lib.SkfError("no fused feed-forward path for d=%d dff=%d" % (d, dff))
    imgs = [torch.empty(nbytes, dtype=torch.uint8, device=pairs[0][0].device) for _ in range(n)]
    PA = C.c_void_p * n
    IA = C.c_int * n
    for w1, w2 in pairs:
        _f32(w1, "W1"); _f32(w2, "W2")
    _lib.call("skf_ffn_weight_images", n, PA(*[w1.data_ptr() for w1, _ in pairs]), IA(*[w1.stride(0) for w1, _ in pairs]),
              PA(*[w2.data_ptr() for _, w2 in pairs]), IA(*[w2.stride(0) for _, w2 in pairs]), IA(*([int(bool(transpose))] * n)),
              PA(*[im.data_ptr() for im in imgs]), d, dff, _prec(precision), _stream())
    return imgs


def ffn_fused_fwd(x, image, b1, b2, gamma, beta, dff, rate=0.0, site=0, state=None, precision=None, proj=None):
    _f32(x, "x")
    M, d = x.shape
    h = torch.empty(M, dff, dtype=torch.float32, device=x.device)
    nb = _lib.load().skf_ffn_relu_bits_bytes(M, d, dff, _prec(precision))
    bits = torch.zeros(max(nb // 8, 1), dtype=torch.int64, device=x.device)
    z = torch.empty_like(x)
    out = torch.empty_like(x)
    stats = torch.empty(M, 2, dtype=torch.float32, device=x.device)
    if proj is not None:
        pimg, pbias = proj
        po = torch.empty(M, pbias.numel(), dtype=torch.float32, device=x.device)
        _lib.call("skf_ffn_fused_fwd_proj_f32", M, d, dff, _p(x), _p(image), _p(b1), _p(b2), _p(h), _p(bits), _p(gamma), _p(beta),
                  _p(z), _p(out), _p(stats), rate, site, _p(state), _p(pimg), _p(pbias), pbias.numel(), _p(po), _prec(precision), _stream())
        return out, z, stats, h, bits, po
    _lib.call("skf_ffn_fused_fwd_f32", M, d, dff, _p(x), _p(image), _p(b1), _p(b2), _p(h), _p(bits), _p(gamma), _p(beta),
              _p(z), _p(out), _p(stats), rate, site, _p(state), _prec(precision), _stream())
    return out, z, stats, h, bits


def ffn_block_fwd(a, residual, pre, image, b1, b2, gamma, beta, dff, rate=0.0, pre_site=0, site=0, state=None, precision=None, proj=None):
    _f32(a, "a")
    M, d = a.shape
    dev = a.device
    e = lambda *sh: torch.empty(*sh, dtype=torch.float32, device=dev)
    r = {"h": e(M, dff), "z": e(M, d), "out": e(M, d), "stats": e(M, 2), "z1": e(M, d), "x1": e(M, d), "stats1": e(M, 2)}
    nb = _lib.load().skf_ffn_relu_bits_bytes(M, d, dff, _prec(precision))
    r["bits"] = torch.zeros(max(nb // 8, 1), dtype=torch.int64, device=dev)
    pimg, pbias, pg, pb = pre
    P = lambda t: t.data_ptr() if t is not None else None
    blk = _lib.SkfFfnBlockFwd(struct_size=C.sizeof(_lib.SkfFfnBlockFwd), M=M, d=d, dff=dff, precision=_prec(precision), x=P(a), image=P(image),
                              b1=P(b1), b2=P(b2), h=P(r["h"]), relu_bits_out=P(r["bits"]), gamma=P(gamma), beta=P(beta), z=P(r["z"]),
                              out=P(r["out"]), stats=P(r["stats"]), rate=rate, site=site, step_state=P(state), pre_image=P(pimg),
                              pre_bias=P(pbias), pre_residual=P(residual), pre_gamma=P(pg), pre_beta=P(pb), pre_z=P(r["z1"]), pre_out=P(r["x1"]),
                              pre_stats=P(r["stats1"]), pre_site=pre_site)
    if proj is not None:
        r["proj_out"] = e(M, proj[1].numel())
        blk.proj_image, blk.proj_bias, blk.proj_out, blk.proj_n = P(proj[0]), P(proj[1]), P(r["proj_out"]), proj[1].numel()
    _lib.call("skf_ffn_block_fwd_f32", C.byref(blk), _stream())
    return r


def attn_tail_proj(a, residual, pre, proj, rate=0.0, pre_site=0, state=None, precision=None):
    _f32(a, "a")
    M, d = a.shape
    e = lambda *sh: torch.empty(*sh, dtype=torch.float32, device=a.device)
    r = {"z1": e(M, d), "x1": e(M, d), "stats1": e(M, 2), "proj_out": e(M, proj[1].numel())}
    pimg, pbias, pg, pb = pre
    P = lambda t: t.data_ptr() if t is not None else None
    blk = _lib.SkfFfnBlockFwd(struct_size=C.sizeof(_lib.SkfFfnBlockFwd), M=M, d=d, dff=4 * d, precision=_prec(precision), x=P(a), rate=rate,
                              step_state=P(state), pre_image=P(pimg), pre_bias=P(pbias), pre_residual=P(residual), pre_gamma=P(pg), pre_beta=P(pb),
                              pre_z=P(r["z1"]), pre_out=P(r["x1"]), pre_stats=P(r["stats1"]), pre_site=pre_site, proj_image=P(proj[0]),
                              proj_bias=P(proj[1]), proj_out=P(r["proj_out"]), proj_n=proj[1].numel())
    _lib.call("skf_ffn_block_fwd_f32", C.byref(blk), _stream())
    return r


def ffn_fused_bwd(dy, image_t, bits, dff, dx=None, row_blocks=None, precision=None):
    _f32(dy, "dy")
    M, d = dy.shape
    dh = torch.empty(M, dff, dtype=torch.float32, device=dy.device)
    acc = dx is not None
    if dx is None:
        dx = torch.empty_like(dy)
    _lib.call("skf_ffn_fused_bwd_f32", M, d, dff, _p(dy), _p(image_t), _p(bits), _p(dh), _p(dx), int(acc), _p(row_blocks),
              16 if row_blocks is not None else 0, _prec(precision), _stream())
    return dh, dx


def ffn_fused_bwd_ln(dout, z, stats, gamma, image_t, bits, dff, rate=0.0, site=0, state=None, row_blocks=None, precision=None):
    _f32(dout, "dout")
    M, d = dout.shape
    lib = _lib.load()
    n = lib.skf_ffn_fused_ln_partials(M)
    part = torch.empty(n, 2, d, dtype=torch.float32, device=dout.device)
    dy, dx = torch.empty_like(dout), torch.empty_like(dout)
    dh = torch.empty(M, dff, dtype=torch.float32, device=dout.device)
    _lib.call("skf_ffn_fused_bwd_ln_f32", M, d, dff, _p(dout), _p(z), _p(stats), _p(gamma), rate, site, _p(state), _p(image_t), _p(bits),
              _p(dy), _p(dh), _p(dx), _p(part), part.numel() * 4, _p(row_blocks), 16 if row_blocks is not None else 0, _prec(precision),
              _stream())
    g = part.sum(0)
    return dy, dh, dx, g[0], g[1]


def dense_weight_image(w, transpose, precision=None):
    _f32(w, "w")
    K, N = (w.shape[1], w.shape[0]) if transpose else (w.shape[0], w.shape[1])
    nbytes = _lib.load().skf_dense_image_bytes(K, N, _prec(precision))
    if not nbytes:
        raise _lib.SkfError("no operand image for K=%d N=%d" % (K, N))
    img = torch.empty(nbytes, dtype=torch.uint8, device=w.device)
    PA, IA = C.c_void_p * 1, C.c_int * 1
    _lib.call("skf_dense_weight_images", 1, PA(w.data_ptr()), IA(w.stride(0)), IA(int(bool(transpose))), IA(K), IA(N), PA(img.data_ptr()),
              _prec(precision), _stream())
    return img


def layernorm_bwd_dgrad(dout, z, stats, gamma, image_t, rate=0.0, site=0, state=None, row_blocks=None, precision=None, lead=None):
    _f32(dout, "dout")
    M, d = dout.shape
    n = _lib.load().skf_layernorm_bwd_dgrad_partials(M)
    part = torch.empty(n, 2, d, dtype=torch.float32, device=dout.device)
    dz, dy, da = torch.empty_like(dout), torch.empty_like(dout), torch.empty_like(dout)
    la, li = lead if lead is not None else (None, None)
    _lib.call("skf_layernorm_bwd_dgrad_lead_f32", M, d, _p(dout), _p(la), _p(li), _p(z), _p(stats), _p(gamma), rate, site, _p(state), _p(image_t),
              _p(dz), _p(dy), _p(da), _p(part), part.numel() * 4, _p(row_blocks), 16 if row_blocks is not None else 0, _prec(precision), _stream())
    g = part.sum(0)
    return dz, dy, da, g[0], g[1]


def layernorm_residual_bwd(dout, z, stats, gamma, rate=0.0, site=0, state=None):
    d = dout.shape[-1]
    rows = dout.numel() // d
    dz = torch.empty_like(dout)
    dy = torch.empty_like(dout) if rate > 0 else None
    dg = torch.empty(d, dtype=torch.float32, device=dout.device)
    db = torch.empty(d, dtype=torch.float32, device=dout.device)
    wsb = _lib.load().skf_layernorm_bwd_workspace_bytes(rows, d)
    ws = _ws(wsb, dout.device)
    _lib.call("skf_layernorm_residual_bwd", _p(dout), _p(z), _p(stats), _p(gamma), _p(dz), _p(dy), _p(dg), _p(db), rows,
              d, rate, site, _p(state), _p(ws), wsb, _stream())
    return dz, (dy if dy is not None else dz), dg, db


def softmax_ce(logits, target, tgt_cols, tgt_off=0, mask_pad=False, scale=1.0, want_probs=False, write_grad=True):
    rows, ncls = logits.shape
    row_loss = torch.empty(rows, dtype=torch.float32, device=logits.device)
    row_hit = torch.empty(rows, dtype=torch.float32, device=logits.device)
    probs = torch.empty(rows, ncls, dtype=torch.float32, device=logits.device) if want_probs else None
    _lib.call("skf_softmax_ce", _p(logits), logits.stride(0), rows, ncls, _p(target), target.stride(0), tgt_cols, tgt_off,
              int(mask_pad), scale, _p(row_loss), _p(row_hit), _p(probs), int(write_grad), _stream())
    return row_loss, row_hit, probs


def pool_fwd(u, Vw, x):
    B, L, U = u.shape
    d = x.shape[-1]
    a = torch.empty(B, L, dtype=torch.float32, device=x.device)
    emb = torch.empty(B, d, dtype=torch.float32, device=x.device)
    _lib.call("skf_pool_fwd", _p(u), _p(Vw), _p(x), B, L, U, d, _p(a), _p(emb), _stream())
    return a, emb


def pool_bwd(u, Vw, x, a, demb):
    B, L, U = u.shape
    d = x.shape[-1]
    dpre = u.clone()
    dx = torch.empty_like(x)
    dV = torch.empty(U, dtype=torch.float32, device=x.device)
    ws = _ws(B * U * 4, x.device)
    _lib.call("skf_pool_bwd", _p(dpre), _p(Vw), _p(x), _p(a), _p(demb), B, L, U, d, _p(dx), _p(dV), _p(ws), B * U * 4,
              _stream())
    return dpre, dx, dV


def expander_fwd(emb, w, bias):
    B, d = emb.shape
    L = w.numel()
    pre = torch.empty(B, L, d, dtype=torch.float32, device=emb.device)
    _lib.call("skf_expander_fwd", _p(emb), _p(w), _p(bias), B, L, d, _p(pre), _stream())
    return pre


def expander_bwd(dpre, emb, w):
    B, L, d = dpre.shape
    demb = torch.empty(B, d, dtype=torch.float32, device=emb.device)
    dw = torch.empty(L, dtype=torch.float32, device=emb.device)
    db = torch.empty(L, dtype=torch.float32, device=emb.device)
    ws = _ws(2 * B * L * 4, emb.device)
    _lib.call("skf_expander_bwd", _p(dpre), _p(emb), _p(w), B, L, d, _p(demb), 0, _p(dw), _p(db), _p(ws), 2 * B * L * 4,
              _stream())
    return demb, dw, db


def adam_step(w, g, m, v, state, grad_scale=1.0, beta1=0.9, beta2=0.98, eps=1e-9):
    _lib.call("skf_adam_step", _p(w), _p(g), _p(m), _p(v), w.numel(), _p(state), grad_scale, beta1, beta2, eps, _stream())


def dropout(x, rate, site=0, state=None):
    if rate <= 0.0 or state is None:
        return x
    _f32(x, "x")
    y = torch.empty_like(x)
    _lib.call("skf_dropout", _p(x), _p(y), x.numel(), float(rate), int(site), _p(state), _stream())
    return y


def embed_continuous_fwd(x, W, bias, pos, L=None, rate=0.0, site=0, state=None):
    _f32(x, "x")
    B, ld = x.shape[0], x.shape[1]
    L = L or ld
    d = W.shape[1]
    out = torch.empty(B, L, d, dtype=torch.float32, device=x.device)
    _lib.call("skf_embed_continuous_fwd", _p(x), ld, B, L, _p(W), _p(bias), d, _p(pos), _p(out), float(rate), int(site), _p(state), _stream())
    return out


def dropout_keep_mask(drop_key, site, rate, n):
    import numpy as np
    out = np.empty(n, dtype=np.uint8)
    _lib.call("skf_dropout_keep_mask", drop_key, site, rate, n, out.ctypes.data_as(C.c_void_p))
    return out.astype(bool)


def sample_uniform(seed, stream_id, step):
    return float(_lib.load().skf_sample_uniform(int(seed) & 0xffffffff, int(stream_id) & 0xffffffff, int(step) & 0xffffffff))


def sample_tokens(logits, temperature, top_k, top_p, seed, stream_ids, step):
    _f32(logits, "logits")
    if logits.dim() != 2:
        raise ValueError("logits must be (B, V)")
    _p(logits)
    B, V = logits.shape
    dev = logits.device
    step = int(step)
    if step < 0:
        raise ValueError("step must be >= 0")
    if not torch.is_tensor(stream_ids):
        stream_ids = torch.tensor([int(v) for v in stream_ids], dtype=torch.int32)
    stream_ids = stream_ids.to(device=dev, dtype=torch.int32).contiguous()
    if stream_ids.shape != (B,):
        raise ValueError("stream_ids must hold one integer per row")
    smp = _lib.SkfSampling(temperature=float(temperature), top_k=int(top_k), top_p=float(top_p), seed=int(seed) & 0xffffffff)
    tokens = torch.zeros(B, step + 2, dtype=torch.int64, device=dev)
    mask = torch.zeros(B, step + 2, dtype=torch.uint8, device=dev)
    flags = torch.zeros(B + 1, dtype=torch.int32, device=dev)
    _lib.call("skf_decode_sample_tokens", _p(logits), logits.stride(0), B, V, B, step, -1, _p(tokens), step + 2, _p(mask), step + 2,
              _p(flags), C.c_void_p(flags.data_ptr() + 4 * B), None, None, C.byref(smp), _p(stream_ids), _stream())
    return tokens[:, step + 1].clone()


def beam_step(cand_logp, cand_tok, scores, finished, anc, step, eos, lengths=None):
    _f32(cand_logp, "cand_logp")
    _f32(scores, "scores")
# ... 469 lines not shown
```

Baseline: 7.390 million stroke-tokens/sec.

## Fuse attention-tail LayerNorm backward and output-projection dgrad into FFN backward kernel

Extends the fused FFN backward kernel with a TAIL variant. The same kernel now also computes the preceding attention block's LayerNorm backward (with dropout mask), stores dz/dy, and runs the attention output-projection dgrad GEMM on the tile it already holds in registers and LDS. This replaces a separate ln_oproj_bwd launch in both encoder and decoder layers, saving one kernel launch and a global round trip of the intermediate gradient per layer. In exchange it uses more shared memory and more registers per block, which may lower occupancy, and it adds complexity to how the LayerNorm partial arena is allocated.

```diff
diff --git a/include/skf.h b/include/skf.h
--- a/include/skf.h
+++ b/include/skf.h
@@ -85,6 +85,13 @@
                              float rate, unsigned site, const void* step_state, const void* image_t, const void* relu_bits_in,
                              float* dy, float* dh, float* dx, float* ln_partials, size_t ln_partials_bytes,
                              const int* row_blocks, int row_block_rows, int precision, skf_stream_t stream);
+int skf_ffn_fused_bwd_ln_tail_f32(int M, int d, int dff, const float* dout, const float* z, const float* stats, const float* gamma,
+                                  float rate, unsigned site, const void* step_state, const void* image_t, const void* relu_bits_in,
+                                  float* dy, float* dh, float* ln_partials, size_t ln_partials_bytes,
+                                  const float* tail_z, const float* tail_stats, const float* tail_gamma, float tail_rate,
+                                  unsigned tail_site, const void* tail_image_t, float* tail_dz, float* tail_dy, float* tail_da,
+                                  float* tail_partials, size_t tail_partials_bytes, const int* row_blocks, int row_block_rows,
+                                  int precision, skf_stream_t stream);
 size_t skf_dense_image_bytes(int K, int N, int precision);
 int skf_dense_weight_images(int n, const float* const* src, const int* ld, const int* transpose, const int* K, const int* N,
                             void* const* images, int precision, skf_stream_t stream);
diff --git a/sketchformer_amd/_lib.py b/sketchformer_amd/_lib.py
--- a/sketchformer_amd/_lib.py
+++ b/sketchformer_amd/_lib.py
@@ -125,6 +125,8 @@
     "skf_ffn_fused_bwd_f32": (_I, [_I, _I, _I, _P, _P, _P, _P, _P, _I, _P, _I, _I, _P]),
     "skf_ffn_fused_ln_partials": (_I, [_I]),
     "skf_ffn_fused_bwd_ln_f32": (_I, [_I, _I, _I, _P, _P, _P, _P, _F, _U, _P, _P, _P, _P, _P, _P, _P, _Z, _P, _I, _I, _P]),
+    "skf_ffn_fused_bwd_ln_tail_f32": (_I, [_I, _I, _I, _P, _P, _P, _P, _F, _U, _P, _P, _P, _P, _P, _P, _Z, _P, _P, _P, _F, _U, _P, _P, _P, _P, _P, _Z,
+                                           _P, _I, _I, _P]),
     "skf_dense_image_bytes": (_Z, [_I, _I, _I]),
     "skf_dense_weight_images": (_I, [_I, _P, _P, _P, _P, _P, _P, _I, _P]),
     "skf_layernorm_bwd_dgrad_supported": (_I, [_I, _I, _I]),
diff --git a/sketchformer_amd/csrc/skf_ffn_fused.h b/sketchformer_amd/csrc/skf_ffn_fused.h
--- a/sketchformer_amd/csrc/skf_ffn_fused.h
+++ b/sketchformer_amd/csrc/skf_ffn_fused.h
@@ -21,6 +21,10 @@
   const float* ln_dout; const float* ln_z; const float* ln_stats;
   float* ln_dy;
   float* ln_part;
+  const float* tail_z; const float* tail_stats; const float* tail_gamma; float tail_rate; unsigned tail_site;
+  const char* tail_img;
+  float* tail_dz; float* tail_dy; float* tail_da;
+  float* tail_part;
 };
 
 int skf_ffn_fused_launch(const FfnFusedParams& p, int pieces, int direction, hipStream_t st);
diff --git a/sketchformer_amd/csrc/skf_ffn_fused.hip b/sketchformer_amd/csrc/skf_ffn_fused.hip
--- a/sketchformer_amd/csrc/skf_ffn_fused.hip
+++ b/sketchformer_amd/csrc/skf_ffn_fused.hip
@@ -131,8 +131,9 @@
   return v + __shfl_xor(v, 16, 64);
 }
 
-template <int P, int MODE, bool LNB, bool POST, bool PRE, bool NOFFN>
+template <int P, int MODE, bool LNB, bool POST, bool PRE, bool NOFFN, bool TAIL>
 __device__ __forceinline__ void ffn_fused_body(const FfnFusedParams& p) {
+  static_assert(!TAIL || (MODE == 1 && LNB), "attention-tail backward: behind the LayerNorm-backward prologue only");
   static_assert(!LNB || MODE == 1, "LayerNorm-backward prologue: backward only");
   static_assert(!POST || MODE == 0, "chained projection: forward only");
   static_assert(!PRE || MODE == 0, "leading projection + LayerNorm: forward only");
@@ -175,6 +176,7 @@
     const float* src = which == 0 ? p.pre_bias : which == 1 ? p.pre_gamma : p.pre_beta;
     *reinterpret_cast<f32x4*>(PREs + which * FD + c4) = *reinterpret_cast<const f32x4*>(src + c4);
   }
+  if (TAIL && tid < FD / 4) *reinterpret_cast<f32x4*>(B1s + 4 * tid) = *reinterpret_cast<const f32x4*>(p.tail_gamma + 4 * tid);
   const float* bias1_p = B1s + 16 * wave + 4 * g;
   const f32x4 bias2_r = MODE == 0 && !NOFFN ? *reinterpret_cast<const f32x4*>(p.bias2 + 16 * wave + 4 * g) : (f32x4){0.f, 0.f, 0.f, 0.f};
 
@@ -196,6 +198,13 @@
     }
   }
   f32x4 ln_dg = (f32x4){0.f, 0.f, 0.f, 0.f}, ln_db = ln_dg;
+  float* TLs = PREs + 3 * FD;
+  if constexpr (TAIL) {
+    if (lane < 32) {
+      *reinterpret_cast<f32x4*>(TLs + (wave * 2 + 0) * FD + 4 * lane) = (f32x4){0.f, 0.f, 0.f, 0.f};
+      *reinterpret_cast<f32x4*>(TLs + (wave * 2 + 1) * FD + 4 * lane) = (f32x4){0.f, 0.f, 0.f, 0.f};
+    }
+  }
 
   const __amdgpu_buffer_rsrc_t r_H = __builtin_amdgcn_make_buffer_rsrc(p.H, 0, p.M * (FF * 4), 0x00020000);
   const __amdgpu_buffer_rsrc_t r_A = __builtin_amdgcn_make_buffer_rsrc(const_cast<float*>(LNB ? p.ln_dout : p.A), 0, p.M * p.lda * 4, 0x00020000);
@@ -447,6 +456,21 @@
       request_rows(tn, xn);
     }
     if constexpr (POST) load_frags<P>(w2, r_img3, lane16, wave * (NKS * P * 1024));
+    const unsigned tail_bytes = TAIL ? (unsigned)p.M * (FD * 4) : 0u;
+    const __amdgpu_buffer_rsrc_t r_TDZ = __builtin_amdgcn_make_buffer_rsrc(TAIL ? p.tail_dz : p.H, 0, tail_bytes, 0x00020000);
+    const __amdgpu_buffer_rsrc_t r_TDY = __builtin_amdgcn_make_buffer_rsrc(TAIL ? p.tail_dy : p.H, 0, tail_bytes, 0x00020000);
+    const __amdgpu_buffer_rsrc_t r_TDA = __builtin_amdgcn_make_buffer_rsrc(TAIL ? p.tail_da : p.H, 0, tail_bytes, 0x00020000);
+    float tl_inv_keep = 1.f;
+    uint32_t tl_thresh = 0u, tl_sk = 0u;
+    if constexpr (TAIL) {
+      if (p.tail_rate > 0.f) {
+        typedef const __attribute__((address_space(4))) uint32_t* const_u32p;
+        tl_sk = skf_site_key(*(const_u32p)&reinterpret_cast<const SkfStepState*>(p.state)->drop_key, p.tail_site);
+        tl_thresh = skf_drop_thresh(p.tail_rate);
+        tl_inv_keep = 1.0f / (1.0f - p.tail_rate);
+      }
+      load_frags<P>(w2, __builtin_amdgcn_make_buffer_rsrc(const_cast<char*>(p.tail_img), 0, P * FD * FD * 2, 0x00020000), lane16, wave * (NKS * P * 1024));
+    }
     if constexpr (!NOFFN) {
 #pragma unroll
     for (int rt = 0; rt < NRT; ++rt) *reinterpret_cast<f32x4*>(Yt + (rt * TR + i) * YPITCH + 16 * wave + 4 * g) = y[rt];
@@ -455,6 +479,18 @@
 #pragma unroll
       for (int rt = 0; rt < NRT; ++rt)
         xres[rt] = __builtin_bit_cast(f32x4, __builtin_amdgcn_raw_buffer_load_b128(r_R, tl[rt] < ntiles ? st_voff + (unsigned)tl[rt] * (unsigned)(TR * (PRE ? FD : p.lda) * 4) : OOB, 0, 0));
+    }
+    f32x4 tl_dg = (f32x4){0.f, 0.f, 0.f, 0.f}, tl_db = tl_dg;
+    f32x4 tz[TAIL ? NRT : 1];
+    u32x2 ts[TAIL ? NRT : 1];
+    if constexpr (TAIL) {
+      const __amdgpu_buffer_rsrc_t r_TZ = __builtin_amdgcn_make_buffer_rsrc(const_cast<float*>(p.tail_z), 0, tail_bytes, 0x00020000);
+      const __amdgpu_buffer_rsrc_t r_TS = __builtin_amdgcn_make_buffer_rsrc(const_cast<float*>(p.tail_stats), 0, p.M * 8, 0x00020000);
+#pragma unroll
+      for (int rt = 0; rt < NRT; ++rt) {
+        tz[rt] = __builtin_bit_cast(f32x4, __builtin_amdgcn_raw_buffer_load_b128(r_TZ, tl[rt] < ntiles ? st_voff + (unsigned)tl[rt] * (unsigned)(TR * FD * 4) : OOB, 0, 0));
+        ts[rt] = __builtin_amdgcn_raw_buffer_load_b64(r_TS, tl[rt] < ntiles ? (unsigned)(tl[rt] * TR + st_row) * 8u : OOB, 0, 0);
+      }
     }
     __syncthreads();
 #pragma unroll
@@ -466,6 +502,29 @@
       const f32x4 yv = *reinterpret_cast<const f32x4*>(Yt + rloc * YPITCH + 4 * e_sub);
       if constexpr (MODE == 0) {
         ln_row(rt, yv, xres[rt], sk, gm, bt, p.C, p.out, p.stats, POST);
+      } else if constexpr (TAIL) {
+        typedef float f32x2_t __attribute__((ext_vector_type(2)));
+        const f32x2_t ms = __builtin_bit_cast(f32x2_t, ts[rt]);
+        const f32x4 gm2 = *reinterpret_cast<const f32x4*>(B1s + 4 * e_sub);
+        const f32x4 dv = yv + dzr[rt];
+        const f32x4 xh = (tz[rt] - ms[0]) * ms[1], gg = dv * gm2;
+        tl_dg += dv * xh; tl_db += dv;
+        const float s1 = ffn_half_wave_sum((gg[0] + gg[1]) + (gg[2] + gg[3])) * (1.0f / FD);
+        const float s2 = ffn_half_wave_sum((gg[0] * xh[0] + gg[1] * xh[1]) + (gg[2] * xh[2] + gg[3] * xh[3])) * (1.0f / FD);
+        const f32x4 gz = ms[1] * (gg - s1 - xh * s2);
+        f32x4 gy = gz;
+        const unsigned voff = tl[rt] < ntiles ? st_voff + (unsigned)tl[rt] * (unsigned)(TR * FD * 4) : OOB;
+        if (p.tail_rate > 0.f) {
+#pragma unroll
+          for (int e = 0; e < 4; ++e) gy[e] = gz[e] * (skf_keep(tl_sk, (voff >> 2) + e, tl_thresh) ? tl_inv_keep : 0.f);
+        }
+        __builtin_amdgcn_raw_buffer_store_b128(__builtin_bit_cast(u32x4, gz), r_TDZ, voff, 0, 0);
+        __builtin_amdgcn_raw_buffer_store_b128(__builtin_bit_cast(u32x4, gy), r_TDY, voff, 0, 0);
+        unsigned lo[P], hi[P];
+        skf_split2<P>(gy[0], gy[1], lo, sel);
+        skf_split2<P>(gy[2], gy[3], hi, sel);
+#pragma unroll
+        for (int q = 0; q < P; ++q) *reinterpret_cast<u32x2*>(Xp + q * PLANE + rt * TILE + st_off) = (u32x2){lo[q], hi[q]};
       } else {
         if (ok) {
           f32x4 v = yv;
@@ -475,6 +534,34 @@
         }
       }
     }
+    if constexpr (TAIL) {
+#pragma unroll
+      for (int e = 0; e < 4; ++e) { tl_dg[e] += __shfl_xor(tl_dg[e], 32, 64); tl_db[e] += __shfl_xor(tl_db[e], 32, 64); }
+      if (lane < 32) {
+        *reinterpret_cast<f32x4*>(TLs + (wave * 2 + 0) * FD + 4 * lane) += tl_dg;
+        *reinterpret_cast<f32x4*>(TLs + (wave * 2 + 1) * FD + 4 * lane) += tl_db;
+      }
+    }
+    }
+    if constexpr (TAIL) {
+      const unsigned c_voff = (unsigned)(i * FD + 16 * wave + 4 * g) * 4u;
+      __syncthreads();
+      load_half<P>(Xp, a_off, fr.f[0], 0);
+#pragma unroll
+      for (int t = 0; t < NRT; ++t) {
+        if (t < nrt) {
+          load_half<P>(Xp + t * TILE, a_off, fr.f[1], 1);
+          f32x4 acc0 = (f32x4){0.f, 0.f, 0.f, 0.f}, acc1 = acc0;
+          int c = 0;
+          half_products<P>(w2, fr.f[0], 0, acc0, acc1, c);
+          if (t + 1 < NRT) load_half<P>(Xp + (t + 1) * TILE, a_off, fr.f[0], 0);
+          half_products<P>(w2, fr.f[1], 1, acc0, acc1, c);
+          const f32x4 r = acc0 + acc1;
+          __builtin_amdgcn_raw_buffer_store_b128(__builtin_bit_cast(u32x4, r), r_TDA, c_voff + (unsigned)tl[t] * (TR * FD * 4), 0, 0);
+          __builtin_amdgcn_sched_barrier(0);
+        }
+      }
+      __syncthreads();
     }
     if constexpr (POST) {
       const int nb2 = p.n2 >> 7;
@@ -524,8 +611,14 @@
       if (LNB || !p.accumulate) {
         const int row = tile * TR + (tid >> 5);
         if (row < p.M) {
-          *reinterpret_cast<f32x4*>(p.C + (size_t)row * FD + 4 * (tid & 31)) = zero;
-          if constexpr (LNB) *reinterpret_cast<f32x4*>(p.ln_dy + (size_t)row * FD + 4 * (tid & 31)) = zero;
+          const size_t off = (size_t)row * FD + 4 * (tid & 31);
+          if constexpr (!TAIL) *reinterpret_cast<f32x4*>(p.C + off) = zero;
+          if constexpr (LNB) *reinterpret_cast<f32x4*>(p.ln_dy + off) = zero;
+          if constexpr (TAIL) {
+            *reinterpret_cast<f32x4*>(p.tail_dz + off) = zero;
+            *reinterpret_cast<f32x4*>(p.tail_dy + off) = zero;
+            *reinterpret_cast<f32x4*>(p.tail_da + off) = zero;
+          }
         }
       }
     }
@@ -545,14 +638,20 @@
 #pragma unroll
       for (int k = 1; k < 8; ++k) t += red[k * 2 * FD + tid];
       p.ln_part[(size_t)wg * 2 * FD + tid] = t;
-    }
-  }
-}
-
-template <int P, int MODE, bool LNB = false, bool POST = false, bool PRE = false>
-__global__ __launch_bounds__(512, 2) void ffn_fused_kernel(FfnFusedParams p) { ffn_fused_body<P, MODE, LNB, POST, PRE, false>(p); }
+    } else if (TAIL) {
+      const float* red2 = TLs - 2 * FD;
+      float t = red2[tid];
+#pragma unroll
+      for (int k = 1; k < 8; ++k) t += red2[k * 2 * FD + tid];
+      p.tail_part[(size_t)wg * 2 * FD + (tid - 2 * FD)] = t;
+    }
+  }
+}
+
+template <int P, int MODE, bool LNB = false, bool POST = false, bool PRE = false, bool TAIL = false>
+__global__ __launch_bounds__(512, 2) void ffn_fused_kernel(FfnFusedParams p) { ffn_fused_body<P, MODE, LNB, POST, PRE, false, TAIL>(p); }
 template <int P>
-__global__ __launch_bounds__(512, 2) void attn_tail_proj_kernel(FfnFusedParams p) { ffn_fused_body<P, 0, false, true, true, true>(p); }
+__global__ __launch_bounds__(512, 2) void attn_tail_proj_kernel(FfnFusedParams p) { ffn_fused_body<P, 0, false, true, true, true, false>(p); }
 
 struct LnDgradParams {
   const float* dout; const float* z; const float* stats; const float* gamma;
@@ -766,18 +865,19 @@
   return g > ntiles ? ntiles : g;
 }
 
-template <int P, int MODE, bool LNB = false, bool POST = false, bool PRE = false>
+template <int P, int MODE, bool LNB = false, bool POST = false, bool PRE = false, bool TAIL = false>
 int launch_ffn(const FfnFusedParams& p, hipStream_t st) {
   const int grid = ffn_grid(p.M);
-  const size_t smem = (size_t)3 * P * PLANE + (P * PLANE >= ROWS * YPITCH * 4 ? 0 : ROWS * YPITCH * 4) + (FF + 384 + 3 * FD) * sizeof(float);
-  SKF_HIP(hipFuncSetAttribute(reinterpret_cast<const void*>(&ffn_fused_kernel<P, MODE, LNB, POST, PRE>), hipFuncAttributeMaxDynamicSharedMemorySize, (int)smem));
+  const size_t smem = (size_t)3 * P * PLANE + (P * PLANE >= ROWS * YPITCH * 4 ? 0 : ROWS * YPITCH * 4) + (FF + 384 + 3 * FD + (TAIL ? 16 * FD : 0)) * sizeof(float);
+  SKF_HIP(hipFuncSetAttribute(reinterpret_cast<const void*>(&ffn_fused_kernel<P, MODE, LNB, POST, PRE, TAIL>), hipFuncAttributeMaxDynamicSharedMemorySize, (int)smem));
   static const std::string tag = "ffn_fused<d128,dff512,bf16x" + std::to_string(P * (P + 1) / 2) + ">";
   const double live = skf_prof_list_fraction(p.row_blocks);
-  const double flops = 2.0 * 2.0 * p.M * FD * FF + (POST ? 2.0 * p.M * FD * p.n2 : 0.0) + (PRE ? 2.0 * p.M * FD * FD : 0.0);
-  const double bytes = 4.0 * ((double)p.M * FD * (MODE == 0 ? 4 : 3) + (double)p.M * FF + (POST ? (double)p.M * p.n2 : 0.0) + (PRE ? 4.0 * p.M * FD : 0.0)) + 2.0 * image_bytes(P) / 2;
+  const double flops = 2.0 * 2.0 * p.M * FD * FF + (POST ? 2.0 * p.M * FD * p.n2 : 0.0) + (PRE || TAIL ? 2.0 * p.M * FD * FD : 0.0);
+  const double bytes = 4.0 * ((double)p.M * FD * (MODE == 0 ? 4 : 3) + (double)p.M * FF + (POST ? (double)p.M * p.n2 : 0.0) + (PRE ? 4.0 * p.M * FD : 0.0) +
+                              (TAIL ? 3.0 * p.M * FD : 0.0)) + 2.0 * image_bytes(P) / 2 + (TAIL ? 2.0 * P * FD * FD : 0.0);
   SkfProfScope ps(st, tag.c_str(), flops, bytes);
   ps.done(flops * live, bytes * live);
-  SKF_LAUNCH_TAIL((ffn_fused_kernel<P, MODE, LNB, POST, PRE>), dim3(grid), dim3(512), smem, st, p);
+  SKF_LAUNCH_TAIL((ffn_fused_kernel<P, MODE, LNB, POST, PRE, TAIL>), dim3(grid), dim3(512), smem, st, p);
   SKF_LAUNCH_CHECK();
   return SKF_OK;
 }
@@ -801,6 +901,7 @@
 
 int skf_ffn_fused_launch(const FfnFusedParams& p, int pieces, int direction, hipStream_t st) {
   if (direction == 0 && p.pre_img && p.img3 && !p.img1) return pieces == 2 ? launch_tail_proj<2>(p, st) : launch_tail_proj<3>(p, st);
+  if (direction == 1 && p.ln_dout && p.tail_img) return pieces == 2 ? launch_ffn<2, 1, true, false, false, true>(p, st) : launch_ffn<3, 1, true, false, false, true>(p, st);
   if (direction == 1 && p.ln_dout) return pieces == 2 ? launch_ffn<2, 1, true>(p, st) : launch_ffn<3, 1, true>(p, st);
   if (direction == 0 && p.pre_img && p.img3) return pieces == 2 ? launch_ffn<2, 0, false, true, true>(p, st) : launch_ffn<3, 0, false, true, true>(p, st);
   if (direction == 0 && p.pre_img) return pieces == 2 ? launch_ffn<2, 0, false, false, true>(p, st) : launch_ffn<3, 0, false, false, true>(p, st);
@@ -923,6 +1024,39 @@
   p.C = dx; p.accumulate = 0; p.row_blocks = row_blocks;
   p.gamma = gamma; p.rate = rate; p.site = site; p.state = step_state;
   p.ln_dout = dout; p.ln_z = z; p.ln_stats = stats; p.ln_dy = dy; p.ln_part = ln_partials;
+  return skf_ffn_fused_launch(p, P, 1, (hipStream_t)stream);
+}
+
+extern "C" int skf_ffn_fused_bwd_ln_tail_f32(int M, int d, int dff, const float* dout, const float* z, const float* stats, const float* gamma,
+                                             float rate, unsigned site, const void* step_state, const void* image_t, const void* relu_bits_in,
+                                             float* dy, float* dh, float* ln_partials, size_t ln_partials_bytes,
+                                             const float* tail_z, const float* tail_stats, const float* tail_gamma, float tail_rate,
+                                             unsigned tail_site, const void* tail_image_t, float* tail_dz, float* tail_dy, float* tail_da,
+                                             float* tail_partials, size_t tail_partials_bytes, const int* row_blocks, int row_block_rows,
+                                             int precision, skf_stream_t stream) {
+  const int rc = ffn_common_checks(M, d, dff, precision, dout, image_t, dh, dy);
+  if (rc != SKF_OK) return rc;
+  SKF_CHECK_ARG(z && stats && gamma && ln_partials, "null LayerNorm operand");
+  SKF_CHECK_ARG((((uintptr_t)z | (uintptr_t)gamma | (uintptr_t)ln_partials) & 15) == 0 && ((uintptr_t)stats & 7) == 0, "operands must be 16-byte aligned");
+  SKF_CHECK_ARG(tail_z && tail_stats && tail_gamma && tail_image_t && tail_dz && tail_dy && tail_da && tail_partials, "null attention-tail operand");
+  SKF_CHECK_ARG((((uintptr_t)tail_z | (uintptr_t)tail_gamma | (uintptr_t)tail_image_t | (uintptr_t)tail_dz | (uintptr_t)tail_dy | (uintptr_t)tail_da |
+                  (uintptr_t)tail_partials) & 15) == 0 && ((uintptr_t)tail_stats & 7) == 0, "attention-tail operands must be 16-byte aligned");
+  SKF_CHECK_ARG(relu_bits_in && ((uintptr_t)relu_bits_in & 7) == 0, "the backward needs the sign bits the forward wrote");
+  SKF_CHECK_ARG(rate >= 0.f && rate < 1.f && tail_rate >= 0.f && tail_rate < 1.f && ((rate == 0.f && tail_rate == 0.f) || step_state),
+                "dropout needs 0 <= rate < 1 and the step state");
+  SKF_CHECK_ARG(!row_blocks || row_block_rows == TR, "row-block lists of this kernel have 16-row blocks");
+  const size_t need = (size_t)ffn_grid(M) * 2 * FD * sizeof(float);
+  SKF_CHECK_ARG(ln_partials_bytes >= need && tail_partials_bytes >= need, "partial buffer too small (skf_ffn_fused_ln_partials(M) x 2 x d floats each)");
+  const int P = precision == SKF_PREC_BF16X3 ? 2 : 3;
+  FfnFusedParams p{};
+  p.A = dout; p.lda = d; p.M = M;
+  p.img1 = (const char*)image_t; p.img2 = (const char*)image_t + image_bytes(P) / 2;
+  p.H = dh; p.bits_in = (const unsigned long long*)relu_bits_in;
+  p.accumulate = 0; p.row_blocks = row_blocks;
+  p.gamma = gamma; p.rate = rate; p.site = site; p.state = step_state;
+  p.ln_dout = dout; p.ln_z = z; p.ln_stats = stats; p.ln_dy = dy; p.ln_part = ln_partials;
+  p.tail_z = tail_z; p.tail_stats = tail_stats; p.tail_gamma = tail_gamma; p.tail_rate = tail_rate; p.tail_site = tail_site;
+  p.tail_img = (const char*)tail_image_t; p.tail_dz = tail_dz; p.tail_dy = tail_dy; p.tail_da = tail_da; p.tail_part = tail_partials;
   return skf_ffn_fused_launch(p, P, 1, (hipStream_t)stream);
 }
 
diff --git a/sketchformer_amd/csrc/skf_model_bwd.hip b/sketchformer_amd/csrc/skf_model_bwd.hip
--- a/sketchformer_amd/csrc/skf_model_bwd.hip
+++ b/sketchformer_amd/csrc/skf_model_bwd.hip
@@ -128,6 +128,38 @@
                                            pbytes, blocks, blocks ? 16 : 0, M->cfg.gemm_precision, s));
   SKF_TRY(ln_partials_desc(M, ln, part, skf_layernorm_bwd_dgrad_partials(rows)));
   return dense_wgrad(M, o, a_in, d, dy, d, rows, s);
+}
+
+bool ffn_attn_tail_fused(const SkfModel* M, const LnP& ln, const LnP& tln, const DenseP& o, int rows) {
+  const size_t pbytes = (size_t)skf_ffn_fused_ln_partials(rows) * 2 * M->cfg.d_model * sizeof(float);
+  return row_owner_takes_ln(M, ln, pbytes) && row_owner_takes_ln(M, tln, pbytes, rows, &o);
+}
+int ffn_attn_tail_bwd(SkfModel* M, const LnP& ln, const DenseP& f1, const DenseP& f2, const float* dout, const float* z, const float* st,
+                      const float* x_in, const float* h, float* dy, float* dh, int rows, float rate, unsigned site, hipStream_t s,
+                      const void* hbits, const void* image_t, const LnP& tln, const DenseP& o, const float* tz, const float* tst,
+                      const float* a_in, float* tdz, float* tdy, float* da, unsigned tsite, const void* timage_t) {
+  const int d = M->cfg.d_model;
+  M->ctx.last_ready = nullptr;
+  const int splits = skf_ffn_fused_ln_partials(rows);
+  const size_t pbytes = (size_t)splits * 2 * d * sizeof(float);
+  float* part = M->red.take_ln_partial(M);
+  float* tpart = M->red.take_ln_partial(M, 1);
+  if (!part || !tpart) return SKF_EINVAL;
+  for (const float* w : {dy, dh, tdz, tdy, da}) SKF_TRY(M->sched.before_write(M, w, s));
+  const int* blocks = M->ctx.live_blocks(rows, 16);
+  hipEvent_t ready = nullptr;
+  SKF_TRY(with_ready_event(M, M->sched.holding(), &ready, [&] {
+    return skf_ffn_fused_bwd_ln_tail_f32(rows, d, M->cfg.dff, dout, z, st, M->P(ln.g), rate, site, M->state, image_t, hbits, dy, dh, part, pbytes,
+                                         tz, tst, M->P(tln.g), rate, tsite, timage_t, tdz, tdy, da, tpart, pbytes, blocks, blocks ? 16 : 0,
+                                         M->cfg.gemm_precision, s);
+  }));
+  SKF_TRY(ln_partials_desc(M, ln, part, splits));
+  SKF_TRY(ln_partials_desc(M, tln, tpart, splits));
+  M->ctx.last_ready = ready;
+  SKF_TRY(M->sched.issue_held(M, s, ready));
+  SKF_TRY(dense_wgrad(M, f2, h, f2.in, dy, f2.out, rows, s));
+  SKF_TRY(dense_wgrad(M, f1, x_in, f1.in, dh, f1.out, rows, s));
+  return dense_wgrad(M, o, a_in, d, tdy, d, rows, s);
 }
 
 int build_row_lists(SkfModel* M, hipStream_t s) {
@@ -187,10 +219,17 @@
     const Plan::GradSet& gs = P.gs[layer_no % P.n_gs];
     float* dy3 = M->at<float>(gs.dy[0]); float* dy2 = M->at<float>(gs.dy[1]); float* dy1 = M->at<float>(gs.dy[2]);
     float* dqkv = M->at<float>(gs.dqkv); float* dkv2 = M->at<float>(gs.dkv2); float* dq2 = M->at<float>(gs.dq2);
-    SKF_TRY(ffn_ln_bwd(M, w.ln3, w.f1, w.f2, G, M->at<float>(a.z3), M->at<float>(a.st3), M->at<float>(a.out2), M->at<float>(a.h), dy3,
-                       M->at<float>(gs.dh), G2, Md, rate, site_dec(N, i, 2), s, hbits_of(M, a.hbits, Md), M->at<char>(a.img[1])));
-    SKF_TRY(ln_oproj_bwd(M, w.ln2, w.mha2.o, G2, M->at<float>(a.z2), M->at<float>(a.st2), M->at<float>(a.o2), G, dy2, dO, Md, rate,
-                         site_dec(N, i, 1), s, M->at<char>(a.img_o2)));
+    if (ffn_attn_tail_fused(M, w.ln3, w.ln2, w.mha2.o, Md)) {
+      SKF_TRY(ffn_attn_tail_bwd(M, w.ln3, w.f1, w.f2, G, M->at<float>(a.z3), M->at<float>(a.st3), M->at<float>(a.out2), M->at<float>(a.h), dy3,
+                                M->at<float>(gs.dh), Md, rate, site_dec(N, i, 2), s, hbits_of(M, a.hbits, Md), M->at<char>(a.img[1]), w.ln2,
+                                w.mha2.o, M->at<float>(a.z2), M->at<float>(a.st2), M->at<float>(a.o2), G, dy2, dO, site_dec(N, i, 1),
+                                M->at<char>(a.img_o2)));
+    } else {
+      SKF_TRY(ffn_ln_bwd(M, w.ln3, w.f1, w.f2, G, M->at<float>(a.z3), M->at<float>(a.st3), M->at<float>(a.out2), M->at<float>(a.h), dy3,
+                         M->at<float>(gs.dh), G2, Md, rate, site_dec(N, i, 2), s, hbits_of(M, a.hbits, Md), M->at<char>(a.img[1])));
+      SKF_TRY(ln_oproj_bwd(M, w.ln2, w.mha2.o, G2, M->at<float>(a.z2), M->at<float>(a.st2), M->at<float>(a.o2), G, dy2, dO, Md, rate,
+                           site_dec(N, i, 1), s, M->at<char>(a.img_o2)));
+    }
     const float* kv2 = M->at<float>(a.kv2);
     SKF_TRY(M->sched.before_write(M, dq2, s));
     SKF_TRY(M->sched.before_write(M, dkv2, s));
@@ -305,6 +344,14 @@
     const Plan::GradSet& gs = P.gs[layer_no % P.n_gs];
     float* dy2 = M->at<float>(gs.dy[0]); float* dy1 = M->at<float>(gs.dy[1]);
     float* dqkv = M->at<float>(gs.dqkv);
+    const bool tail = ffn_attn_tail_fused(M, w.ln2, w.ln1, w.mha.o, Me);
+    if (tail) {
+      SKF_TRY(ffn_attn_tail_bwd(M, w.ln2, w.f1, w.f2, G, M->at<float>(a.z2), M->at<float>(a.st2), M->at<float>(a.x1), M->at<float>(a.h), dy2,
+                                M->at<float>(gs.dh), Me, rate, site_enc(i, 1), s, hbits_of(M, a.hbits, Me), M->at<char>(a.img[1]), w.ln1, w.mha.o,
+                                M->at<float>(a.z1), M->at<float>(a.st1), M->at<float>(a.o), G, dy1, dO, site_enc(i, 0), M->at<char>(a.img_o)));
+      if (i == 0) SKF_TRY(M->sched.issue(M, s, M->ctx.last_ready));
+      M->ctx.last_ready = nullptr;
+    } else {
     SKF_TRY(ffn_ln_bwd(M, w.ln2, w.f1, w.f2, G, M->at<float>(a.z2), M->at<float>(a.st2), M->at<float>(a.x1), M->at<float>(a.h), dy2,
                        M->at<float>(gs.dh), G2, Me, rate, site_enc(i, 1), s, hbits_of(M, a.hbits, Me), M->at<char>(a.img[1])));
     if (i == 0) SKF_TRY(M->sched.issue(M, s, M->ctx.last_ready));
@@ -316,6 +363,7 @@
                             site_enc(i, 0), s, M->at<char>(a.img_o));
       }));
       if (i == 0) SKF_TRY(M->sched.issue(M, s, ready));
+    }
     }
     const float* qkv = M->at<float>(a.qkv);
     SKF_TRY(M->sched.before_write(M, dqkv, s));
diff --git a/sketchformer_amd/csrc/skf_model_internal.h b/sketchformer_amd/csrc/skf_model_internal.h
--- a/sketchformer_amd/csrc/skf_model_internal.h
+++ b/sketchformer_amd/csrc/skf_model_internal.h
@@ -118,7 +118,7 @@
   void begin_step();
   void reset();
   int add(const SkfReduceDesc& d, int blocks);
-  float* take_ln_partial(SkfModel* M);
+  float* take_ln_partial(SkfModel* M, size_t ahead = 0);
   float* take_slab(SkfModel* M, size_t bytes, size_t queued);
   size_t begin() const { return phase_desc_begin; }
   size_t end() const { return desc_cursor; }
diff --git a/sketchformer_amd/csrc/skf_model_sched.hip b/sketchformer_amd/csrc/skf_model_sched.hip
--- a/sketchformer_amd/csrc/skf_model_sched.hip
+++ b/sketchformer_amd/csrc/skf_model_sched.hip
@@ -239,13 +239,13 @@
   side_used = true;
   return SKF_OK;
 }
-float* ReduceBatch::take_ln_partial(SkfModel* M) {
+float* ReduceBatch::take_ln_partial(SkfModel* M, size_t ahead) {
   const Plan& P = M->plan;
-  if (!(ln_cursor < 5 * (size_t)M->cfg.num_layers && desc_cursor < P.n_wgrads)) {
+  if (!(ln_cursor + ahead < 5 * (size_t)M->cfg.num_layers && desc_cursor + ahead < P.n_wgrads)) {
     skf_set_error("%s: LayerNorm partial arena exhausted", __func__);
     return nullptr;
   }
-  return M->at<float>(P.ln_part + ln_cursor * P.ln_part_stride);
+  return M->at<float>(P.ln_part + (ln_cursor + ahead) * P.ln_part_stride);
 }
 float* ReduceBatch::take_slab(SkfModel* M, size_t bytes, size_t queued) {
   if (!(slab_cursor + bytes <= M->plan.slab_arena_bytes && desc_cursor + queued < M->plan.n_wgrads)) {
diff --git a/sketchformer_amd/ops.py b/sketchformer_amd/ops.py
--- a/sketchformer_amd/ops.py
+++ b/sketchformer_amd/ops.py
@@ -363,6 +363,22 @@
               _stream())
     g = part.sum(0)
     return dy, dh, dx, g[0], g[1]
+
+
+def ffn_fused_bwd_ln_tail(dout, z, stats, gamma, image_t, bits, dff, tail_z, tail_stats, tail_gamma, tail_image_t, rate=0.0, site=0,
+                          tail_rate=0.0, tail_site=0, state=None, row_blocks=None, precision=None):
+    _f32(dout, "dout")
+    M, d = dout.shape
+    n = _lib.load().skf_ffn_fused_ln_partials(M)
+    part = torch.empty(2, n, 2, d, dtype=torch.float32, device=dout.device)
+    dy, dz1, dy1, da = (torch.empty_like(dout) for _ in range(4))
+    dh = torch.empty(M, dff, dtype=torch.float32, device=dout.device)
+    _lib.call("skf_ffn_fused_bwd_ln_tail_f32", M, d, dff, _p(dout), _p(z), _p(stats), _p(gamma), rate, site, _p(state), _p(image_t), _p(bits),
+              _p(dy), _p(dh), _p(part[0]), part[0].numel() * 4, _p(tail_z), _p(tail_stats), _p(tail_gamma), tail_rate, tail_site,
+              _p(tail_image_t), _p(dz1), _p(dy1), _p(da), _p(part[1]), part[1].numel() * 4, _p(row_blocks),
+              16 if row_blocks is not None else 0, _prec(precision), _stream())
+    g = part.sum(1)
+    return dy, dh, g[0, 0], g[0, 1], dz1, dy1, da, g[1, 0], g[1, 1]
 
 
 def dense_weight_image(w, transpose, precision=None):
```

New measurement: 7.450 million stroke-tokens/sec (median of 6 runs). No clear change (+0.8%).
